# angeladai/sgnn

Hardware: AMD Instinct MI355X
Metric: TSDF blocks/sec fwd+bwd (64^3@5% occ, bs32) (higher is better)
Workload: dtype f32

## Files before the change

include/sgnn_hip.h:

```cpp
#ifndef SGNN_HIP_H
#define SGNN_HIP_H

#include <stdint.h>

#ifdef __cplusplus
extern "C" {
#endif

#define SGNN_OK 0
#define SGNN_EINVAL (-1)
#define SGNN_EHIP (-2)
#define SGNN_EOVERFLOW (-3)
#define SGNN_ENOWS (-4)

#define SGNN_STATUS_COORD_RANGE 1
#define SGNN_STATUS_DUPLICATE 2
#define SGNN_STATUS_OVERFLOW 4

typedef void *sgnn_stream_t;

const char *sgnn_last_error(void);
int sgnn_version(void);
const char *sgnn_arch(void);


int64_t sgnn_hash_capacity(int64_t n);

int sgnn_coords_from_i64(const int64_t *locs, int64_t n, int32_t *coords, int32_t *status,
                         const int64_t *n_dev, sgnn_stream_t stream);
int sgnn_coords_to_i64(const int32_t *coords, int64_t n, int64_t *locs, const int64_t *n_dev,
                       sgnn_stream_t stream);

int sgnn_hash_build(const int32_t *coords, int64_t n, uint64_t *keys, int32_t *vals, int64_t cap,
                    int32_t *status, const int64_t *n_dev, sgnn_stream_t stream);

int sgnn_hash_lookup(const uint64_t *keys, const int32_t *vals, int64_t cap, const int32_t *query,
                     int64_t m, int32_t *rows, const int64_t *m_dev, sgnn_stream_t stream);

#define SGNN_TUNE_UNKNOWN INT64_MIN
typedef struct sgnn_tune {
  int64_t conv_small;
  int64_t conv_small_rows;
  int64_t conv_unrolled;
  int64_t conv_one_round;
  int64_t conv_wide_epi;
  int64_t conv_dw_blocks;
  int64_t conv_dw_c1;
  int64_t rulebook_multi;
  int64_t scan_inline;
  int64_t chain_merged;
  int64_t prog_fusion;
  int64_t prog_lin_bn;
  int64_t prog_lin_add;
  int64_t bn_fuse;
} sgnn_tune;
int64_t sgnn_tune_set(const char *name, int64_t value);
int64_t sgnn_tune_get(const char *name);
const char *sgnn_tune_names(void);
const sgnn_tune *sgnn_tune_current(void);


int sgnn_rulebook_subm3(const uint64_t *keys, const int32_t *vals, int64_t cap,
                        const int32_t *coords, int64_t n, int32_t *nbr, int64_t ld,
                        const int64_t *n_dev, sgnn_stream_t stream);

#define SGNN_RULEBOOK_MULTI_MAX 4
int sgnn_rulebook_subm3_multi(int count, const uint64_t *const *keys, const int32_t *const *vals, const int64_t *caps,
                              const int32_t *const *coords, const int64_t *ns, int32_t *const *nbrs, const int64_t *lds,
                              const int64_t *const *n_devs, sgnn_stream_t stream);

int sgnn_rulebook_subm3_dense(const uint64_t *keys, const int32_t *vals, int64_t cap, const int32_t *coords, int64_t n,
                              int dim_z, int dim_y, int dim_x, int32_t *volume, int64_t volume_entries, int32_t *nbr,
                              int64_t ld, const int64_t *n_dev, sgnn_stream_t stream);
int sgnn_rulebook_subm3_volume(const int32_t *coords, int64_t n, int dim_z, int dim_y, int dim_x, int32_t *volume,
                               int64_t volume_entries, int32_t *nbr, int64_t ld, const int64_t *n_dev, int32_t *status,
                               sgnn_stream_t stream);

int64_t sgnn_down2_ws_bytes(int64_t nf);
int sgnn_rulebook_down2(const int32_t *fine_coords, int64_t nf, uint64_t *ckeys, int32_t *cvals,
                        int64_t ccap, int32_t *parent, int32_t *coarse_coords, int64_t *n_coarse,
                        void *ws, int64_t ws_bytes, sgnn_stream_t stream);
int sgnn_down2_tables(const int32_t *fine_coords, const int32_t *parent, int64_t nf,
                      int32_t *children, int64_t ldc, int64_t nc, int32_t *ptable, int64_t ldf,
                      const int64_t *nf_dev, const int64_t *nc_dev, sgnn_stream_t stream);

int64_t sgnn_down2_chain_ws_bytes(int64_t cap);
int sgnn_down2_chain(const int32_t *fine_coords, int64_t n0, const int64_t *n0_dev, int64_t cap, int depth,
                     void *const *ckeys, void *const *cvals, int64_t ccap, void *const *parent,
                     void *const *coarse_coords, int64_t *counts_dev, const int64_t *level_caps, int32_t *status,
                     void *ws, int64_t ws_bytes, sgnn_stream_t stream);

int64_t sgnn_down2_chain_tables_ws_bytes(int64_t cap, int depth);
int sgnn_down2_chain_tables(const int32_t *fine_coords, const int64_t *n0_dev, int64_t cap, int depth,
                            void *const *ckeys, void *const *cvals, int64_t ccap, void *const *parent,
                            void *const *coarse_coords, int64_t *counts_dev, const int64_t *level_caps,
                            void *const *children, void *const *ptable, int32_t *status, void *ws, int64_t ws_bytes,
                            sgnn_stream_t stream);

#define SGNN_CONV_TRANSPOSE_W 1
#define SGNN_CONV_FLIP_K 2
int sgnn_conv_fwd(const float *x, int64_t n_in, int cin, const float *w, int K, const int32_t *table,
                  int64_t ld, int64_t n_out, int cout, float *y, int flags, int in_shift,
                  sgnn_stream_t stream);

int sgnn_conv_fwd_ex(const float *x, int64_t n_in, int cin, const float *w, int K, const int32_t *table,
                     int64_t ld, int64_t n_out, int cout, float *y, int flags, int in_shift,
                     const int32_t *kmap, const int32_t *kadd, int in_mul, int groups, int table_rows,
                     sgnn_stream_t stream);
int sgnn_conv_bwd_weight_ex(const float *x, int64_t n_in, int cin, const float *dy, int cout,
                            const int32_t *table, int64_t ld, int K, int64_t n_out, float *dw, int in_shift,
                            const int32_t *kmap, const int32_t *kadd, int in_mul, int groups, int table_rows,
                            void *ws, int64_t ws_bytes, sgnn_stream_t stream);

int64_t sgnn_conv_stats_blocks(int64_t n_out);
int sgnn_conv_fwd_epi(const float *x, int64_t n_in, int cin, int64_t ldx, const float *w, int K,
                      const int32_t *table, int64_t ld, int64_t n_out, int cout, float *y, int64_t ldy, int flags,
                      const float *addend, int64_t ld_add, int stats, double *partial, const float *bn_x,
                      int64_t ld_bnx, const float *mean, const float *invstd, const float *gamma, const float *beta,
                      float leak, sgnn_stream_t stream);

int64_t sgnn_conv_bwd_weight_ws_bytes(int64_t n_out, int K, int cin, int cout);
int sgnn_conv_bwd_weight(const float *x, int64_t n_in, int cin, const float *dy, int cout,
                         const int32_t *table, int64_t ld, int K, int64_t n_out, float *dw, int in_shift, void *ws,
                         int64_t ws_bytes, sgnn_stream_t stream);

int sgnn_expand_weights(const float *w, int cin, int cout, float *wc, sgnn_stream_t stream);
int sgnn_expand_weights_bwd(const float *dwc, int cin, int cout, float *dw, sgnn_stream_t stream);

int64_t sgnn_bn_ws_bytes(int64_t n, int c);
int sgnn_bn_fwd(const float *x, int64_t n, int c, const float *gamma, const float *beta,
                float *running_mean, float *running_var, float eps, float momentum, int training,
                float leak, float *save_mean, float *save_invstd, float *y, void *ws,
                int64_t ws_bytes, sgnn_stream_t stream);
int sgnn_bn_bwd(const float *x, const float *dy, int64_t n, int c, const float *gamma,
                const float *beta, const float *save_mean, const float *save_invstd, int training,
                float leak, float *dx, float *dgamma, float *dbeta, void *ws, int64_t ws_bytes,
                sgnn_stream_t stream);
int sgnn_bn_bwd_add(const float *x, const float *dy, int64_t n, int c, const float *gamma, const float *beta,
                    const float *save_mean, const float *save_invstd, int training, float leak,
                    const float *addend, float *dx, float *dgamma, float *dbeta, void *ws, int64_t ws_bytes,
                    sgnn_stream_t stream);

int sgnn_bn_fwd_ex(const float *x, int64_t ldx, int64_t n, int c, const float *gamma, const float *beta,
                   float *running_mean, float *running_var, float eps, float momentum, int training, float leak,
                   float *save_mean, float *save_invstd, float *y, int64_t ldy, const double *pre_partial,
                   int64_t pre_nblk, void *ws, int64_t ws_bytes, sgnn_stream_t stream);
int sgnn_bn_bwd_ex(const float *x, int64_t ldx, const float *dy, int64_t ld_dy, int64_t n, int c, const float *gamma,
                   const float *beta, const float *save_mean, const float *save_invstd, int training, float leak,
                   const float *addend, int64_t ld_add, float *dx, int64_t ld_dx, float *dgamma, float *dbeta,
                   const double *pre_partial, int64_t pre_nblk, void *ws, int64_t ws_bytes, sgnn_stream_t stream);

int sgnn_copy_multi(void *const *dst, const void *const *src, const int64_t *bytes, int nregions, sgnn_stream_t stream);

int sgnn_gather_rows(const float *src, int c, const int32_t *idx, int64_t m, float *dst,
                     sgnn_stream_t stream);
int sgnn_gather_rows_dn(const float *src, int c, const int32_t *idx, const int64_t *m_dev, int64_t m_cap,
                        float *dst, sgnn_stream_t stream);
int sgnn_concat3_rows(const float *a, int ca, const int32_t *ia, const float *b, int cb, const int32_t *ib,
                      const float *c, int cc, const int32_t *ic, int64_t m, float *dst, sgnn_stream_t stream);
int sgnn_concat3_rows_bwd(const float *ddst, int ca, const int32_t *ia, int cb, const int32_t *ib, int cc,
                          const int32_t *ic, int64_t m, float *da, int64_t na, float *db, int64_t nb, float *dc,
                          int64_t nc, sgnn_stream_t stream);
int sgnn_scatter_rows(const float *src, int c, const int32_t *idx, int64_t m, float *dst,
                      int64_t n_dst, const int64_t *m_dev, sgnn_stream_t stream);
int sgnn_gather_sum(const float *src, int c, const int32_t *table, int64_t ld, int K,
                    int64_t n_out, float *dst, sgnn_stream_t stream);
int sgnn_repeat_rows(const float *src, int c, int64_t n, int rep, float *dst, sgnn_stream_t stream);
int sgnn_sum_groups(const float *src, int c, int64_t n, int rep, float *dst, sgnn_stream_t stream);
int sgnn_concat_rows(const float *a, int ca, const int32_t *ia, const float *b, int cb,
                     const int32_t *ib, int64_t m, float *dst, sgnn_stream_t stream);
int sgnn_concat_rows_bwd(const float *ddst, int ca, const int32_t *ia, int cb, const int32_t *ib,
                         int64_t m, float *da, int64_t na, float *db, int64_t nb,
                         sgnn_stream_t stream);
int sgnn_add(const float *a, const float *b, int64_t count, float *y, sgnn_stream_t stream);

int sgnn_expand8_coords(const int32_t *coords, int64_t n, int32_t *out, const int64_t *n_dev, sgnn_stream_t stream);
int sgnn_expand8_coords_i64(const int32_t *coords, int64_t n, int32_t *out, int64_t *locs, const int64_t *n_dev,
                            sgnn_stream_t stream);
int sgnn_dense_coords(int batch, int d0, int d1, int d2, int32_t *out, sgnn_stream_t stream);
int64_t sgnn_compact_ws_bytes(int64_t n);
int sgnn_compact_sigmoid(const float *logits, int64_t stride, int64_t n, int32_t *sel,
                         int64_t *count, void *ws, int64_t ws_bytes, sgnn_stream_t stream);
int sgnn_compact_dense(const int32_t *coords, int64_t n, const float *vol, int batch, int d0, int d1, int d2,
                       int32_t *sel, int64_t *count, void *ws, int64_t ws_bytes, sgnn_stream_t stream);
int sgnn_compact_mask(const uint8_t *mask, int64_t n, int32_t *sel, int64_t *count, void *ws,
                      int64_t ws_bytes, sgnn_stream_t stream);
int sgnn_compact_sigmoid_cap(const float *logits, int64_t stride, int64_t n, const int64_t *n_dev, int32_t *sel,
                             int64_t *count2, int64_t keep_cap, int32_t *status, void *ws, int64_t ws_bytes,
                             sgnn_stream_t stream);
int sgnn_compact_dense_cap(const int32_t *coords, int64_t n, const int64_t *n_dev, const float *vol, int batch, int d0,
                           int d1, int d2, int32_t *sel, int64_t *count2, int64_t keep_cap, int32_t *status, void *ws,
                           int64_t ws_bytes, sgnn_stream_t stream);
int sgnn_compact_sigmoid_cap_locs(const float *logits, int64_t stride, int64_t n, const int64_t *n_dev,
                                  const int32_t *coords, int32_t *sel, int32_t *locs, int64_t *count2, int64_t keep_cap,
                                  int32_t *status, void *ws, int64_t ws_bytes, sgnn_stream_t stream);
int sgnn_compact_dense_cap_locs(const int32_t *coords, int64_t n, const int64_t *n_dev, const float *vol, int batch, int d0,
                                int d1, int d2, int32_t *sel, int32_t *locs, int64_t *count2, int64_t keep_cap,
                                int32_t *status, void *ws, int64_t ws_bytes, sgnn_stream_t stream);

int sgnn_sparse_to_dense(const float *feats, const int32_t *coords, int64_t n, int c, float *dense,
                         int batch, int d0, int d1, int d2, sgnn_stream_t stream);
int sgnn_dense_to_sparse(const float *dense, const int32_t *coords, int64_t n, int c, float *feats,
                         int batch, int d0, int d1, int d2, sgnn_stream_t stream);

int64_t sgnn_linear_ws_bytes(int64_t n, int cin, int cout);
int sgnn_linear_fwd(const float *x, int64_t n, int cin, const float *w, const float *bias, int cout,
                    float *y, sgnn_stream_t stream);
// ... 366 lines not shown
```

sgnn_amd/csrc/bn.hip:

```cpp
#include "common.h"

#define BN_MAX_BLOCKS 2048
#define BN_FLUSH 2
#ifndef BN_U
#define BN_U 2
#endif
#define BN_FUSE_BLOCKS 4096
#define BN_FUSE_MAXC 64

struct BnGeom {
  int vec;
  int cq;
  int rpb;
};

static BnGeom bn_geom(int c) {
  BnGeom g;
  g.vec = (c % 4 == 0) ? 4 : 1;
  g.cq = c / g.vec;
  g.rpb = 256 / g.cq;
  if (g.rpb < 1) g.rpb = 1;
  return g;
}

static BnGeom bn_geom_scalar(int c) {
  BnGeom g;
  g.vec = 1;
  g.cq = c;
  g.rpb = 256 / c;
  if (g.rpb < 1) g.rpb = 1;
  return g;
}

static int bn_blocks(int64_t n, const BnGeom &g) {
  int64_t b = (n + (int64_t)g.rpb * BN_FLUSH - 1) / ((int64_t)g.rpb * BN_FLUSH);
  if (b < 1) b = 1;
  if (b > BN_MAX_BLOCKS) b = BN_MAX_BLOCKS;
  return (int)b;
}

SGNN_EXPORT int64_t sgnn_bn_ws_bytes(int64_t n, int c) {
  (void)n;
  return (int64_t)BN_MAX_BLOCKS * 2 * c * (int64_t)sizeof(double) + 4 * (int64_t)c * sizeof(float) + 256;
}

template <int VEC>
__device__ __forceinline__ void load_vec(const float *p, float (&v)[VEC]) {
  if constexpr (VEC == 4) {
    const float4 t = *reinterpret_cast<const float4 *>(p);
    v[0] = t.x; v[1] = t.y; v[2] = t.z; v[3] = t.w;
  } else {
    v[0] = *p;
  }
}
template <int VEC>
__device__ __forceinline__ void store_vec(float *p, const float (&v)[VEC]) {
  if constexpr (VEC == 4) {
    *reinterpret_cast<float4 *>(p) = make_float4(v[0], v[1], v[2], v[3]);
  } else {
    *p = v[0];
  }
}

template <int VEC, int MODE, bool LIN = false>
__global__ __launch_bounds__(256) void k_bn_partial(const float *__restrict__ x, int64_t ldx,
                                                   const float *__restrict__ dy, int64_t ld_dy, int64_t n, int c,
                                                   int cq, int rpb, const float *__restrict__ mean,
                                                   const float *__restrict__ invstd,
                                                   const float *__restrict__ gamma,
                                                   const float *__restrict__ beta, float leak,
                                                   double *__restrict__ partial, const int64_t *n_dev, BnLin lin) {
  extern __shared__ double sh[];
  const int tid = threadIdx.x;
  unsigned nblk = gridDim.x;
  if (n_dev) {
    n = sgnn_dyn_n(n, n_dev);
    int64_t b = (n + (int64_t)rpb * BN_FLUSH - 1) / ((int64_t)rpb * BN_FLUSH);
    if (b < 1) b = 1;
    if (b > BN_MAX_BLOCKS) b = BN_MAX_BLOCKS;
    if (b < (int64_t)nblk) nblk = (unsigned)b;
    if (blockIdx.x >= nblk) {
      for (int o = tid; o < 2 * c; o += 256) partial[(size_t)blockIdx.x * 2 * c + o] = 0.0;
      return;
    }
  }
  const int col = tid % cq, rloc = tid / cq;
  const bool active = rloc < rpb;
  double sa[VEC], sb[VEC];
#pragma unroll
  for (int v = 0; v < VEC; ++v) sa[v] = sb[v] = 0.0;
  float m_[VEC], is_[VEC], g_[VEC], b_[VEC];
  float lw[2][VEC];
  if constexpr (LIN) {
#pragma unroll
    for (int o = 0; o < 2; ++o)
#pragma unroll
      for (int v = 0; v < VEC; ++v) lw[o][v] = (active && o < lin.nout) ? lin.w[o][col * VEC + v] : 0.f;
  }
  if (MODE == 1 && active) {
#pragma unroll
    for (int v = 0; v < VEC; ++v) {
      m_[v] = mean[col * VEC + v];
      is_[v] = invstd[col * VEC + v];
      g_[v] = gamma ? gamma[col * VEC + v] : 1.f;
      b_[v] = beta ? beta[col * VEC + v] : 0.f;
    }
  }
  if (active) {
    const int64_t step = (int64_t)nblk * rpb;
    int64_t row = (int64_t)blockIdx.x * rpb + rloc;
    while (row < n) {
      float fa[VEC], fb[VEC];
#pragma unroll
      for (int v = 0; v < VEC; ++v) fa[v] = fb[v] = 0.f;
      float xv[BN_FLUSH][VEC], dv[BN_FLUSH][VEC];
      bool keep[BN_FLUSH];
#pragma unroll
      for (int it = 0; it < BN_FLUSH; ++it) {
        const int64_t rr = row + it * step;
        keep[it] = rr < n;
        const int64_t rc = rr < n ? rr : row;
        load_vec<VEC>(x + rc * ldx + col * VEC, xv[it]);
        if constexpr (LIN) {
#pragma unroll
          for (int v = 0; v < VEC; ++v) dv[it][v] = 0.f;
#pragma unroll
          for (int o = 0; o < 2; ++o)
            if (o < lin.nout) {
              const float gv = lin.g[rc * lin.ldg + o];
#pragma unroll
              for (int v = 0; v < VEC; ++v) dv[it][v] = fmaf(gv, lw[o][v], dv[it][v]);
            }
        } else if (MODE == 1) {
          load_vec<VEC>(dy + rc * ld_dy + col * VEC, dv[it]);
        }
      }
#pragma unroll
      for (int it = 0; it < BN_FLUSH; ++it) {
        if (MODE == 0) {
#pragma unroll
          for (int v = 0; v < VEC; ++v) {
            const float xm = keep[it] ? xv[it][v] : 0.f;
            fa[v] += xm;
            fb[v] = fmaf(xm, xm, fb[v]);
          }
        } else {
#pragma unroll
          for (int v = 0; v < VEC; ++v) {
            const float xh = (xv[it][v] - m_[v]) * is_[v];
            const float yv = fmaf(xh, g_[v], b_[v]);
            const float dz = keep[it] ? (yv > 0.f ? dv[it][v] : dv[it][v] * leak) : 0.f;
            fa[v] += dz;
            fb[v] = fmaf(dz, xh, fb[v]);
          }
        }
      }
      row += (int64_t)BN_FLUSH * step;
#pragma unroll
      for (int v = 0; v < VEC; ++v) {
        sa[v] += (double)fa[v];
        sb[v] += (double)fb[v];
      }
    }
  }
  double *mine = sh + ((size_t)rloc * cq + col) * 2 * VEC;
  if (active) {
#pragma unroll
    for (int v = 0; v < VEC; ++v) {
      mine[v] = sa[v];
      mine[VEC + v] = sb[v];
    }
  }
  __syncthreads();
  const int outs = cq * VEC * 2;
  for (int o = tid; o < outs; o += 256) {
    const int which = o / (cq * VEC);
    const int ch = o % (cq * VEC);
    const int cg = ch / VEC, v = ch % VEC;
    double s = 0.0;
    for (int rr = 0; rr < rpb; ++rr) s += sh[((size_t)rr * cq + cg) * 2 * VEC + which * VEC + v];
    partial[((size_t)blockIdx.x * 2 + which) * c + ch] = s;
  }
}

__device__ __forceinline__ void bn_reduce_channel(const double *__restrict__ partial, int nblk, int c, int ch,
                                                  double *sh, double &s, double &s2) {
  double a = 0.0, b = 0.0;
  for (int blk = threadIdx.x; blk < nblk; blk += 8 * 256) {
    double va[8], vb[8];
#pragma unroll
    for (int u = 0; u < 8; ++u) {
      const int bi = blk + u * 256;
      const bool ok = bi < nblk;
      va[u] = ok ? partial[((size_t)bi * 2 + 0) * c + ch] : 0.0;
      vb[u] = ok ? partial[((size_t)bi * 2 + 1) * c + ch] : 0.0;
    }
#pragma unroll
    for (int u = 0; u < 8; ++u) {
      a += va[u];
      b += vb[u];
    }
  }
  sh[threadIdx.x] = a;
  sh[256 + threadIdx.x] = b;
  __syncthreads();
  for (int d = 128; d > 0; d >>= 1) {
    if (threadIdx.x < d) {
      sh[threadIdx.x] += sh[threadIdx.x + d];
      sh[256 + threadIdx.x] += sh[256 + threadIdx.x + d];
    }
    __syncthreads();
  }
  s = sh[0];
  s2 = sh[256];
}

__global__ __launch_bounds__(256) void k_bn_finalize_fwd(const double *__restrict__ partial, int nblk,
                                                        int64_t n, int c, float eps, float momentum,
                                                        float *__restrict__ running_mean,
                                                        float *__restrict__ running_var,
                                                        float *__restrict__ save_mean,
                                                        float *__restrict__ save_invstd, const int64_t *n_dev) {
  __shared__ double sh[512];
  n = sgnn_dyn_n(n, n_dev);
  const int ch = blockIdx.x;
  double s, s2;
  bn_reduce_channel(partial, nblk, c, ch, sh, s, s2);
  if (threadIdx.x == 0) {
    if (n <= 0) {
      save_mean[ch] = 0.f;
      save_invstd[ch] = 0.f;
      return;
    }
    const double mean = s / (double)n;
    double var = s2 / (double)n - mean * mean;
    if (var < 0.0) var = 0.0;
    save_mean[ch] = (float)mean;
    save_invstd[ch] = (float)(1.0 / sqrt(var + (double)eps));
    if (running_mean) running_mean[ch] = momentum * running_mean[ch] + (1.f - momentum) * (float)mean;
    if (running_var) {
      const double unb = var * ((double)n / (double)(n > 1 ? n - 1 : 1));
      running_var[ch] = momentum * running_var[ch] + (1.f - momentum) * (float)unb;
    }
  }
}

__global__ __launch_bounds__(256) void k_bn_eval_stats(const float *__restrict__ running_mean,
                                                      const float *__restrict__ running_var, int c, float eps,
                                                      float *__restrict__ save_mean,
                                                      float *__restrict__ save_invstd) {
  for (int ch = threadIdx.x; ch < c; ch += 256) {
    save_mean[ch] = running_mean[ch];
    save_invstd[ch] = 1.0f / sqrtf(running_var[ch] + eps);
  }
}


struct BnFuse {
  const double *partial;
  int nblk;
  float eps, momentum;
  float *running_mean, *running_var, *save_mean, *save_invstd;
  float *dgamma, *dbeta;
};

#ifndef BN_TOTALS_WIDE
#define BN_TOTALS_WIDE 1
#endif
typedef double f64x2 __attribute__((ext_vector_type(2)));
__device__ __forceinline__ void bn_fuse_totals(const BnFuse &f, int c, double *scratch, double *tot) {
  const int tid = threadIdx.x;
  const int tpc = 256 / c;
  if (BN_TOTALS_WIDE && (c & 1) == 0 && (((uintptr_t)f.partial) & 15) == 0) {
    const int hp = c >> 1;
    const int p2 = tid % hp, which = (tid / hp) & 1, part = tid / c;
    f64x2 acc = {0.0, 0.0};
    if (part < tpc) {
      constexpr int U = 32;
      for (int blk = part; blk < f.nblk; blk += U * tpc) {
        f64x2 v[U];
#pragma unroll
        for (int u = 0; u < U; ++u) {
          const int bi = blk + u * tpc;
          v[u] = bi < f.nblk ? *reinterpret_cast<const f64x2 *>(f.partial + ((size_t)bi * 2 + which) * c + 2 * p2) : f64x2{0.0, 0.0};
        }
#pragma unroll
        for (int u = 0; u < U; ++u) acc += v[u];
      }
      scratch[which * 256 + part * c + 2 * p2] = acc[0];
      scratch[which * 256 + part * c + 2 * p2 + 1] = acc[1];
    }
  } else {
    const int ch = tid % c, part = tid / c;
    double a = 0.0, b = 0.0;
    if (part < tpc) {
      for (int blk = part; blk < f.nblk; blk += 8 * tpc) {
        double va[8], vb[8];
#pragma unroll
        for (int u = 0; u < 8; ++u) {
          const int bi = blk + u * tpc;
          const bool ok = bi < f.nblk;
          va[u] = ok ? f.partial[((size_t)bi * 2 + 0) * c + ch] : 0.0;
          vb[u] = ok ? f.partial[((size_t)bi * 2 + 1) * c + ch] : 0.0;
        }
#pragma unroll
        for (int u = 0; u < 8; ++u) {
          a += va[u];
          b += vb[u];
        }
      }
      scratch[part * c + ch] = a;
      scratch[256 + part * c + ch] = b;
    }
  }
  __syncthreads();
  if (tid < c) {
    double s1 = 0.0, s2 = 0.0;
    for (int p = 0; p < tpc; ++p) {
      s1 += scratch[p * c + tid];
      s2 += scratch[256 + p * c + tid];
    }
    tot[tid] = s1;
    tot[c + tid] = s2;
  }
  __syncthreads();
}

template <int VEC, bool FUSE>
__global__ __launch_bounds__(256) void k_bn_apply(const float *__restrict__ x, int64_t ldx, int64_t n, int c, int cq,
                                                 int rpb, const float *__restrict__ mean,
                                                 const float *__restrict__ invstd,
                                                 const float *__restrict__ gamma,
                                                 const float *__restrict__ beta, float leak,
                                                 float *__restrict__ y, int64_t ldy, BnFuse fuse,
                                                 const int64_t *n_dev) {
  __shared__ float s_mean[BN_FUSE_MAXC], s_inv[BN_FUSE_MAXC];
  __shared__ double s_scratch[512], s_tot[2 * BN_FUSE_MAXC];
  n = sgnn_dyn_n(n, n_dev);
  if (n <= 0) return;
  if constexpr (FUSE) {
    bn_fuse_totals(fuse, c, s_scratch, s_tot);
    for (int ch = threadIdx.x; ch < c; ch += 256) {
      const double s1 = s_tot[ch], s2 = s_tot[c + ch];
      const double mu = s1 / (double)n;
      double var = s2 / (double)n - mu * mu;
      if (var < 0.0) var = 0.0;
      const float fm = (float)mu, fi = (float)(1.0 / sqrt(var + (double)fuse.eps));
      s_mean[ch] = fm;
      s_inv[ch] = fi;
      if (blockIdx.x == 0) {
        fuse.save_mean[ch] = fm;
        fuse.save_invstd[ch] = fi;
        if (fuse.running_mean) fuse.running_mean[ch] = fuse.momentum * fuse.running_mean[ch] + (1.f - fuse.momentum) * fm;
        if (fuse.running_var) {
          const double unb = var * ((double)n / (double)(n > 1 ? n - 1 : 1));
          fuse.running_var[ch] = fuse.momentum * fuse.running_var[ch] + (1.f - fuse.momentum) * (float)unb;
        }
      }
    }
    __syncthreads();
    mean = s_mean;
    invstd = s_inv;
  }
  const int tid = threadIdx.x;
  const int col = tid % cq, rloc = tid / cq;
  if (rloc >= rpb) return;
  float km[VEC], ki[VEC], kg[VEC], kb[VEC];
#pragma unroll
  for (int v = 0; v < VEC; ++v) {
    const int ch = col * VEC + v;
    km[v] = mean[ch];
    ki[v] = invstd[ch];
    kg[v] = gamma ? gamma[ch] : 1.f;
    kb[v] = beta ? beta[ch] : 0.f;
  }
  const int64_t step = (int64_t)gridDim.x * rpb;
  for (int64_t r0 = (int64_t)blockIdx.x * rpb + rloc; r0 < n; r0 += step * BN_U) {
    float xv[BN_U][VEC];
#pragma unroll
    for (int u = 0; u < BN_U; ++u) {
      const int64_t r = r0 + u * step;
      load_vec<VEC>(x + (r < n ? r : r0) * ldx + col * VEC, xv[u]);
    }
#pragma unroll
    for (int u = 0; u < BN_U; ++u) {
      const int64_t r = r0 + u * step;
      if (r >= n) break;
      float yv[VEC];
#pragma unroll
      for (int v = 0; v < VEC; ++v) yv[v] = sgnn_bn_act(xv[u][v], km[v], ki[v], kg[v], kb[v], leak);
      store_vec<VEC>(y + r * ldy + col * VEC, yv);
    }
  }
}

__global__ __launch_bounds__(256) void k_bn_finalize_bwd(const double *__restrict__ partial, int nblk,
                                                        int64_t n, int c, float *__restrict__ dgamma,
                                                        float *__restrict__ dbeta, float *__restrict__ coef,
                                                        const int64_t *n_dev) {
  __shared__ double sh[512];
  n = sgnn_dyn_n(n, n_dev);
  const int ch = blockIdx.x;
  double s, s2;
  bn_reduce_channel(partial, nblk, c, ch, sh, s, s2);
  if (threadIdx.x == 0) {
    if (dbeta) dbeta[ch] = (float)s;
    if (dgamma) dgamma[ch] = (float)s2;
    coef[ch] = n > 0 ? (float)(s / (double)n) : 0.f;
    coef[c + ch] = n > 0 ? (float)(s2 / (double)n) : 0.f;
  }
}

template <int VEC, bool LIN, bool FUSE>
__global__ __launch_bounds__(256) void k_bn_bwd_apply(const float *__restrict__ x, int64_t ldx,
                                                     const float *__restrict__ dy, int64_t ld_dy, int64_t n, int c,
                                                     int cq, int rpb, const float *__restrict__ mean,
                                                     const float *__restrict__ invstd,
                                                     const float *__restrict__ gamma,
                                                     const float *__restrict__ beta, float leak, int training,
                                                     const float *__restrict__ coef, float *dx, int64_t ld_dx,
                                                     BnFuse fuse, const float *addend, int64_t ld_add,
                                                     const int64_t *n_dev, BnLin lin) {
  __shared__ float s_coef[2 * BN_FUSE_MAXC];
  __shared__ double s_scratch[512], s_tot[2 * BN_FUSE_MAXC];
  n = sgnn_dyn_n(n, n_dev);
  if constexpr (FUSE) {
    bn_fuse_totals(fuse, c, s_scratch, s_tot);
    for (int ch = threadIdx.x; ch < c; ch += 256) {
      const double s1 = s_tot[ch], s2 = s_tot[c + ch];
      s_coef[ch] = n > 0 ? (float)(s1 / (double)n) : 0.f;
      s_coef[c + ch] = n > 0 ? (float)(s2 / (double)n) : 0.f;
      if (blockIdx.x == 0) {
        if (fuse.dbeta) fuse.dbeta[ch] = (float)s1;
        if (fuse.dgamma) fuse.dgamma[ch] = (float)s2;
      }
    }
    __syncthreads();
    coef = s_coef;
  }
  const int tid = threadIdx.x;
  const int col = tid % cq, rloc = tid / cq;
  if (rloc >= rpb) return;
  float km[VEC], ki[VEC], kg[VEC], kb[VEC], k4[VEC], k5[VEC];
#pragma unroll
  for (int v = 0; v < VEC; ++v) {
    const int ch = col * VEC + v;
    km[v] = mean[ch];
    ki[v] = invstd[ch];
    kg[v] = gamma ? gamma[ch] : 1.f;
    kb[v] = beta ? beta[ch] : 0.f;
    k4[v] = training ? coef[ch] : 0.f;
    k5[v] = training ? coef[c + ch] : 0.f;
  }
  float lw[2][VEC];
  if constexpr (LIN) {
#pragma unroll
    for (int o = 0; o < 2; ++o)
#pragma unroll
      for (int v = 0; v < VEC; ++v) lw[o][v] = o < lin.nout ? lin.w[o][col * VEC + v] : 0.f;
  }
  const int64_t step = (int64_t)gridDim.x * rpb;
  for (int64_t r0 = (int64_t)blockIdx.x * rpb + rloc; r0 < n; r0 += step * BN_U) {
    float xv[BN_U][VEC], dv[BN_U][VEC], av[BN_U][VEC];
#pragma unroll
    for (int u = 0; u < BN_U; ++u) {
      const int64_t r = r0 + u * step, rc = (r < n ? r : r0);
      load_vec<VEC>(x + rc * ldx + col * VEC, xv[u]);
      if constexpr (LIN) {
#pragma unroll
        for (int v = 0; v < VEC; ++v) dv[u][v] = 0.f;
#pragma unroll
        for (int o = 0; o < 2; ++o)
          if (o < lin.nout) {
            const float gv = lin.g[rc * lin.ldg + o];
#pragma unroll
            for (int v = 0; v < VEC; ++v) dv[u][v] = fmaf(gv, lw[o][v], dv[u][v]);
          }
      } else {
        load_vec<VEC>(dy + rc * ld_dy + col * VEC, dv[u]);
      }
      if (addend) load_vec<VEC>(addend + rc * ld_add + col * VEC, av[u]);
    }
#pragma unroll
    for (int u = 0; u < BN_U; ++u) {
      const int64_t r = r0 + u * step;
      if (r >= n) break;
      float ov[VEC];
#pragma unroll
      for (int v = 0; v < VEC; ++v) {
        const float xh = (xv[u][v] - km[v]) * ki[v];
        const float t = fmaf(xh, kg[v], kb[v]);
        const float dz = t > 0.f ? dv[u][v] : dv[u][v] * leak;
        float d = dz;
        if (training) d = dz - k4[v] - xh * k5[v];
        ov[v] = d * kg[v] * ki[v];
        if (addend) ov[v] += av[u][v];
      }
      store_vec<VEC>(dx + r * ld_dx + col * VEC, ov);
    }
  }
}

static bool bn_fuse_ok(int64_t nblk, int c, int apply_grid) {
  return c <= BN_FUSE_MAXC && nblk <= BN_FUSE_BLOCKS && nblk * (int64_t)apply_grid * 2 * c * (int64_t)sizeof(double) <= (48ll << 20);
}

static int bn_apply_grid(int64_t n, const BnGeom &g) {
  int64_t b = (n + (int64_t)g.rpb * BN_U - 1) / ((int64_t)g.rpb * BN_U);
  if (b < 1) b = 1;
  if (b > 4096) b = 4096;
  return (int)b;
}

int sgnn_bn_fwd_impl(const float *x, int64_t ldx, int64_t n, int c, const float *gamma, const float *beta,
                     float *running_mean, float *running_var, float eps, float momentum, int training, float leak,
                     float *save_mean, float *save_invstd, float *y, int64_t ldy, const double *pre_partial,
                     int64_t pre_nblk, void *ws, int64_t ws_bytes, sgnn_stream_t stream, const int64_t *n_dev) {
  hipStream_t s = (hipStream_t)stream;
  SGNN_CHECK_ARG(n >= 0 && c >= 1 && (c % 4 == 0 ? c <= 1024 : c <= 256) && save_mean && save_invstd);
  SGNN_CHECK_ARG(training || (running_mean && running_var));
  if (ldx <= 0) ldx = c;
  if (ldy <= 0) ldy = c;
  SGNN_CHECK_ARG(ldx >= c && ldy >= c);
  BnGeom g = bn_geom(c);
  if (g.vec == 4 && (ldx % 4 || ldy % 4 || ((uintptr_t)x & 15) || ((uintptr_t)y & 15))) g = bn_geom_scalar(c);
  if (g.cq > 256) {
    sgnn_set_error("sgnn_bn_fwd: %d channels need 16-byte aligned rows (row strides multiples of 4 floats)", c);
    return SGNN_EINVAL;
  }
  BnFuse fuse{nullptr, 0, 0.f, 0.f, nullptr, nullptr, nullptr, nullptr, nullptr, nullptr};
  if (training && n > 0) {
    SGNN_CHECK_ARG(x);
    const double *partial = pre_partial;
    int64_t nblk = pre_nblk;
    if (!partial) {
      if (!ws || ws_bytes < sgnn_bn_ws_bytes(n, c)) {
        sgnn_set_error("sgnn_bn_fwd: workspace too small");
        return SGNN_ENOWS;
      }
      nblk = bn_blocks(n, g);
      const size_t shbytes = (size_t)g.rpb * g.cq * 2 * g.vec * sizeof(double);
      if (g.vec == 4)
        SGNN_LAUNCH((k_bn_partial<4, 0>), dim3((unsigned)nblk), dim3(256), shbytes, s, x, ldx, nullptr, 0, n, c,
                           g.cq, g.rpb, nullptr, nullptr, nullptr, nullptr, 0.f, (double *)ws, n_dev, BnLin{});
      else
        SGNN_LAUNCH((k_bn_partial<1, 0>), dim3((unsigned)nblk), dim3(256), shbytes, s, x, ldx, nullptr, 0, n, c,
                           g.cq, g.rpb, nullptr, nullptr, nullptr, nullptr, 0.f, (double *)ws, n_dev, BnLin{});
      partial = (const double *)ws;
    }
    if (g_tune.bn_fuse && bn_fuse_ok(nblk, c, bn_apply_grid(n, g)))
      fuse = BnFuse{partial, (int)nblk, eps, momentum, running_mean, running_var, save_mean, save_invstd, nullptr, nullptr};
    else
      SGNN_LAUNCH(k_bn_finalize_fwd, dim3(c), dim3(256), 0, s, partial, (int)nblk, n, c, eps, momentum,
                         running_mean, running_var, save_mean, save_invstd, n_dev);
  } else if (training) {
    SGNN_HIP_TRY(hipMemsetAsync(save_mean, 0, c * sizeof(float), s));
    SGNN_HIP_TRY(hipMemsetAsync(save_invstd, 0, c * sizeof(float), s));
  } else {
    SGNN_LAUNCH(k_bn_eval_stats, dim3(1), dim3(256), 0, s, (const float *)running_mean,
                       (const float *)running_var, c, eps, save_mean, save_invstd);
  }
  if (n > 0) {
    SGNN_CHECK_ARG(x && y);
    const int grid = bn_apply_grid(n, g);
#define BN_APPLY(VECV, FUSEV)                                                                                 \
  SGNN_LAUNCH((k_bn_apply<VECV, FUSEV>), dim3(grid), dim3(256), 0, s, x, ldx, n, c, g.cq, g.rpb,              \
              (const float *)save_mean, (const float *)save_invstd, gamma, beta, leak, y, ldy, fuse, n_dev)
    if (g.vec == 4 && fuse.partial) BN_APPLY(4, true);
    else if (g.vec == 4) BN_APPLY(4, false);
    else if (fuse.partial) BN_APPLY(1, true);
    else BN_APPLY(1, false);
#undef BN_APPLY
  }
  SGNN_CHECK_LAUNCH();
  return SGNN_OK;
}

SGNN_EXPORT int sgnn_bn_fwd(const float *x, int64_t n, int c, const float *gamma, const float *beta,
                            float *running_mean, float *running_var, float eps, float momentum, int training,
                            float leak, float *save_mean, float *save_invstd, float *y, void *ws,
                            int64_t ws_bytes, sgnn_stream_t stream) {
  return sgnn_bn_fwd_impl(x, c, n, c, gamma, beta, running_mean, running_var, eps, momentum, training, leak, save_mean,
                          save_invstd, y, c, nullptr, 0, ws, ws_bytes, stream);
}

SGNN_EXPORT int sgnn_bn_fwd_ex(const float *x, int64_t ldx, int64_t n, int c, const float *gamma, const float *beta,
                               float *running_mean, float *running_var, float eps, float momentum, int training,
                               float leak, float *save_mean, float *save_invstd, float *y, int64_t ldy,
                               const double *pre_partial, int64_t pre_nblk, void *ws, int64_t ws_bytes,
                               sgnn_stream_t stream) {
  return sgnn_bn_fwd_impl(x, ldx, n, c, gamma, beta, running_mean, running_var, eps, momentum, training, leak,
                          save_mean, save_invstd, y, ldy, pre_partial, pre_nblk, ws, ws_bytes, stream);
}

SGNN_EXPORT int sgnn_bn_bwd(const float *x, const float *dy, int64_t n, int c, const float *gamma,
                            const float *beta, const float *save_mean, const float *save_invstd, int training,
                            float leak, float *dx, float *dgamma, float *dbeta, void *ws, int64_t ws_bytes,
                            sgnn_stream_t stream) {
  return sgnn_bn_bwd_impl(x, c, dy, c, n, c, gamma, beta, save_mean, save_invstd, training, leak, nullptr, c, dx, c,
                          dgamma, dbeta, nullptr, 0, ws, ws_bytes, stream);
}

SGNN_EXPORT int sgnn_bn_bwd_add(const float *x, const float *dy, int64_t n, int c, const float *gamma,
                                const float *beta, const float *save_mean, const float *save_invstd, int training,
                                float leak, const float *addend, float *dx, float *dgamma, float *dbeta, void *ws,
                                int64_t ws_bytes, sgnn_stream_t stream) {
  return sgnn_bn_bwd_impl(x, c, dy, c, n, c, gamma, beta, save_mean, save_invstd, training, leak, addend, c, dx, c,
                          dgamma, dbeta, nullptr, 0, ws, ws_bytes, stream);
}

SGNN_EXPORT int sgnn_bn_bwd_ex(const float *x, int64_t ldx, const float *dy, int64_t ld_dy, int64_t n, int c,
                               const float *gamma, const float *beta, const float *save_mean,
                               const float *save_invstd, int training, float leak, const float *addend,
                               int64_t ld_add, float *dx, int64_t ld_dx, float *dgamma, float *dbeta,
                               const double *pre_partial, int64_t pre_nblk, void *ws, int64_t ws_bytes,
                               sgnn_stream_t stream) {
  return sgnn_bn_bwd_impl(x, ldx, dy, ld_dy, n, c, gamma, beta, save_mean, save_invstd, training, leak, addend, ld_add,
                          dx, ld_dx, dgamma, dbeta, pre_partial, pre_nblk, ws, ws_bytes, stream);
}

int sgnn_bn_bwd_impl(const float *x, int64_t ldx, const float *dy, int64_t ld_dy, int64_t n, int c, const float *gamma,
                     const float *beta, const float *save_mean, const float *save_invstd, int training, float leak,
                     const float *addend, int64_t ld_add, float *dx, int64_t ld_dx, float *dgamma, float *dbeta,
                     const double *pre_partial, int64_t pre_nblk, void *ws, int64_t ws_bytes, sgnn_stream_t stream,
                     const int64_t *n_dev, const BnLin *lin) {
  hipStream_t s = (hipStream_t)stream;
  SGNN_CHECK_ARG(n >= 0 && c >= 1 && (c % 4 == 0 ? c <= 1024 : c <= 256) && save_mean && save_invstd);
  SGNN_CHECK_ARG(!lin || (lin->g && lin->nout >= 1 && lin->nout <= 2 && lin->w[0] && (lin->nout < 2 || lin->w[1]) && !pre_partial));
  if (n == 0) {
    if (dgamma) SGNN_HIP_TRY(hipMemsetAsync(dgamma, 0, c * sizeof(float), s));
    if (dbeta) SGNN_HIP_TRY(hipMemsetAsync(dbeta, 0, c * sizeof(float), s));
    return SGNN_OK;
  }
  SGNN_CHECK_ARG(x && (dy || lin) && dx);
  if (ldx <= 0) ldx = c;
  if (ld_dy <= 0) ld_dy = c;
  if (ld_dx <= 0) ld_dx = c;
  if (ld_add <= 0) ld_add = c;
  SGNN_CHECK_ARG(ldx >= c && ld_dy >= c && ld_dx >= c && ld_add >= c);
  if (!ws || ws_bytes < sgnn_bn_ws_bytes(n, c)) {
    sgnn_set_error("sgnn_bn_bwd: workspace too small");
    return SGNN_ENOWS;
  }
  BnGeom g = bn_geom(c);
  if (g.vec == 4 && (ldx % 4 || ld_dy % 4 || ld_dx % 4 || ld_add % 4 || ((uintptr_t)x & 15) || ((uintptr_t)dy & 15) ||
                     ((uintptr_t)dx & 15) || ((uintptr_t)addend & 15)))
    g = bn_geom_scalar(c);
  if (g.cq > 256) {
    sgnn_set_error("sgnn_bn_bwd: %d channels need 16-byte aligned rows (row strides multiples of 4 floats)", c);
    return SGNN_EINVAL;
  }
  const double *partial = pre_partial;
  int64_t nblk = pre_nblk;
  float *coef = (float *)((char *)ws + (size_t)BN_MAX_BLOCKS * 2 * c * sizeof(double));
  if (!partial) {
    nblk = bn_blocks(n, g);
    const size_t shbytes = (size_t)g.rpb * g.cq * 2 * g.vec * sizeof(double);
    if (lin && g.vec == 4)
      SGNN_LAUNCH((k_bn_partial<4, 1, true>), dim3((unsigned)nblk), dim3(256), shbytes, s, x, ldx, dy, ld_dy, n, c, g.cq,
// ... 32 lines not shown
```

sgnn_amd/csrc/common.h:

```cpp
#pragma once
#include <hip/hip_runtime.h>
#include <stdint.h>
#include <stdio.h>
#include "../../include/sgnn_hip.h"

#define SGNN_EXPORT extern "C" __attribute__((visibility("default")))

extern "C" int sgnn_stamp(const char *label, sgnn_stream_t stream);
extern sgnn_tune g_tune;

void sgnn_set_error(const char *fmt, ...);
int sgnn_prof_begin_launch(int kind, int64_t n_out, int cin, int cout, int K, int flags, hipStream_t s);
void sgnn_prof_end_launch(int slot, hipStream_t s);

__device__ __forceinline__ float sgnn_bn_act(float x, float mean, float invstd, float gamma, float beta, float leak) {
  const float xh = (x - mean) * invstd;
  const float t = fmaf(xh, gamma, beta);
  return t > 0.f ? t : t * leak;
}

struct ConvEpi {
  int64_t ldx, ldy, ld_add;
  const float *addend;
  int stats;
  double *partial;
  const float *bn_x;
  int64_t ld_bnx;
  const float *mean, *invstd, *gamma, *beta;
  float leak;
  const int64_t *n_dev;
};

int sgnn_conv_fwd_impl(const float *x, int64_t n_in, int cin, const float *w, int K, const int32_t *table, int64_t ld,
                       int64_t n_out, int cout, float *y, int flags, int in_shift, const int32_t *kmap,
                       const int32_t *kadd, int in_mul, int groups, int table_rows, const ConvEpi *epi,
                       sgnn_stream_t stream);
int64_t sgnn_conv_grid_blocks(int64_t n_out, int cin, int cout, int K);
struct BnLin {
  const float *g;
  int64_t ldg;
  const float *w[2];
  int nout;
};
int sgnn_bn_fwd_impl(const float *x, int64_t ldx, int64_t n, int c, const float *gamma, const float *beta,
                     float *running_mean, float *running_var, float eps, float momentum, int training, float leak,
                     float *save_mean, float *save_invstd, float *y, int64_t ldy, const double *pre_partial,
                     int64_t pre_nblk, void *ws, int64_t ws_bytes, sgnn_stream_t stream, const int64_t *n_dev = nullptr);
int sgnn_bn_bwd_impl(const float *x, int64_t ldx, const float *dy, int64_t ld_dy, int64_t n, int c, const float *gamma,
                     const float *beta, const float *save_mean, const float *save_invstd, int training, float leak,
                     const float *addend, int64_t ld_add, float *dx, int64_t ld_dx, float *dgamma, float *dbeta,
                     const double *pre_partial, int64_t pre_nblk, void *ws, int64_t ws_bytes, sgnn_stream_t stream,
                     const int64_t *n_dev = nullptr, const struct BnLin *lin = nullptr);
bool sgnn_conv_epi_supported(int cin, int cout);
bool dw_shape_ok(int cin, int cout);
#define DW_BATCH_MAX 28
struct DwDesc {
  const float *partial;
  float *dw;
  int64_t nblk, elems;
  int blk0;
};
struct DwBatch {
  DwDesc d[DW_BATCH_MAX];
  int n;
};
extern DwBatch *sgnn_dw_batch;
int sgnn_dw_batch_flush(DwBatch *b, hipStream_t s);
int sgnn_gather_rows_ld(const float *src, int64_t ld_src, int c, const int32_t *idx, int64_t m, float *dst,
                        int64_t ld_dst, sgnn_stream_t stream, const int64_t *n_dev = nullptr);
int sgnn_gather_sum_ld(const float *src, int64_t ld_src, int c, const int32_t *table, int64_t ld, int K, int64_t n_out,
                       float *dst, int64_t ld_dst, sgnn_stream_t stream, const int64_t *n_dev = nullptr);
int sgnn_add_ld(const float *a, int64_t lda, const float *b, int64_t ldb, int64_t n, int c, float *y, int64_t ldy,
                sgnn_stream_t stream, const int64_t *n_dev = nullptr);
int sgnn_fill32(void *p, uint32_t pattern, int64_t words, hipStream_t s);
int sgnn_fill32_multi(void *const *p, const int64_t *words, int nregions, uint32_t pattern, hipStream_t s);
int sgnn_copy_words(void *dst, const void *src, int64_t words, hipStream_t s);
int sgnn_sum_groups_dn(const float *src, int c, int64_t n, int rep, float *dst, sgnn_stream_t stream, const int64_t *n_dev);
int sgnn_concat_rows_dn(const float *a, int ca, const int32_t *ia, const float *b, int cb, const int32_t *ib, int64_t m,
                        float *dst, sgnn_stream_t stream, const int64_t *n_dev);
int sgnn_concat_rows_bwd_dn(const float *ddst, int ca, const int32_t *ia, int cb, const int32_t *ib, int64_t m, float *da,
                            int64_t na, float *db, int64_t nb, sgnn_stream_t stream, const int64_t *n_dev);
int sgnn_concat3_rows_dn(const float *a, int ca, const int32_t *ia, const float *b, int cb, const int32_t *ib,
                         const float *c, int cc, const int32_t *ic, int64_t m, float *dst, sgnn_stream_t stream,
                         const int64_t *n_dev);
int sgnn_concat3_rows_bwd_dn(const float *ddst, int ca, const int32_t *ia, int cb, const int32_t *ib, int cc,
                             const int32_t *ic, int64_t m, float *da, int64_t na, float *db, int64_t nb, float *dc,
                             int64_t nc, sgnn_stream_t stream, const int64_t *n_dev);
int sgnn_conv_bwd_weight_impl(const float *x, int64_t n_in, int cin, int64_t ldx, const float *dy, int cout, int64_t ld_dy,
                              const int32_t *table, int64_t ld, int K, int64_t n_out, float *dw, int in_shift,
                              const int32_t *kmap, const int32_t *kadd, int in_mul, int groups, int table_rows, void *ws,
                              int64_t ws_bytes, sgnn_stream_t stream, const int64_t *n_dev = nullptr);
int sgnn_expand_maps(const int32_t **S, const int32_t **ST, const int32_t **PAR);
int sgnn_linear_fwd_rows(const float *x, int64_t n, int cin, const float *const *w, const float *const *b, int cout,
                         float *y, sgnn_stream_t stream, const int64_t *n_dev = nullptr);
int sgnn_linear_bwd_rows(const float *x, const float *dy, int64_t n, int cin, const float *const *w, int cout,
                         float *dx, float *const *dw, float *const *db, void *ws, int64_t ws_bytes,
                         sgnn_stream_t stream, const int64_t *n_dev = nullptr, const float *addend = nullptr,
                         int64_t ld_add = 0);

extern long long sgnn_launch_counter;
#define SGNN_LAUNCH(...)           \
  do {                             \
    ++sgnn_launch_counter;         \
    hipLaunchKernelGGL(__VA_ARGS__); \
  } while (0)

#define SGNN_CHECK_ARG(cond)                                                    \
  do {                                                                          \
    if (!(cond)) {                                                              \
      sgnn_set_error("%s: invalid argument: %s", __func__, #cond);              \
      return SGNN_EINVAL;                                                       \
    }                                                                           \
  } while (0)

#define SGNN_CHECK_LAUNCH()                                                     \
  do {                                                                          \
    hipError_t e_ = hipGetLastError();                                          \
    if (e_ != hipSuccess) {                                                     \
      sgnn_set_error("%s: HIP error: %s", __func__, hipGetErrorString(e_));     \
      return SGNN_EHIP;                                                         \
    }                                                                           \
  } while (0)

#define SGNN_HIP_TRY(expr)                                                      \
  do {                                                                          \
    hipError_t e_ = (expr);                                                     \
    if (e_ != hipSuccess) {                                                     \
      sgnn_set_error("%s: %s failed: %s", __func__, #expr, hipGetErrorString(e_)); \
      return SGNN_EHIP;                                                         \
    }                                                                           \
  } while (0)

__device__ __forceinline__ int64_t sgnn_dyn_n(int64_t n_host, const int64_t *n_dev) {
  if (!n_dev) return n_host;
  const int64_t v = *n_dev;
  return v < n_host ? (v < 0 ? 0 : v) : n_host;
}

static inline int sgnn_grid_for(int64_t work, int block, int cap = 1 << 20) {
  int64_t g = (work + block - 1) / block;
  if (g < 1) g = 1;
  if (g > cap) g = cap;
  return (int)g;
}

__device__ __forceinline__ unsigned sgnn_xcd_tile(unsigned b, unsigned nwg) {
  const unsigned q = nwg >> 3, r = nwg & 7u, xcd = b & 7u, i = b >> 3;
  return (xcd < r ? xcd * (q + 1) : r * (q + 1) + (xcd - r) * q) + i;
}

#define SGNN_EMPTY_KEY 0xFFFFFFFFFFFFFFFFull

__device__ __forceinline__ uint64_t sgnn_pack_key(int z, int y, int x, int b) {
  return ((uint64_t)(uint32_t)b << 48) | ((uint64_t)(uint32_t)z << 32) | ((uint64_t)(uint32_t)y << 16) |
         (uint64_t)(uint32_t)x;
}

__device__ __forceinline__ uint64_t sgnn_hash64(uint64_t k) {
  k ^= k >> 33;
  k *= 0xff51afd7ed558ccdull;
  k ^= k >> 33;
  k *= 0xc4ceb9fe1a85ec53ull;
  k ^= k >> 33;
  return k;
}

__device__ __forceinline__ int32_t sgnn_hash_find(const uint64_t *__restrict__ keys,
                                                  const int32_t *__restrict__ vals, uint64_t mask,
                                                  uint64_t key) {
  uint64_t slot = sgnn_hash64(key) & mask;
  while (true) {
    uint64_t k = keys[slot];
    if (k == key) return vals[slot];
    if (k == SGNN_EMPTY_KEY) return -1;
    slot = (slot + 1) & mask;
  }
}

__device__ __forceinline__ uint8_t sgnn_known_code(float s, float vs) {
  if (s < -vs) {
    const float q = __fdiv_rn(-s, vs);
    return !(q < 2147483648.0f) ? 2 : (uint8_t)max(2, min(255, (int)q + 1));
  }
  return s <= vs ? 1 : 0;
}

__device__ __forceinline__ int sgnn_block_rank256(bool flag, int *lds4, int &total) {
  const int lane = threadIdx.x & 63, wave = threadIdx.x >> 6;
  unsigned long long bal = __ballot(flag);
  int prefix = __popcll(bal & ((1ull << lane) - 1ull));
  if (lane == 0) lds4[wave] = __popcll(bal);
  __syncthreads();
  int w0 = lds4[0], w1 = lds4[1], w2 = lds4[2], w3 = lds4[3];
  __syncthreads();
  int base = (wave > 0 ? w0 : 0) + (wave > 1 ? w1 : 0) + (wave > 2 ? w2 : 0);
  total = w0 + w1 + w2 + w3;
  return base + prefix;
}

template <typename T, int NC>
__device__ __forceinline__ void sgnn_block_sum256(T (&sh)[NC][256], const T (&v)[NC]) {
  for (int c = 0; c < NC; ++c) sh[c][threadIdx.x] = v[c];
  __syncthreads();
  for (int d = 128; d > 0; d >>= 1) {
    if (threadIdx.x < d)
      for (int c = 0; c < NC; ++c) sh[c][threadIdx.x] += sh[c][threadIdx.x + d];
    __syncthreads();
  }
}
```

sgnn_amd/csrc/conv.hip:

```cpp
#include <stdlib.h>
#include "common.h"

#include "conv_common.h"

#define CONV_SMALL_GRID ((int64_t)((g_tune.conv_small_rows + CONV_ROWS_PER_BLOCK - 1) / CONV_ROWS_PER_BLOCK))

template <int CIN, int COUT, int M, bool EX, bool WEPI>
__device__ __forceinline__ void conv_fwd_body(const float *__restrict__ x, int64_t n_in,
                                              const float *__restrict__ w, const int32_t *__restrict__ table,
                                              int64_t ld, int K, int64_t n_out, float *y, int flags,
                                              int in_shift, const ConvEx &ex, const ConvEpi &epi, int wg_cap) {
  using C = ConvCfg<CIN, COUT>;
  constexpr int V = C::V, CINP = C::CINP, NT = C::NT, KC = C::KC;
  constexpr int RPW = 16 * M;
  __shared__ __attribute__((aligned(16))) float wl[KC * C::PER_K];
  __shared__ double sred[4 * 2 * NT * 16];
  static_assert(!WEPI || (NT == 1 && M == 4 && !EX && COUT % 4 == 0), "wide epilogue: one column tile of whole 16-byte chunks");
  __shared__ float ecst[WEPI ? 64 : 1];

  const int tid = threadIdx.x, lane = tid & 63, wave = tid >> 6;
  const int r = lane & 15, q = lane >> 4;
  const unsigned groups = EX ? (unsigned)ex.groups : 1u;
  unsigned nwg = gridDim.x;
  if (epi.n_dev) n_out = sgnn_dyn_n(n_out, epi.n_dev);
  int J = 1;
  if constexpr (!EX) {
    if (wg_cap > 0) {
      const int64_t w1 = (n_out + 4 * RPW - 1) / (4 * RPW);
      J = (int)((w1 + wg_cap - 1) / wg_cap);
      if (J < 1) J = 1;
    }
  }
  if (epi.n_dev || J > 1) {
    const int64_t rows_wg = (int64_t)4 * RPW * J;
    nwg = (unsigned)((n_out + rows_wg - 1) / rows_wg) * groups;
    if (blockIdx.x >= nwg) {
      if (!EX && epi.stats)
        for (int o = tid; o < 2 * COUT; o += 256) epi.partial[(size_t)blockIdx.x * 2 * COUT + o] = 0.0;
      return;
    }
  }
  const unsigned lin = sgnn_xcd_tile(blockIdx.x, nwg);
  const unsigned tile = lin / groups, grp = lin % groups;
  int64_t row0 = ((int64_t)tile * J * 4 + wave) * RPW;
  const int32_t *kmap = nullptr, *kadd_g = nullptr;
  if constexpr (EX) {
    w += (int64_t)grp * K * CIN * COUT;
    kmap = ex.kmap ? ex.kmap + grp * K : nullptr;
    kadd_g = ex.kadd ? ex.kadd + grp * K : nullptr;
  }
  const int table_rows = EX ? ex.table_rows : K;
  const bool transpose = flags & SGNN_CONV_TRANSPOSE_W, flip = flags & SGNN_CONV_FLIP_K;

  const uint32_t ldx4 = (uint32_t)epi.ldx * 4u;
  const __amdgpu_buffer_rsrc_t rs_x = make_rsrc(x, (uint32_t)(((n_in - 1) * epi.ldx + CIN) * 4));
  const __amdgpu_buffer_rsrc_t rs_t = make_rsrc(table, (uint32_t)((int64_t)table_rows * ld * 4));
  uint32_t lane_off = (uint32_t)(row0 + (lane & (RPW - 1))) * 4u;
  const uint32_t ld4 = (uint32_t)ld * 4u;
  int perm[M];
#pragma unroll
  for (int m = 0; m < M; ++m) perm[m] = (m * 16 + r) * 4;

  f32x4 acc[M][NT];
  double s1[NT], s2[NT];
#pragma unroll
  for (int nt = 0; nt < NT; ++nt) s1[nt] = s2[nt] = 0.0;
  if constexpr (WEPI) conv_epi_wide_constants<COUT>(ecst, epi, epi.stats);

  auto load_idx = [&](int k) -> int32_t {
    if constexpr (EX) {
      const int trow = kmap ? kmap[k] : k;
      int32_t id = (int32_t)__builtin_amdgcn_raw_buffer_load_b32(rs_t, lane_off, trow * ld4, 0);
      return (id >> in_shift) * ex.in_mul + ((kadd_g && id >= 0) ? kadd_g[k] : 0);
    } else {
      return (int32_t)__builtin_amdgcn_raw_buffer_load_b32(rs_t, lane_off, k * ld4, 0) >> in_shift;
    }
  };
  auto gather = [&](int32_t iv, float(&a)[M][V]) {
#pragma unroll
    for (int m = 0; m < M; ++m) {
      const int32_t id = __builtin_amdgcn_ds_bpermute(perm[m], iv);
      buf_load_floats<V>(rs_x, (uint32_t)id * ldx4 + (uint32_t)(q * V * 4), a[m]);
    }
  };
  auto stage = [&](int k) {
    conv_stage_weights<CIN, COUT>(wl, w, K, k, (K - k) < KC ? (K - k) : KC, transpose, flip);
  };
  auto load_b = [&](int kk, float(&b)[NT][V]) {
#pragma unroll
    for (int nt = 0; nt < NT; ++nt) {
      const float *bp = wl + (kk * NT * 16 + nt * 16 + r) * CINP + q * V;
#pragma unroll
      for (int s = 0; s < V; ++s) b[nt][s] = bp[s];
    }
  };
  auto mma_b = [&](float(&a)[M][V], const float(&b)[NT][V]) {
    if constexpr (CINP != CIN) {
#pragma unroll
      for (int m = 0; m < M; ++m)
#pragma unroll
        for (int s = 0; s < V; ++s)
          if (3 * V + s >= CIN) a[m][s] = (q >= conv_first_pad_quarter<CIN, V>(s)) ? 0.f : a[m][s];
    }
#pragma unroll
    for (int s = 0; s < V; ++s)
#pragma unroll
      for (int m = 0; m < M; ++m)
#pragma unroll
        for (int nt = 0; nt < NT; ++nt)
          acc[m][nt] = __builtin_amdgcn_mfma_f32_16x16x4f32(a[m][s], b[nt][s], acc[m][nt], 0, 0, 0);
  };
  auto mma = [&](int kk, float(&a)[M][V]) {
    float b[NT][V];
    load_b(kk, b);
    mma_b(a, b);
  };

  const int klast = K - 1;
  auto idx_at = [&](int k) { return load_idx(k < klast ? k : klast); };
  for (int j = 0; j < J; ++j) {
  if (j > 0) {
    const int64_t wg_row0 = ((int64_t)tile * J + j) * 4 * RPW;
    if (wg_row0 >= n_out) break;
    row0 = wg_row0 + wave * RPW;
    lane_off = (uint32_t)(row0 + (lane & (RPW - 1))) * 4u;
  }
  const bool restage = j == 0 || K > KC;
  EpiRows<WEPI ? M : 1> erows;
#pragma unroll
  for (int m = 0; m < M; ++m)
#pragma unroll
    for (int nt = 0; nt < NT; ++nt) acc[m][nt] = f32x4{0.f, 0.f, 0.f, 0.f};
  if constexpr (V <= 4 && (NT >= 2 || M == 1)) {
    float a0[M][V], a1[M][V], a2[M][V];
    for (int k0 = 0; k0 < K; k0 += KC) {
      const int kc = (K - k0) < KC ? (K - k0) : KC;
      if (restage) stage(k0);
      gather(idx_at(k0), a0);
      gather(idx_at(k0 + 1), a1);
      int32_t iv2 = idx_at(k0 + 2), iv3 = idx_at(k0 + 3), iv4 = idx_at(k0 + 4);
      int kk = 0;
      for (; kk + 2 < kc; kk += 3) {
        gather(iv2, a2);
        iv2 = idx_at(k0 + kk + 5);
        __builtin_amdgcn_sched_barrier(0);
        mma(kk, a0);
        __builtin_amdgcn_sched_barrier(0);
        gather(iv3, a0);
        iv3 = idx_at(k0 + kk + 6);
        __builtin_amdgcn_sched_barrier(0);
        mma(kk + 1, a1);
        __builtin_amdgcn_sched_barrier(0);
        gather(iv4, a1);
        iv4 = idx_at(k0 + kk + 7);
        __builtin_amdgcn_sched_barrier(0);
        mma(kk + 2, a2);
        __builtin_amdgcn_sched_barrier(0);
      }
      if (kk < kc) mma(kk, a0);
      if (kk + 1 < kc) mma(kk + 1, a1);
    }
  } else {
    float a0[M][V], a1[M][V], b0[NT][V], b1[NT][V];
    for (int k0 = 0; k0 < (WEPI ? 1 : K); k0 += KC) {
      const int kc = (K - k0) < KC ? (K - k0) : KC;
      if (restage) stage(k0);
      int32_t iv1 = idx_at(k0 + 1), iv2 = idx_at(k0 + 2);
      gather(idx_at(k0), a0);
      load_b(0, b0);
      int kk = 0;
      for (; kk + 1 < kc; kk += 2) {
        gather(iv1, a1);
        const int32_t iv3 = idx_at(k0 + kk + 3);
        load_b(kk + 1, b1);
        __builtin_amdgcn_sched_barrier(0);
        mma_b(a0, b0);
        __builtin_amdgcn_sched_barrier(0);
        gather(iv2, a0);
        iv1 = iv3;
        iv2 = idx_at(k0 + kk + 4);
        load_b(kk + 2 < kc ? kk + 2 : kc - 1, b0);
        __builtin_amdgcn_sched_barrier(0);
        mma_b(a1, b1);
        __builtin_amdgcn_sched_barrier(0);
      }
      if constexpr (WEPI) {
        __builtin_amdgcn_sched_barrier(0);
        if constexpr (SGNN_WEPI_EARLY != 0) conv_epi_wide_prefetch<COUT, M>(erows, row0, n_out, epi, epi.stats, x, SGNN_WEPI_EARLY);
        __builtin_amdgcn_sched_barrier(0);
      }
      if (kk < kc) mma_b(a0, b0);
    }
  }

  if constexpr (WEPI)
    conv_epi_wide_finish<COUT, M>(acc, erows, row0, n_out, y, epi, epi.stats, ecst, s1, s2, x);
  else
    conv_epilogue_rows<COUT, M, NT>(acc, row0, n_out, groups, grp, y, epi, EX ? 0 : epi.stats, x, s1, s2);
  }
  conv_epilogue_stats<COUT, NT>(s1, s2, epi, EX ? 0 : epi.stats, sred, blockIdx.x);
}

template <int CIN, int COUT, int M, bool EX>
__global__ __launch_bounds__(256) void k_conv_fwd(const float *__restrict__ x, int64_t n_in,
                                                 const float *__restrict__ w, const int32_t *__restrict__ table,
                                                 int64_t ld, int K, int64_t n_out, float *y, int flags,
                                                 int in_shift, ConvEx ex, ConvEpi epi, int wg_cap) {
  conv_fwd_body<CIN, COUT, M, EX, false>(x, n_in, w, table, ld, K, n_out, y, flags, in_shift, ex, epi, wg_cap);
}

template <int CIN, int COUT>
__global__ __launch_bounds__(256) __attribute__((amdgpu_waves_per_eu(4, 8))) void k_conv_fwd_w(
    const float *__restrict__ x, int64_t n_in, const float *__restrict__ w, const int32_t *__restrict__ table, int64_t ld,
    int K, int64_t n_out, float *y, int flags, int in_shift, ConvEx ex, ConvEpi epi, int wg_cap) {
  conv_fwd_body<CIN, COUT, CONV_MREP, false, true>(x, n_in, w, table, ld, K, n_out, y, flags, in_shift, ex, epi, wg_cap);
}

template <int CIN, int COUT>
__global__ __launch_bounds__(256) void k_conv_small(const float *__restrict__ x, int64_t n_in,
                                                   const float *__restrict__ w, const int32_t *__restrict__ table,
                                                   int64_t ld, int K, int64_t n_out, float *y, int flags, int in_shift,
                                                   ConvEpi epi) {
  using C = ConvCfg<CIN, COUT>;
  constexpr int V = C::V, CINP = C::CINP, NT = C::NT;
  constexpr int KW = 7;
  __shared__ float red[4][NT * 256];
  __shared__ double sred[4][2][NT * 16];
  const int tid = threadIdx.x, lane = tid & 63, wave = tid >> 6;
  const int r = lane & 15, q = lane >> 4;
  const int64_t row0 = (int64_t)blockIdx.x * 16;
  if (epi.n_dev) {
    n_out = sgnn_dyn_n(n_out, epi.n_dev);
    if (row0 >= n_out) {
      if (epi.stats)
        for (int o = tid; o < 2 * COUT; o += 256) epi.partial[(size_t)blockIdx.x * 2 * COUT + o] = 0.0;
      return;
    }
  }
  const bool transpose = flags & SGNN_CONV_TRANSPOSE_W, flip = flags & SGNN_CONV_FLIP_K;
  const int per = (K + 3) >> 2;
  const int k0 = wave * per;
  const int nk = (K - k0) < per ? ((K - k0) > 0 ? (K - k0) : 0) : per;

  const uint32_t ldx4 = (uint32_t)epi.ldx * 4u, ldy4 = (uint32_t)epi.ldy * 4u;
  const __amdgpu_buffer_rsrc_t rs_x = make_rsrc(x, (uint32_t)(((n_in - 1) * epi.ldx + CIN) * 4));
  const __amdgpu_buffer_rsrc_t rs_t = make_rsrc(table, (uint32_t)((int64_t)K * ld * 4));
  const __amdgpu_buffer_rsrc_t rs_y = make_rsrc(y, (uint32_t)(((n_out - 1) * epi.ldy + COUT) * 4));
  const uint32_t lane_off = (uint32_t)(row0 + r) * 4u;
  const uint32_t ld4 = (uint32_t)ld * 4u;

  int32_t id[KW];
#pragma unroll
  for (int kk = 0; kk < KW; ++kk) {
    const int k = k0 + (kk < nk ? kk : (nk > 0 ? nk - 1 : 0));
    id[kk] = (int32_t)__builtin_amdgcn_raw_buffer_load_b32(rs_t, lane_off, (k < K ? k : K - 1) * ld4, 0) >> in_shift;
  }
  float a[KW][V];
#pragma unroll
  for (int kk = 0; kk < KW; ++kk) buf_load_floats<V>(rs_x, (uint32_t)id[kk] * ldx4 + (uint32_t)(q * V * 4), a[kk]);
  float b[KW][NT][V];
  if (transpose) {
    const __amdgpu_buffer_rsrc_t rs_w = make_rsrc(w, (uint32_t)((int64_t)K * CIN * COUT * 4));
#pragma unroll
    for (int kk = 0; kk < KW; ++kk) {
      const int k = k0 + kk;
      const int ks = flip ? (K - 1 - k) : k;
#pragma unroll
      for (int nt = 0; nt < NT; ++nt) {
        const int n = nt * 16 + r;
        const bool okw = kk < nk && n < COUT;
        buf_load_floats<V>(rs_w, okw ? (uint32_t)((ks * COUT + n) * CIN + q * V) * 4u : 0xFFFFF800u, b[kk][nt]);
        if constexpr (CINP != CIN) {
#pragma unroll
          for (int s = 0; s < V; ++s)
            if (3 * V + s >= CIN) b[kk][nt][s] = (q >= conv_first_pad_quarter<CIN, V>(s)) ? 0.f : b[kk][nt][s];
        }
      }
    }
  } else if constexpr (V == 4 && CIN <= 16 && (CIN * COUT) % 4 == 0) {
    constexpr int SL = CIN * COUT, G4 = SL / 4, NL = (G4 + 63) / 64;
    static_assert(SL <= NT * 256, "the weight slice must fit the wave's partial-tile buffer");
    float *ws = red[wave];
    const __amdgpu_buffer_rsrc_t rs_w = make_rsrc(w, (uint32_t)((int64_t)K * SL * 4));
    float g[KW][NL][4];
#pragma unroll
    for (int kk = 0; kk < KW; ++kk) {
      const int k = k0 + kk;
      const int ks = flip ? (K - 1 - k) : k;
#pragma unroll
      for (int l = 0; l < NL; ++l) {
        const int e4 = l * 64 + lane;
        buf_load_floats<4>(rs_w, (kk < nk && e4 < G4) ? (uint32_t)(ks * SL + e4 * 4) * 4u : 0xFFFFF800u, g[kk][l]);
      }
    }
    auto wave_sync = [] {
      __builtin_amdgcn_fence(__ATOMIC_RELEASE, "wavefront");
      __builtin_amdgcn_wave_barrier();
      __builtin_amdgcn_fence(__ATOMIC_ACQUIRE, "wavefront");
    };
#pragma unroll
    for (int kk = 0; kk < KW; ++kk) {
      wave_sync();
#pragma unroll
      for (int l = 0; l < NL; ++l) {
        const int e4 = l * 64 + lane;
        if (e4 < G4) {
#pragma unroll
          for (int j = 0; j < 4; ++j) ws[e4 * 4 + j] = g[kk][l][j];
        }
      }
      wave_sync();
#pragma unroll
      for (int nt = 0; nt < NT; ++nt) {
        const int n = nt * 16 + r;
#pragma unroll
        for (int s = 0; s < V; ++s) {
          const int c = q * V + s;
          b[kk][nt][s] = (c < CIN && n < COUT) ? ws[c * COUT + n] : 0.f;
        }
      }
    }
  } else {
#pragma unroll
    for (int kk = 0; kk < KW; ++kk) {
      const int k = k0 + kk;
      const int ks = flip ? (K - 1 - k) : k;
#pragma unroll
      for (int nt = 0; nt < NT; ++nt) {
        const int n = nt * 16 + r;
#pragma unroll
        for (int s = 0; s < V; ++s) {
          const int c = q * V + s;
          float v = 0.f;
          if (kk < nk && c < CIN && n < COUT) v = w[((int64_t)ks * CIN + c) * COUT + n];
          b[kk][nt][s] = v;
        }
      }
    }
  }
  if constexpr (CINP != CIN) {
#pragma unroll
    for (int kk = 0; kk < KW; ++kk)
#pragma unroll
      for (int s = 0; s < V; ++s)
        if (3 * V + s >= CIN) a[kk][s] = (q >= conv_first_pad_quarter<CIN, V>(s)) ? 0.f : a[kk][s];
  }
  f32x4 acc[2][NT];
#pragma unroll
  for (int h = 0; h < 2; ++h)
#pragma unroll
    for (int nt = 0; nt < NT; ++nt) acc[h][nt] = f32x4{0.f, 0.f, 0.f, 0.f};
#pragma unroll
  for (int kk = 0; kk < KW; ++kk) {
    if (kk < nk) {
#pragma unroll
      for (int s = 0; s < V; ++s)
#pragma unroll
        for (int nt = 0; nt < NT; ++nt)
          acc[kk & 1][nt] = __builtin_amdgcn_mfma_f32_16x16x4f32(a[kk][s], b[kk][nt][s], acc[kk & 1][nt], 0, 0, 0);
    }
  }
#pragma unroll
  for (int nt = 0; nt < NT; ++nt)
#pragma unroll
    for (int i = 0; i < 4; ++i) red[wave][nt * 256 + (q * 4 + i) * 16 + r] = acc[0][nt][i] + acc[1][nt][i];
  __syncthreads();

  const bool has_add = epi.addend != nullptr;
  const __amdgpu_buffer_rsrc_t rs_a =
      make_rsrc(has_add ? epi.addend : x, has_add ? (uint32_t)(((n_out - 1) * epi.ld_add + COUT) * 4) : 0u);
  const uint32_t lda4 = (uint32_t)epi.ld_add * 4u;
  const int stats = epi.stats;
  const __amdgpu_buffer_rsrc_t rs_b =
      make_rsrc(stats == 2 ? epi.bn_x : x, stats == 2 ? (uint32_t)(((n_out - 1) * epi.ld_bnx + COUT) * 4) : 0u);
  const uint32_t ldb4 = (uint32_t)epi.ld_bnx * 4u;
  const int orow_l = tid >> 4, ocol_l = tid & 15;
  const int64_t row = row0 + orow_l;
#pragma unroll
  for (int nt = 0; nt < NT; ++nt) {
    const int col = nt * 16 + ocol_l;
    const bool ok = col < COUT && row < n_out;
    const int e = nt * 256 + orow_l * 16 + ocol_l;
    float v = (red[0][e] + red[1][e]) + (red[2][e] + red[3][e]);
    const uint32_t orow = (uint32_t)row;
    if (has_add) v += __uint_as_float(__builtin_amdgcn_raw_buffer_load_b32(rs_a, ok ? orow * lda4 + col * 4u : 0xFFFFFFFFu, 0, 0));
    __builtin_amdgcn_raw_buffer_store_b32(__float_as_uint(v), rs_y, ok ? orow * ldy4 + col * 4u : 0xFFFFFFFFu, 0, 0);
    if (stats) {
      double f1 = 0.0, f2 = 0.0;
      if (stats == 1) {
        f1 = ok ? (double)v : 0.0;
        f2 = f1 * f1;
      } else {
        float cm = 0.f, ci = 0.f, cg = 1.f, cb = 0.f;
        if (col < COUT) {
          cm = epi.mean[col];
          ci = epi.invstd[col];
          cg = epi.gamma ? epi.gamma[col] : 1.f;
          cb = epi.beta ? epi.beta[col] : 0.f;
        }
        const float xb = __uint_as_float(__builtin_amdgcn_raw_buffer_load_b32(rs_b, ok ? orow * ldb4 + col * 4u : 0xFFFFFFFFu, 0, 0));
        const float xh = (xb - cm) * ci;
        const float t = fmaf(xh, cg, cb);
        const float dz = ok ? (t > 0.f ? v : v * epi.leak) : 0.f;
        f1 = (double)dz;
        f2 = (double)dz * (double)xh;
      }
      f1 += __shfl_xor(f1, 16); f2 += __shfl_xor(f2, 16);
      f1 += __shfl_xor(f1, 32); f2 += __shfl_xor(f2, 32);
      if (lane < 16) {
        sred[wave][0][nt * 16 + lane] = f1;
        sred[wave][1][nt * 16 + lane] = f2;
      }
    }
  }
  if (stats) {
    __syncthreads();
    for (int o = tid; o < 2 * NT * 16; o += 256) {
      const int which = o / (NT * 16), col = o % (NT * 16);
      if (col < COUT)
        epi.partial[((size_t)blockIdx.x * 2 + which) * COUT + col] =
            (sred[0][which][col] + sred[1][which][col]) + (sred[2][which][col] + sred[3][which][col]);
    }
  }
}

__global__ __launch_bounds__(256) void k_conv_fwd_generic(const float *__restrict__ x, int cin,
                                                         const float *__restrict__ w, int K,
                                                         const int32_t *__restrict__ table, int64_t ld,
                                                         int64_t n_out, int cout, float *__restrict__ y,
                                                         int flags, int in_shift, ConvEx ex, const int64_t *n_dev) {
  n_out = sgnn_dyn_n(n_out, n_dev);
  const int64_t t = (int64_t)blockIdx.x * 256 + threadIdx.x;
  if (t >= n_out * ex.groups * cout) return;
  const int64_t orow = t / cout;
  const int n = (int)(t - orow * cout);
  const int64_t row = orow / ex.groups;
  const int grp = (int)(orow - row * ex.groups);
  w += (int64_t)grp * K * cin * cout;
  const bool transpose = flags & SGNN_CONV_TRANSPOSE_W, flip = flags & SGNN_CONV_FLIP_K;
  float acc = 0.f;
  for (int k = 0; k < K; ++k) {
    const int32_t idx = table[(int64_t)(ex.kmap ? ex.kmap[grp * K + k] : k) * ld + row];
    if (idx < 0) continue;
    const float *xr = x + ((int64_t)(idx >> in_shift) * ex.in_mul + (ex.kadd ? ex.kadd[grp * K + k] : 0)) * cin;
    const int ks = flip ? (K - 1 - k) : k;
    for (int c = 0; c < cin; ++c) {
      const float wv = transpose ? w[((int64_t)ks * cout + n) * cin + c] : w[((int64_t)ks * cin + c) * cout + n];
      acc = fmaf(xr[c], wv, acc);
    }
  }
  y[t] = acc;
}

#define CONV_EX_CASES(X) \
  X(48, 16) X(16, 48) X(24, 8) X(8, 24) X(16, 24) X(24, 16) X(24, 32) X(32, 24) X(64, 32) X(32, 64) X(56, 28) X(28, 56)

#define CONV_FWD_CASES(X) \
  X(1, 8) X(8, 8) X(8, 12) X(12, 12) X(12, 16) X(16, 16) X(34, 16) X(30, 16) X(26, 16) X(48, 16) \
  X(8, 1) X(12, 8) X(16, 12) X(16, 34) X(16, 30) X(16, 26) X(16, 48) X(32, 16) X(16, 32) X(4, 16) X(16, 4) \
  X(16, 24) X(24, 16) X(24, 32) X(32, 24) X(64, 32) X(32, 64) X(56, 28) X(28, 56) X(32, 32) X(28, 16) X(16, 28)

int64_t sgnn_conv_grid_blocks(int64_t n_out, int cin, int cout, int K) {
  const int64_t grid4 = (n_out + CONV_ROWS_PER_BLOCK - 1) / CONV_ROWS_PER_BLOCK;
  if (grid4 < CONV_SMALL_GRID) return (n_out + 15) / 16;
  return grid4;
}


bool sgnn_conv_u_supported(int cin, int cout, int K);
bool sgnn_conv_u_launch(const float *x, int64_t n_in, int cin, const float *w, int K, const int32_t *table, int64_t ld,
                        int64_t n_out, int cout, float *y, int flags, int in_shift, const ConvEpi &epi, hipStream_t s);

bool conv_wide_epi_ok(const ConvEpi &epi, const float *y, int K) {
  if (!g_tune.conv_wide_epi || K > 27 || (epi.ldy & 3) || ((uintptr_t)y & 15)) return false;
  if (epi.addend && ((epi.ld_add & 3) || ((uintptr_t)epi.addend & 15))) return false;
  if (epi.stats == 2 && ((epi.ld_bnx & 3) || ((uintptr_t)epi.bn_x & 15))) return false;
  return true;
}
template <int CI, int CO, bool EXV>
static void conv_launch_big(unsigned grid4, hipStream_t s, const float *x, int64_t n_in, const float *w, const int32_t *table,
                            int64_t ld, int K, int64_t n_out, float *y, int flags, int in_shift, const ConvEx &ex,
                            const ConvEpi &epi) {
  if constexpr (!EXV && CO % 4 == 0 && CO <= 16 && CI <= 16) {
    static_assert(ConvCfg<CI, CO>::KC >= 27, "one weight chunk holds a 3x3x3 filter");
    if (conv_wide_epi_ok(epi, y, K)) {
      SGNN_LAUNCH((k_conv_fwd_w<CI, CO>), dim3(grid4), dim3(256), 0, s, x, n_in, w, table, ld, K, n_out, y, flags, in_shift,
                  ex, epi, !g_tune.conv_one_round ? 0 : conv_wg_capacity<k_conv_fwd_w<CI, CO>>());
      return;
    }
  }
  SGNN_LAUNCH((k_conv_fwd<CI, CO, CONV_MREP, EXV>), dim3(grid4), dim3(256), 0, s, x, n_in, w, table, ld, K, n_out, y,
              flags, in_shift, ex, epi,
              (EXV || !g_tune.conv_one_round) ? 0 : conv_wg_capacity<k_conv_fwd<CI, CO, CONV_MREP, EXV>>());
}

bool sgnn_conv_epi_supported(int cin, int cout) {
#define X(CI, CO) \
  if (cin == CI && cout == CO) return true;
  CONV_FWD_CASES(X)
#undef X
  return false;
}

int sgnn_conv_fwd_impl(const float *x, int64_t n_in, int cin, const float *w, int K, const int32_t *table, int64_t ld,
                       int64_t n_out, int cout, float *y, int flags, int in_shift, const int32_t *kmap,
                       const int32_t *kadd, int in_mul, int groups, int table_rows, const ConvEpi *epi_in,
                       sgnn_stream_t stream) {
  SGNN_CHECK_ARG(cin >= 1 && cout >= 1 && K >= 1 && K <= 64 && n_out >= 0 && ld >= n_out && in_shift >= 0 &&
                 in_shift < 31 && in_mul >= 1 && groups >= 1 && groups <= 64 && table_rows >= 1 &&
                 table_rows <= 64 && (kmap || table_rows >= K));
  if (n_out == 0) return SGNN_OK;
  SGNN_CHECK_ARG(x && w && table && y && n_in >= 1);
  SGNN_CHECK_ARG(ld % CONV_ROWS_PER_BLOCK == 0);
  ConvEpi epi{};
  if (epi_in) epi = *epi_in;
  if (epi.ldx <= 0) epi.ldx = cin;
  if (epi.ldy <= 0) epi.ldy = cout;
  if (epi.ld_add <= 0) epi.ld_add = cout;
  if (epi.ld_bnx <= 0) epi.ld_bnx = cout;
  const bool plain = !kmap && !kadd && in_mul == 1 && groups == 1 && table_rows == K;
  const bool has_epi = epi.ldx != cin || epi.ldy != cout || epi.addend || epi.stats;
  SGNN_CHECK_ARG(epi.ldx >= cin && epi.ldx <= 1024 && epi.ldy >= cout && epi.ldy <= 1024 && epi.ld_add >= cout &&
                 epi.ld_add <= 1024 && epi.ld_bnx >= cout && epi.ld_bnx <= 1024);
  SGNN_CHECK_ARG(epi.stats >= 0 && epi.stats <= 2 && (!epi.stats || (plain && epi.partial)));
  SGNN_CHECK_ARG(epi.stats != 2 || (epi.bn_x && epi.mean && epi.invstd));
  SGNN_CHECK_ARG(!epi.stats || K <= 28);
  const int64_t lmax = epi.ldy > epi.ld_add ? (epi.ldy > epi.ld_bnx ? epi.ldy : epi.ld_bnx)
                                            : (epi.ld_add > epi.ld_bnx ? epi.ld_add : epi.ld_bnx);
  if (n_in * epi.ldx * 4 > 0xFFFFF000ll || n_out * groups * lmax * 4 > 0xFFFFF000ll ||
      (int64_t)table_rows * ld * 4 > 0xFFFFF000ll) {
    sgnn_set_error("sgnn_conv_fwd: a slab exceeds the 4 GiB raw-buffer window (n_in=%lld cin=%d n_out=%lld cout=%d)",
                   (long long)n_in, cin, (long long)n_out, cout);
    return SGNN_EOVERFLOW;
  }
  hipStream_t s = (hipStream_t)stream;
  const ConvEx ex{kmap, kadd, in_mul, groups, table_rows};
  const unsigned grid4 = (unsigned)((n_out + CONV_ROWS_PER_BLOCK - 1) / CONV_ROWS_PER_BLOCK) * (unsigned)groups;
  const unsigned grid1 = (unsigned)((n_out + 63) / 64) * (unsigned)groups;
  const bool small = grid4 < CONV_SMALL_GRID;
  bool done = false;
  const int prof = sgnn_prof_begin_launch(0, n_out * groups, cin, cout, K, flags, s);
#define LAUNCH_FWD(CI, CO, EXV)                                                                         \
  do {                                                                                                  \
    if (small && !EXV && K <= 28 && (g_tune.conv_small || epi.stats))                                      \
      SGNN_LAUNCH((k_conv_small<CI, CO>), dim3((unsigned)((n_out + 15) / 16)), dim3(256), 0, s,         \
                         x, n_in, w, table, ld, K, n_out, y, flags, in_shift, epi);                     \
    else if (small)                                                                                     \
      SGNN_LAUNCH((k_conv_fwd<CI, CO, 1, EXV>), dim3(grid1), dim3(256), 0, s, x, n_in, w, table,        \
                         ld, K, n_out, y, flags, in_shift, ex, epi, 0);                                 \
    else                                                                                                \
      conv_launch_big<CI, CO, EXV>(grid4, s, x, n_in, w, table, ld, K, n_out, y, flags, in_shift, ex, epi); \
    done = true;                                                                                        \
  } while (0)
  if (plain && !small && g_tune.conv_unrolled && sgnn_conv_u_supported(cin, cout, K))
    done = sgnn_conv_u_launch(x, n_in, cin, w, K, table, ld, n_out, cout, y, flags, in_shift, epi, s);
#define X(CI, CO) \
  if (!done && plain && cin == CI && cout == CO) LAUNCH_FWD(CI, CO, false);
  CONV_FWD_CASES(X)
#undef X
#define X(CI, CO) \
  if (!done && !plain && cin == CI && cout == CO) LAUNCH_FWD(CI, CO, true);
  CONV_EX_CASES(X)
#undef X
  if (!done) {
    if (has_epi) {
      sgnn_set_error("sgnn_conv_fwd_epi: strided / fused epilogues need one of the compiled (cin, cout) shapes, got (%d, %d)", cin, cout);
      return SGNN_EINVAL;
    }
    const int64_t total = n_out * groups * cout;
    SGNN_LAUNCH(k_conv_fwd_generic, dim3((unsigned)((total + 255) / 256)), dim3(256), 0, s, x, cin, w, K,
                       table, ld, n_out, cout, y, flags, in_shift, ex, epi.n_dev);
  }
  sgnn_prof_end_launch(prof, s);
  SGNN_CHECK_LAUNCH();
  return SGNN_OK;
}

SGNN_EXPORT int sgnn_conv_fwd_ex(const float *x, int64_t n_in, int cin, const float *w, int K, const int32_t *table,
                                 int64_t ld, int64_t n_out, int cout, float *y, int flags, int in_shift,
                                 const int32_t *kmap, const int32_t *kadd, int in_mul, int groups,
                                 int table_rows, sgnn_stream_t stream) {
  return sgnn_conv_fwd_impl(x, n_in, cin, w, K, table, ld, n_out, cout, y, flags, in_shift, kmap, kadd, in_mul,
                            groups, table_rows, nullptr, stream);
}

SGNN_EXPORT int sgnn_conv_fwd(const float *x, int64_t n_in, int cin, const float *w, int K, const int32_t *table,
                              int64_t ld, int64_t n_out, int cout, float *y, int flags, int in_shift,
                              sgnn_stream_t stream) {
  return sgnn_conv_fwd_impl(x, n_in, cin, w, K, table, ld, n_out, cout, y, flags, in_shift, nullptr, nullptr, 1, 1,
                            K, nullptr, stream);
}

SGNN_EXPORT int64_t sgnn_conv_stats_blocks(int64_t n_out) { return n_out > 0 ? sgnn_conv_grid_blocks(n_out, 0, 0, 0) : 0; }

SGNN_EXPORT int sgnn_conv_fwd_epi(const float *x, int64_t n_in, int cin, int64_t ldx, const float *w, int K,
                                  const int32_t *table, int64_t ld, int64_t n_out, int cout, float *y, int64_t ldy,
                                  int flags, const float *addend, int64_t ld_add, int stats, double *partial,
                                  const float *bn_x, int64_t ld_bnx, const float *mean, const float *invstd,
                                  const float *gamma, const float *beta, float leak, sgnn_stream_t stream) {
  ConvEpi epi{ldx, ldy, ld_add, addend, stats, partial, bn_x, ld_bnx, mean, invstd, gamma, beta, leak, nullptr};
  return sgnn_conv_fwd_impl(x, n_in, cin, w, K, table, ld, n_out, cout, y, flags, 0, nullptr, nullptr, 1, 1, K, &epi,
                            stream);
}

__device__ int32_t g_expand_maps[192];

int sgnn_expand_maps(const int32_t **S, const int32_t **ST, const int32_t **PAR) {
  static const int32_t *base = nullptr;
  if (!base) {
    int32_t host[192];
    for (int g = 0; g < 8; ++g)
      for (int i = 0; i < 8; ++i) {
        const int o0 = ((i >> 2) & 1) - 1 + ((g >> 2) & 1), o1 = ((i >> 1) & 1) - 1 + ((g >> 1) & 1),
                  o2 = (i & 1) - 1 + (g & 1);
        const int srow = (o0 + 1) * 9 + (o1 + 1) * 3 + (o2 + 1);
        host[g * 8 + i] = srow;
        host[64 + g * 8 + i] = 26 - srow;
        host[128 + g * 8 + i] = g;
      }
    SGNN_HIP_TRY(hipMemcpyToSymbol(HIP_SYMBOL(g_expand_maps), host, sizeof(host)));
    void *p = nullptr;
    SGNN_HIP_TRY(hipGetSymbolAddress(&p, HIP_SYMBOL(g_expand_maps)));
    base = (const int32_t *)p;
  }
  *S = base;
  *ST = base + 64;
  *PAR = base + 128;
  return SGNN_OK;
}

__device__ __forceinline__ void axis_taps(int j, int i, int &lo, int &hi) {
  if (j == 0) { lo = i ? 0 : -1; hi = i ? 1 : -1; }
  else        { lo = i ? 1 : -1; hi = i ? 1 : 0; }
}

__global__ __launch_bounds__(256) void k_expand_weights(const float *__restrict__ w, int cc, float *__restrict__ wc) {
  const int t = blockIdx.x * 256 + threadIdx.x;
  if (t >= 64 * cc) return;
  const int gi = t / cc, e = t - gi * cc, g = gi >> 3, i = gi & 7;
  int l0, h0, l1, h1, l2, h2;
  axis_taps((g >> 2) & 1, (i >> 2) & 1, l0, h0);
  axis_taps((g >> 1) & 1, (i >> 1) & 1, l1, h1);
  axis_taps(g & 1, i & 1, l2, h2);
  float acc = 0.f;
  for (int dz = l0; dz <= h0; ++dz)
    for (int dy = l1; dy <= h1; ++dy)
      for (int dx = l2; dx <= h2; ++dx) acc += w[(size_t)((dz + 1) * 9 + (dy + 1) * 3 + (dx + 1)) * cc + e];
  wc[t] = acc;
}

__global__ __launch_bounds__(256) void k_expand_weights_bwd(const float *__restrict__ dwc, int cc,
                                                           float *__restrict__ dw) {
  const int t = blockIdx.x * 256 + threadIdx.x;
  if (t >= 27 * cc) return;
  const int tap = t / cc, e = t - tap * cc;
  const int d0 = tap / 9 - 1, d1 = (tap / 3) % 3 - 1, d2 = tap % 3 - 1;
  float acc = 0.f;
  for (int g = 0; g < 8; ++g) {
    const int j0 = (g >> 2) & 1, j1 = (g >> 1) & 1, j2 = g & 1;
    const int i0 = j0 ? (d0 > 0) : (d0 >= 0), i1 = j1 ? (d1 > 0) : (d1 >= 0), i2 = j2 ? (d2 > 0) : (d2 >= 0);
    acc += dwc[(size_t)(g * 8 + i0 * 4 + i1 * 2 + i2) * cc + e];
  }
  dw[t] = acc;
}

SGNN_EXPORT int sgnn_expand_weights(const float *w, int cin, int cout, float *wc, sgnn_stream_t stream) {
  SGNN_CHECK_ARG(w && wc && cin >= 1 && cout >= 1);
  const int cc = cin * cout;
  SGNN_LAUNCH(k_expand_weights, dim3((64 * cc + 255) / 256), dim3(256), 0, (hipStream_t)stream, w, cc, wc);
  SGNN_CHECK_LAUNCH();
  return SGNN_OK;
}

SGNN_EXPORT int sgnn_expand_weights_bwd(const float *dwc, int cin, int cout, float *dw, sgnn_stream_t stream) {
  SGNN_CHECK_ARG(dwc && dw && cin >= 1 && cout >= 1);
  const int cc = cin * cout;
  SGNN_LAUNCH(k_expand_weights_bwd, dim3((27 * cc + 255) / 256), dim3(256), 0, (hipStream_t)stream, dwc, cc, dw);
  SGNN_CHECK_LAUNCH();
  return SGNN_OK;
}

template <int CIN, int COUT>
struct DwCfg {
  static constexpr int MT = (CIN + 15) / 16, NT = (COUT + 15) / 16;
  static constexpr int KPB = (MT * NT == 1) ? 9 : ((MT * NT <= 3) ? 5 : 3);
};

#ifndef DW_PAIR
#define DW_PAIR 1
#endif
template <int CIN, int COUT, bool EX, int KPBT = 0>
__global__ __launch_bounds__(256) void k_conv_dw(const float *__restrict__ x, int64_t n_in,
                                                const float *__restrict__ dy, const int32_t *__restrict__ table,
                                                int64_t ld, int K, int64_t n_out, float *__restrict__ partial,
                                                int64_t rows_per_block, int in_shift, ConvEx ex, int64_t ldx,
                                                int64_t ld_dy, const int64_t *n_dev) {
  if (n_dev) {
    n_out = sgnn_dyn_n(n_out, n_dev);
    const int64_t per = (n_out + gridDim.x - 1) / gridDim.x;
    rows_per_block = ((per + 255) / 256) * 256;
    if (rows_per_block < 256) rows_per_block = 256;
  }
  constexpr int MT = (CIN + 15) / 16, NT = (COUT + 15) / 16;
  constexpr int DW_KPB = KPBT > 0 ? KPBT : DwCfg<CIN, COUT>::KPB;
  constexpr int V = (CIN + 3) / 4, CINP = 4 * V;
  constexpr int W = (COUT + 3) / 4, COUTP = 4 * W;
  constexpr int XS = 64 * CINP, YS = 64 * COUTP;
  constexpr bool PAIR = DW_PAIR && MT * NT == 1 && CIN == 8 && KPBT == 0 && !EX;
  constexpr int XT = PAIR ? 2 : 1;
  constexpr int RED = DW_KPB * MT * 16 * NT * 16;
  constexpr int LDS_FLOATS = (4 * (XT * XS + YS) > RED) ? 4 * (XT * XS + YS) : RED;
  __shared__ __attribute__((aligned(16))) float lds[LDS_FLOATS];

  const int tid = threadIdx.x, lane = tid & 63, wave = tid >> 6;
  const int i16 = lane & 15, q = lane >> 4;
  const unsigned lin = sgnn_xcd_tile(blockIdx.y * gridDim.x + blockIdx.x, gridDim.x * gridDim.y);
  const unsigned bx = lin / gridDim.y, by = lin % gridDim.y;
  const unsigned groups = EX ? (unsigned)ex.groups : 1u;
  const unsigned kgroups = gridDim.y / groups;
  const unsigned grp = by / kgroups;
  const int k0 = (by % kgroups) * DW_KPB;
  const int32_t *kmap = (EX && ex.kmap) ? ex.kmap + grp * K : nullptr;
  const int table_rows = EX ? ex.table_rows : K;
  const int kc = (K - k0) < DW_KPB ? (K - k0) : DW_KPB;
  const int64_t blk_row0 = (int64_t)bx * rows_per_block;
  int64_t blk_row1 = blk_row0 + rows_per_block;
  if (blk_row1 > n_out) blk_row1 = n_out;

  const uint32_t ldx4 = (uint32_t)ldx * 4u;
  const __amdgpu_buffer_rsrc_t rs_x = make_rsrc(x, (uint32_t)(((n_in - 1) * ldx + CIN) * 4));
  const __amdgpu_buffer_rsrc_t rs_t = make_rsrc(table, (uint32_t)((int64_t)table_rows * ld * 4));
  const __amdgpu_buffer_rsrc_t rs_dy = make_rsrc(dy, (uint32_t)(((n_out * groups - 1) * ld_dy + COUT) * 4));
  const uint32_t ld4 = (uint32_t)ld * 4u;
  float *xs = lds + wave * (XT * XS + YS);
  float *ys = xs + XT * XS;

  constexpr int NP = (DW_KPB + 1) / 2;
  f32x4 accp[PAIR ? NP : 1];
#pragma unroll
  for (int p = 0; p < (PAIR ? NP : 1); ++p) accp[p] = f32x4{0.f, 0.f, 0.f, 0.f};
  f32x4 acc[DW_KPB][MT][NT];
#pragma unroll
  for (int kk = 0; kk < DW_KPB; ++kk)
#pragma unroll
    for (int mt = 0; mt < MT; ++mt)
#pragma unroll
      for (int nt = 0; nt < NT; ++nt) acc[kk][mt][nt] = f32x4{0.f, 0.f, 0.f, 0.f};

  constexpr bool RCX = (CIN == 16 || CIN == 8);
  constexpr int LPR = RCX ? CIN / 4 : 1, RPI = 64 / LPR, NI = RCX ? LPR : 4, GW = RCX ? 4 : V;
  const int rc_row = lane / LPR, rc_chunk = lane % LPR;
  auto gather = [&](int32_t iv, float(&g)[NI][GW]) {
#pragma unroll
    for (int m = 0; m < NI; ++m) {
      const int32_t id = __builtin_amdgcn_ds_bpermute((RCX ? m * RPI + rc_row : m * 16 + i16) * 4, iv);
      buf_load_floats<GW>(rs_x, (uint32_t)id * ldx4 + (uint32_t)(RCX ? rc_chunk * 16 : q * V * 4), g[m]);
    }
  };
  auto norm_rows = [&](float(&g)[NI][GW]) {
    if constexpr (CINP != CIN) {
#pragma unroll
      for (int m = 0; m < NI; ++m)
#pragma unroll
        for (int s = 0; s < GW; ++s)
          if (3 * V + s >= CIN) g[m][s] = (q == 3) ? 0.f : g[m][s];
    }
  };
  auto store_rows = [&](const float(&g)[NI][GW]) {
#pragma unroll
    for (int m = 0; m < NI; ++m) {
      float *p = RCX ? xs + (m * RPI + rc_row) * CINP + rc_chunk * 4 : xs + (m * 16 + i16) * CINP + q * V;
#pragma unroll
      for (int s = 0; s < GW; ++s) p[s] = g[m][s];
    }
  };
  auto store_rows_to = [&](const float(&g)[NI][GW], float *tile) {
#pragma unroll
    for (int m = 0; m < NI; ++m) {
      float *p = tile + (m * RPI + rc_row) * CINP + rc_chunk * 4;
#pragma unroll
      for (int s = 0; s < GW; ++s) p[s] = g[m][s];
    }
  };
  auto mma_pair = [&](int p, const float(&b)[16][NT]) {
    const float *src = xs + (i16 >> 3) * XS + (i16 & 7);
#pragma unroll
    for (int t = 0; t < 16; ++t) {
      const float a = ((i16 & 7) < CINP) ? src[(4 * t + q) * CINP] : 0.f;
      accp[p] = __builtin_amdgcn_mfma_f32_16x16x4f32(a, b[t][0], accp[p], 0, 0, 0);
    }
  };
  auto mma_chunk = [&](int kk, const float(&b)[16][NT]) {
#pragma unroll
    for (int t = 0; t < 16; ++t) {
      float a[MT];
#pragma unroll
      for (int mt = 0; mt < MT; ++mt) {
        const int ch = mt * 16 + i16;
        a[mt] = (ch < CINP) ? xs[(4 * t + q) * CINP + ch] : 0.f;
      }
#pragma unroll
      for (int mt = 0; mt < MT; ++mt)
#pragma unroll
        for (int nt = 0; nt < NT; ++nt)
          acc[kk][mt][nt] = __builtin_amdgcn_mfma_f32_16x16x4f32(a[mt], b[t][nt], acc[kk][mt][nt], 0, 0, 0);
    }
  };

  for (int64_t base = blk_row0 + wave * 64; base < blk_row1; base += 256) {
    int32_t idxv[DW_KPB];
#pragma unroll
    for (int kk = 0; kk < DW_KPB; ++kk) {
      const int ko = k0 + (kk < kc ? kk : kc - 1);
      int32_t id;
      if constexpr (EX) {
        const int trow = kmap ? kmap[ko] : ko;
        id = (int32_t)__builtin_amdgcn_raw_buffer_load_b32(rs_t, (uint32_t)(base + lane) * 4u, trow * ld4, 0);
        id = (id >> in_shift) * ex.in_mul + ((ex.kadd && id >= 0) ? ex.kadd[grp * K + ko] : 0);
      } else {
        id = (int32_t)__builtin_amdgcn_raw_buffer_load_b32(rs_t, (uint32_t)(base + lane) * 4u, ko * ld4, 0) >> in_shift;
      }
      idxv[kk] = (kk < kc) ? id : -1;
    }
    if constexpr (COUT == 16 || COUT == 8) {
      constexpr int LY = COUT / 4, RY = 64 / LY;
      const int yr = lane / LY, yc = lane % LY;
      float g[LY][4];
#pragma unroll
      for (int m = 0; m < LY; ++m) {
        const int64_t row = base + m * RY + yr;
        const uint32_t off = (row < blk_row1) ? (uint32_t)((row * groups + grp) * ld_dy + yc * 4) * 4u : 0xFFFFF800u;
        buf_load_floats<4>(rs_dy, off, g[m]);
      }
#pragma unroll
      for (int m = 0; m < LY; ++m) {
        float *p = ys + (m * RY + yr) * COUTP + yc * 4;
#pragma unroll
        for (int s = 0; s < 4; ++s) p[s] = g[m][s];
      }
    } else {
      float g[4][W];
#pragma unroll
      for (int m = 0; m < 4; ++m) {
        const int64_t row = base + m * 16 + i16;
        const uint32_t off =
            (row < blk_row1) ? (uint32_t)((row * groups + grp) * ld_dy + q * W) * 4u : 0xFFFFF800u;
        buf_load_floats<W>(rs_dy, off, g[m]);
        if constexpr (COUTP != COUT) {
#pragma unroll
          for (int s = 0; s < W; ++s)
            if (3 * W + s >= COUT) g[m][s] = (q == 3) ? 0.f : g[m][s];
        }
      }
#pragma unroll
      for (int m = 0; m < 4; ++m) {
        float *p = ys + (m * 16 + i16) * COUTP + q * W;
#pragma unroll
        for (int s = 0; s < W; ++s) p[s] = g[m][s];
      }
    }
    float b[16][NT];
#pragma unroll
    for (int t = 0; t < 16; ++t)
#pragma unroll
      for (int nt = 0; nt < NT; ++nt) {
        const int co = nt * 16 + i16;
        b[t][nt] = (co < COUTP) ? ys[(4 * t + q) * COUTP + co] : 0.f;
      }

    if constexpr (PAIR) {
      static_assert(RCX, "the paired path stores row-contiguous gathers");
      float ga[2][NI][GW], gb[2][NI][GW];
      auto idx_of = [&](int kk) { return kk < DW_KPB ? idxv[kk < DW_KPB ? kk : 0] : -1; };
      gather(idx_of(0), ga[0]);
      gather(idx_of(1), gb[0]);
#pragma unroll
      for (int p = 0; p < NP; ++p) {
        if (p + 1 < NP) {
          gather(idx_of(2 * p + 2), ga[(p + 1) & 1]);
          gather(idx_of(2 * p + 3), gb[(p + 1) & 1]);
        }
        __builtin_amdgcn_sched_barrier(0);
        store_rows_to(ga[p & 1], xs);
        store_rows_to(gb[p & 1], xs + XS);
        mma_pair(p, b);
        __builtin_amdgcn_sched_barrier(0);
      }
    } else if constexpr (MT * NT == 1) {
      float g0[NI][GW], g1[NI][GW];
      gather(idxv[0], g0);
#pragma unroll
      for (int kk = 0; kk < DW_KPB; kk += 2) {
        if (kk + 1 < DW_KPB) gather(idxv[kk + 1], g1);
        __builtin_amdgcn_sched_barrier(0);
        norm_rows(g0);
        store_rows(g0);
        mma_chunk(kk, b);
        __builtin_amdgcn_sched_barrier(0);
        if (kk + 1 < DW_KPB) {
          if (kk + 2 < DW_KPB) gather(idxv[kk + 2], g0);
          __builtin_amdgcn_sched_barrier(0);
          norm_rows(g1);
          store_rows(g1);
          mma_chunk(kk + 1, b);
          __builtin_amdgcn_sched_barrier(0);
        }
      }
    } else {
      float g0[NI][GW];
#pragma unroll
      for (int kk = 0; kk < DW_KPB; ++kk) {
        gather(idxv[kk], g0);
        norm_rows(g0);
        store_rows(g0);
        mma_chunk(kk, b);
      }
    }
  }

  __syncthreads();
  float *red = lds;
  for (int wv = 0; wv < 4; ++wv) {
    if constexpr (PAIR) {
      if (wave == wv) {
#pragma unroll
        for (int p = 0; p < NP; ++p)
#pragma unroll
          for (int i = 0; i < 4; ++i) {
            const int row = q * 4 + i, kk = 2 * p + (row >> 3), ci = row & 7, co = i16;
            if (kk < DW_KPB) {
              float *pr = &red[(kk * MT * 16 + ci) * NT * 16 + co];
              if (wv == 0)
                *pr = accp[p][i];
              else
                *pr += accp[p][i];
            }
          }
      }
    } else if (wave == wv) {
#pragma unroll
      for (int kk = 0; kk < DW_KPB; ++kk)
#pragma unroll
        for (int mt = 0; mt < MT; ++mt)
#pragma unroll
          for (int nt = 0; nt < NT; ++nt)
#pragma unroll
            for (int i = 0; i < 4; ++i) {
              const int ci = mt * 16 + q * 4 + i, co = nt * 16 + i16;
              float *p = &red[(kk * MT * 16 + ci) * NT * 16 + co];
              if (wv == 0)
                *p = acc[kk][mt][nt][i];
              else
                *p += acc[kk][mt][nt][i];
            }
    }
    __syncthreads();
  }
  float *out = partial + (((int64_t)bx * groups + grp) * K + k0) * CIN * COUT;
  for (int e = tid; e < kc * CIN * COUT; e += 256) {
    const int co = e % COUT, ci = (e / COUT) % CIN, kk = e / (CIN * COUT);
    out[e] = red[(kk * MT * 16 + ci) * NT * 16 + co];
  }
}

template <int COUT, int KP>
__global__ __launch_bounds__(256) void k_conv_dw_c1(const float *__restrict__ x, int64_t n_in, const float *__restrict__ dy,
                                                   const int32_t *__restrict__ table, int64_t ld, int K, int64_t n_out,
                                                   float *__restrict__ partial, int64_t rows_per_block, int in_shift,
                                                   int64_t ldx, int64_t ld_dy, const int64_t *n_dev) {
  static_assert(COUT % 4 == 0, "dy rows are loaded 16 bytes at a time");
  if (n_dev) {
    n_out = sgnn_dyn_n(n_out, n_dev);
    const int64_t per = (n_out + gridDim.x - 1) / gridDim.x;
    rows_per_block = ((per + 255) / 256) * 256;
    if (rows_per_block < 256) rows_per_block = 256;
  }
  constexpr int NV = KP * COUT;
  __shared__ float red[NV][65];
  const int tid = threadIdx.x, lane = tid & 63, wave = tid >> 6;
  const unsigned lin = sgnn_xcd_tile(blockIdx.y * gridDim.x + blockIdx.x, gridDim.x * gridDim.y);
  const unsigned bx = lin / gridDim.y, by = lin % gridDim.y;
  const int k0 = by * KP;
  const int kc = (K - k0) < KP ? (K - k0) : KP;
  const int64_t blk_row0 = (int64_t)bx * rows_per_block;
  int64_t blk_row1 = blk_row0 + rows_per_block;
  if (blk_row1 > n_out) blk_row1 = n_out;
  const __amdgpu_buffer_rsrc_t rs_x = make_rsrc(x, (uint32_t)(((n_in - 1) * ldx + 1) * 4));
  const __amdgpu_buffer_rsrc_t rs_t = make_rsrc(table, (uint32_t)((int64_t)K * ld * 4));
  const __amdgpu_buffer_rsrc_t rs_dy = make_rsrc(dy, (uint32_t)(((n_out - 1) * ld_dy + COUT) * 4));
  const uint32_t ld4 = (uint32_t)ld * 4u, ldx4 = (uint32_t)ldx * 4u;
  float acc[KP][COUT];
#pragma unroll
  for (int kk = 0; kk < KP; ++kk)
#pragma unroll
    for (int c = 0; c < COUT; ++c) acc[kk][c] = 0.f;
  for (int64_t row = blk_row0 + tid; row < blk_row1; row += 256) {
    int32_t id[KP];
#pragma unroll
    for (int kk = 0; kk < KP; ++kk) {
      const int ko = k0 + (kk < kc ? kk : kc - 1);
      id[kk] = (int32_t)__builtin_amdgcn_raw_buffer_load_b32(rs_t, (uint32_t)row * 4u, ko * ld4, 0) >> in_shift;
    }
    float g[COUT];
    buf_load_floats<COUT>(rs_dy, (uint32_t)(row * ld_dy) * 4u, g);
    float xv[KP];
#pragma unroll
    for (int kk = 0; kk < KP; ++kk)
      xv[kk] = __uint_as_float(__builtin_amdgcn_raw_buffer_load_b32(rs_x, (uint32_t)id[kk] * ldx4, 0, 0));
#pragma unroll
    for (int kk = 0; kk < KP; ++kk) {
      const float v = (kk < kc) ? xv[kk] : 0.f;
#pragma unroll
      for (int c = 0; c < COUT; ++c) acc[kk][c] = fmaf(v, g[c], acc[kk][c]);
    }
  }
  for (int wv = 0; wv < 4; ++wv) {
    if (wave == wv) {
#pragma unroll
      for (int kk = 0; kk < KP; ++kk)
#pragma unroll
        for (int c = 0; c < COUT; ++c) {
          float *p = &red[kk * COUT + c][lane];
          if (wv == 0)
            *p = acc[kk][c];
          else
            *p += acc[kk][c];
        }
    }
    __syncthreads();
  }
  float *out = partial + ((int64_t)bx * K + k0) * COUT;
  if (tid < kc * COUT) {
    float t = 0.f;
    for (int l = 0; l < 64; ++l) t += red[tid][l];
    out[tid] = t;
  }
}

__global__ __launch_bounds__(256) void k_dw_reduce(const float *__restrict__ partial, int64_t nblk,
                                                  int64_t elems, float *__restrict__ dw) {
  __shared__ float red[8][32];
  const int part = threadIdx.x >> 5, le = threadIdx.x & 31;
  const int64_t e = (int64_t)blockIdx.x * 32 + le;
  float s = 0.f;
  if (e < elems)
    for (int64_t b = part; b < nblk; b += 8) s += partial[b * elems + e];
  red[part][le] = s;
  __syncthreads();
  if (part == 0 && e < elems) {
    float t = 0.f;
#pragma unroll
    for (int p = 0; p < 8; ++p) t += red[p][le];
    dw[e] = t;
  }
}

__global__ __launch_bounds__(256) void k_dw_reduce_batch(DwBatch b) {
  __shared__ float red[8][32];
  int i = 0;
  while (i + 1 < b.n && (int)blockIdx.x >= b.d[i + 1].blk0) ++i;
  const DwDesc d = b.d[i];
  const int part = threadIdx.x >> 5, le = threadIdx.x & 31;
  const int64_t e = (int64_t)((int)blockIdx.x - d.blk0) * 32 + le;
  float s = 0.f;
  if (e < d.elems)
    for (int64_t k = part; k < d.nblk; k += 8) s += d.partial[k * d.elems + e];
  red[part][le] = s;
  __syncthreads();
  if (part == 0 && e < d.elems) {
    float t = 0.f;
#pragma unroll
    for (int p = 0; p < 8; ++p) t += red[p][le];
    d.dw[e] = t;
  }
}

DwBatch *sgnn_dw_batch = nullptr;

int sgnn_dw_batch_flush(DwBatch *b, hipStream_t s) {
  if (!b || b->n == 0) return SGNN_OK;
  int blocks = 0;
  for (int i = 0; i < b->n; ++i) {
    b->d[i].blk0 = blocks;
    blocks += (int)((b->d[i].elems + 31) / 32);
  }
  SGNN_LAUNCH(k_dw_reduce_batch, dim3((unsigned)blocks), dim3(256), 0, s, *b);
  b->n = 0;
  SGNN_CHECK_LAUNCH();
  return SGNN_OK;
}

__global__ __launch_bounds__(256) void k_conv_dw_generic(const float *__restrict__ x, int cin,
                                                        const float *__restrict__ dy, int cout,
                                                        const int32_t *__restrict__ table, int64_t ld, int K,
                                                        int64_t n_out, float *__restrict__ dw, int in_shift,
                                                        ConvEx ex, const int64_t *n_dev) {
  n_out = sgnn_dyn_n(n_out, n_dev);
  const int64_t e = (int64_t)blockIdx.x * 256 + threadIdx.x;
  if (e >= (int64_t)ex.groups * K * cin * cout) return;
  const int co = (int)(e % cout), ci = (int)((e / cout) % cin), k = (int)((e / ((int64_t)cin * cout)) % K);
  const int grp = (int)(e / ((int64_t)K * cin * cout));
  float s = 0.f;
  for (int64_t j = 0; j < n_out; ++j) {
    const int32_t id = table[(int64_t)(ex.kmap ? ex.kmap[grp * K + k] : k) * ld + j];
    if (id >= 0) {
      const float xv = x[((int64_t)(id >> in_shift) * ex.in_mul + (ex.kadd ? ex.kadd[grp * K + k] : 0)) * cin + ci];
      s = fmaf(xv, dy[(j * ex.groups + grp) * cout + co], s);
    }
  }
  dw[e] = s;
}

#define DW_FINE_ROWS 16384
static int64_t dw_rows_per_block(int64_t n_out) {
  int64_t rpb = (n_out + g_tune.conv_dw_blocks - 1) / g_tune.conv_dw_blocks;
  rpb = ((rpb + 255) / 256) * 256;
  if (rpb < 256) rpb = 256;
  return rpb;
}

bool dw_shape_ok(int cin, int cout) {
  static const int shapes[][2] = {{1, 8}, {8, 8}, {8, 12}, {12, 12}, {12, 16}, {16, 16}, {34, 16}, {30, 16}, {26, 16}, {48, 16},
                                  {32, 16}, {4, 16}, {16, 24}, {24, 32}, {64, 32}, {56, 28}, {32, 32}, {28, 16}};
  for (const auto &sh : shapes)
    if (sh[0] == cin && sh[1] == cout) return true;
  return false;
}

SGNN_EXPORT int64_t sgnn_conv_bwd_weight_ws_bytes(int64_t n_out, int K, int cin, int cout) {
  if (n_out <= 0) return 0;
  const int64_t rpb = dw_rows_per_block(n_out);
  const int64_t nblk = (n_out + rpb - 1) / rpb;
  return nblk * (int64_t)K * cin * cout * (int64_t)sizeof(float);
}

#define CONV_DW_CASES(X) \
  X(1, 8) X(8, 8) X(8, 12) X(12, 12) X(12, 16) X(16, 16) X(34, 16) X(30, 16) X(26, 16) X(48, 16) X(32, 16) X(4, 16) \
  X(16, 24) X(24, 32) X(64, 32) X(56, 28) X(32, 32) X(28, 16)

SGNN_EXPORT int sgnn_conv_bwd_weight_ex(const float *x, int64_t n_in, int cin, const float *dy, int cout,
                                        const int32_t *table, int64_t ld, int K, int64_t n_out, float *dw,
                                        int in_shift, const int32_t *kmap, const int32_t *kadd, int in_mul,
                                        int groups, int table_rows, void *ws, int64_t ws_bytes,
                                        sgnn_stream_t stream) {
  return sgnn_conv_bwd_weight_impl(x, n_in, cin, cin, dy, cout, cout, table, ld, K, n_out, dw, in_shift, kmap, kadd,
                                   in_mul, groups, table_rows, ws, ws_bytes, stream);
}

int sgnn_conv_bwd_weight_impl(const float *x, int64_t n_in, int cin, int64_t ldx, const float *dy, int cout, int64_t ld_dy,
                              const int32_t *table, int64_t ld, int K, int64_t n_out, float *dw, int in_shift,
                              const int32_t *kmap, const int32_t *kadd, int in_mul, int groups, int table_rows, void *ws,
                              int64_t ws_bytes, sgnn_stream_t stream, const int64_t *n_dev) {
  SGNN_CHECK_ARG(ldx >= cin && ldx <= 1024 && ld_dy >= cout && ld_dy <= 1024);
  SGNN_CHECK_ARG(cin >= 1 && cout >= 1 && K >= 1 && K <= 64 && n_out >= 0 && ld >= n_out && dw &&
                 in_shift >= 0 && in_shift < 31 && in_mul >= 1 && groups >= 1 && groups <= 64 && table_rows >= 1 &&
                 table_rows <= 64 && (kmap || table_rows >= K));
  hipStream_t s = (hipStream_t)stream;
  const int64_t elems = (int64_t)groups * K * cin * cout;
  if (n_out == 0) {
    if (sgnn_fill32(dw, 0u, elems, s) != SGNN_OK) return SGNN_EHIP;
    return SGNN_OK;
  }
  SGNN_CHECK_ARG(x && dy && table && n_in >= 1);
  SGNN_CHECK_ARG(ld % CONV_ROWS_PER_BLOCK == 0);
  if (n_in * ldx * 4 > 0xFFFFF000ll || n_out * groups * ld_dy * 4 > 0xFFFFF000ll ||
      (int64_t)table_rows * ld * 4 > 0xFFFFF000ll) {
    sgnn_set_error("sgnn_conv_bwd_weight: a slab exceeds the 4 GiB raw-buffer window");
    return SGNN_EOVERFLOW;
  }
  const ConvEx ex{kmap, kadd, in_mul, groups, table_rows};
  bool done = false;
  const int64_t rpb = dw_rows_per_block(n_out);
  const int64_t nblk = (n_out + rpb - 1) / rpb;
  const bool plain = !kmap && !kadd && in_mul == 1 && groups == 1 && table_rows == K;
#define LAUNCH_DW(CI, CO, EXV)                                                                             \
  do {                                                                                                     \
    if (!ws || ws_bytes < sgnn_conv_bwd_weight_ws_bytes(n_out, groups * K, cin, cout)) {                   \
      sgnn_set_error("sgnn_conv_bwd_weight: workspace too small");                                         \
      return SGNN_ENOWS;                                                                                   \
    }                                                                                                      \
    constexpr int kpb_ = DwCfg<CI, CO>::KPB;                                                               \
    const int prof = sgnn_prof_begin_launch(1, n_out * groups, cin, cout, K, 0, s);                        \
    if constexpr (!EXV && kpb_ == 9) {                                                                     \
       \
       \
      if (n_out < DW_FINE_ROWS && g_tune.conv_small)                                                          \
        SGNN_LAUNCH((k_conv_dw<CI, CO, false, 1>), dim3((unsigned)nblk, (unsigned)K), dim3(256), 0, s, \
                           x, n_in, dy, table, ld, K, n_out, (float *)ws, rpb, in_shift, ex, ldx, ld_dy, n_dev); \
      else                                                                                                 \
        SGNN_LAUNCH((k_conv_dw<CI, CO, false, 0>), dim3((unsigned)nblk, (unsigned)((K + kpb_ - 1) / kpb_)), \
                           dim3(256), 0, s, x, n_in, dy, table, ld, K, n_out, (float *)ws, rpb, in_shift,  \
                           ex, ldx, ld_dy, n_dev);                                                         \
    } else {                                                                                               \
      SGNN_LAUNCH((k_conv_dw<CI, CO, EXV, 0>),                                                \
                         dim3((unsigned)nblk, (unsigned)(groups * ((K + kpb_ - 1) / kpb_))), dim3(256), 0, \
                         s, x, n_in, dy, table, ld, K, n_out, (float *)ws, rpb, in_shift, ex, ldx, ld_dy, n_dev); \
    }                                                                                                      \
    sgnn_prof_end_launch(prof, s);                                                                         \
    if (sgnn_dw_batch && sgnn_dw_batch->n < DW_BATCH_MAX) {                                                \
      sgnn_dw_batch->d[sgnn_dw_batch->n++] = DwDesc{(const float *)ws, dw, nblk, elems, 0};                \
    } else {                                                                                               \
      SGNN_LAUNCH(k_dw_reduce, dim3((unsigned)((elems + 31) / 32)), dim3(256), 0, s,                \
                         (const float *)ws, nblk, elems, dw);                                              \
    }                                                                                                      \
    done = true;                                                                                           \
  } while (0)
  if (plain && cin == 1 && cout == 8 && g_tune.conv_dw_c1) {
    if (!ws || ws_bytes < sgnn_conv_bwd_weight_ws_bytes(n_out, K, cin, cout)) {
      sgnn_set_error("sgnn_conv_bwd_weight: workspace too small");
      return SGNN_ENOWS;
    }
    const int prof = sgnn_prof_begin_launch(1, n_out, cin, cout, K, 0, s);
    SGNN_LAUNCH((k_conv_dw_c1<8, 9>), dim3((unsigned)nblk, (unsigned)((K + 8) / 9)), dim3(256), 0, s, x, n_in, dy, table, ld,
                K, n_out, (float *)ws, rpb, in_shift, ldx, ld_dy, n_dev);
    sgnn_prof_end_launch(prof, s);
    if (sgnn_dw_batch && sgnn_dw_batch->n < DW_BATCH_MAX)
      sgnn_dw_batch->d[sgnn_dw_batch->n++] = DwDesc{(const float *)ws, dw, nblk, elems, 0};
    else
      SGNN_LAUNCH(k_dw_reduce, dim3((unsigned)((elems + 31) / 32)), dim3(256), 0, s, (const float *)ws, nblk, elems, dw);
    done = true;
  }
#define X(CI, CO) \
  if (!done && plain && cin == CI && cout == CO) LAUNCH_DW(CI, CO, false);
  CONV_DW_CASES(X)
#undef X
#define X(CI, CO) \
  if (!done && !plain && cin == CI && cout == CO) LAUNCH_DW(CI, CO, true);
  X(48, 16) X(24, 8) X(64, 32) X(56, 28)
#undef X
  if (!done) {
    if (ldx != cin || ld_dy != cout) {
      sgnn_set_error("sgnn_conv_bwd_weight: strided rows need one of the compiled (cin, cout) shapes, got (%d, %d)", cin, cout);
      return SGNN_EINVAL;
    }
    SGNN_LAUNCH(k_conv_dw_generic, dim3((unsigned)((elems + 255) / 256)), dim3(256), 0, s, x, cin, dy,
                       cout, table, ld, K, n_out, dw, in_shift, ex, n_dev);
  }
  SGNN_CHECK_LAUNCH();
  return SGNN_OK;
}

SGNN_EXPORT int sgnn_conv_bwd_weight(const float *x, int64_t n_in, int cin, const float *dy, int cout,
                                     const int32_t *table, int64_t ld, int K, int64_t n_out, float *dw,
                                     int in_shift, void *ws, int64_t ws_bytes, sgnn_stream_t stream) {
  return sgnn_conv_bwd_weight_ex(x, n_in, cin, dy, cout, table, ld, K, n_out, dw, in_shift, nullptr, nullptr, 1, 1,
                                 K, ws, ws_bytes, stream);
}
```

sgnn_amd/csrc/prog.hip:

```cpp
#include <mutex>
#include <vector>
#include "common.h"

enum {
  OP_CONV_SUBM = 0, OP_CONV_DOWN = 1, OP_UNPOOL = 2, OP_BN = 3, OP_ADD = 4, OP_JOIN = 5,
  OP_CONCAT_IN = 6,
  OP_EXPAND = 7,
  OP_LINEAR = 8
};
#define OPW 12
#define EXPAND_DX_SPLIT 4

extern "C" int sgnn_expand_weights(const float *w, int cin, int cout, float *wc, sgnn_stream_t stream);
extern "C" int sgnn_expand_weights_bwd(const float *dwc, int cin, int cout, float *dw, sgnn_stream_t stream);
int64_t sgnn_bf16_wfrag_bytes(int cin, int cout, int K, int groups);
int sgnn_bf16_conv_prepare(const float *w, int cin, int cout, int K, int groups, void *wf, sgnn_stream_t stream);
int sgnn_bf16_conv_run(const void *x, int64_t n_in, int cin, int64_t ldx, const float *w, const void *wf, int K,
                       const int32_t *table, int64_t ld, int64_t n_out, int cout, void *y, int64_t ldy,
                       const void *addend, int64_t ld_add, const int32_t *kmap, int groups, int table_rows,
                       const int64_t *n_dev, sgnn_stream_t stream);
int sgnn_bf16_conv_expand_impl(const void *x, int64_t n, int cin, int64_t ldx, const float *w, const int32_t *nbr,
                               int64_t ld, int cout, void *y, int64_t ldy, const int64_t *n_dev, void *ws,
                               sgnn_stream_t stream);
int sgnn_bf16_linear_rows(const void *x, int64_t ldx, int64_t n, int cin, const float *const *w, const float *const *b,
                          int cout, float *y, const int64_t *n_dev, sgnn_stream_t stream);

namespace {

struct Op {
  int32_t type, in0, in1, out, par, lev, cin, cout, in2, ia, ib, ic;
  bool is_conv() const { return type == OP_CONV_SUBM || type == OP_CONV_DOWN; }
  int K() const { return type == OP_CONV_DOWN ? 8 : 27; }
  int out_class() const { return type == OP_CONV_DOWN ? lev + 1 : lev; }
  template <class F>
  void for_inputs(F f) const {
    f(in0);
    if (type == OP_ADD || type == OP_JOIN || type == OP_CONCAT_IN) f(in1);
    if (type == OP_CONCAT_IN) f(in2);
  }
};
static_assert(sizeof(Op) == sizeof(int32_t[OPW]), "Op mirrors one record of the caller's int32 array");

struct View {
  const int32_t *ops;
  const float *opf;
  int nops;
  const int32_t *bufs;
  int nbuf, n_ext;
  const int64_t *lev_n, *lev_ld;
  void *const *lev_nbr, *const *lev_children, *const *lev_ptable, *const *lev_parent;
  int nlev;
  const Op &op(int i) const { return reinterpret_cast<const Op *>(ops)[i]; }
};

enum Kind { TRAINING, INFERENCE, INFERENCE_BF16 };

Kind kind_of_mode(int mode) { return mode == 3 ? INFERENCE_BF16 : mode == 2 ? INFERENCE : TRAINING; }

inline int64_t round64(int64_t v) { return (v + 63) & ~int64_t(63); }

struct ConvSetup {
  bool ok = false;
  int K = 0, cnt_class = 0;
  int64_t n = 0, n_out = 0;
  const int32_t *tab_f = nullptr, *tab_b = nullptr;
  int64_t ld_f = 0, ld_b = 0;
  int flags_b = 0;
  ConvSetup(const View &v, const Op &o) {
    const bool down = o.type == OP_CONV_DOWN;
    K = o.K();
    cnt_class = o.out_class();
    ok = o.lev >= 0 && cnt_class < v.nlev;
    if (!ok) return;
    n = v.lev_n[o.lev];
    n_out = v.lev_n[cnt_class];
    if (!v.lev_ld) return;
    tab_f = (const int32_t *)(down ? v.lev_children[o.lev] : v.lev_nbr[o.lev]);
    ld_f = v.lev_ld[cnt_class];
    tab_b = (const int32_t *)(down ? v.lev_ptable[o.lev] : v.lev_nbr[o.lev]);
    ld_b = v.lev_ld[o.lev];
    flags_b = down ? SGNN_CONV_TRANSPOSE_W : (SGNN_CONV_TRANSPOSE_W | SGNN_CONV_FLIP_K);
  }
};

std::vector<int> count_readers(const View &v) {
  std::vector<int> r(v.nbuf, 0);
  for (int i = 0; i < v.nops; ++i)
    v.op(i).for_inputs([&](int b) {
      if (b >= 0 && b < v.nbuf) ++r[b];
    });
  return r;
}

#define g_fuse (g_tune.prog_fusion != 0)
#define g_lin_add (g_tune.prog_lin_add != 0)
#define g_lin_bn (g_tune.prog_lin_bn != 0)
struct Plan {
  std::vector<int> add_dst;
  std::vector<int> add_src;
  std::vector<char> skip;
  std::vector<int> root, col;
  std::vector<int64_t> ld;
  std::vector<char> join_view;
  std::vector<int> lin_bn;
  Kind kind = TRAINING;
  std::vector<char> f32;
  bool bf16() const { return kind == INFERENCE_BF16; }
};

inline int64_t round8(int64_t v) { return (v + 7) & ~int64_t(7); }

bool strided_conv_ok(const Op &o) {
  return sgnn_conv_epi_supported(o.cin, o.cout) && sgnn_conv_epi_supported(o.cout, o.cin) && dw_shape_ok(o.cin, o.cout);
}

void make_plan(const View &v, const int32_t *keep, Plan &P, Kind kind) {
  P.kind = kind;
  P.f32.assign(v.nbuf, P.bf16() ? 0 : 1);
  if (P.bf16())
    for (int i = 0; i < v.nops; ++i)
      if (v.op(i).type == OP_LINEAR && v.op(i).out >= 0 && v.op(i).out < v.nbuf) P.f32[v.op(i).out] = 1;
  auto row_ld = [&](int r) -> int64_t { return P.f32[r] ? v.bufs[2 * r + 1] : round8(v.bufs[2 * r + 1]); };
  P.add_dst.assign(v.nops, -1);
  P.add_src.assign(v.nops, -1);
  P.skip.assign(v.nops, 0);
  P.join_view.assign(v.nops, 0);
  P.lin_bn.assign(v.nops, -1);
  P.root.resize(v.nbuf);
  P.col.assign(v.nbuf, 0);
  P.ld.resize(v.nbuf);
  for (int b = 0; b < v.nbuf; ++b) {
    P.root[b] = b;
    P.ld[b] = row_ld(b);
  }
  if (!g_fuse) return;
  std::vector<int> readers = count_readers(v);
  if (keep)
    for (int b = 0; b < v.nbuf; ++b)
      if (keep[b]) ++readers[b];
  if (g_lin_bn)
    for (int i = 0; i < v.nops; ++i) {
      const Op &o = v.op(i);
      if (o.type != OP_LINEAR || o.cout > 2 || readers[o.in0] != 1) continue;
      for (int j = 0; j < i; ++j) {
        const Op &b = v.op(j);
        if (b.type == OP_BN && b.out == o.in0 && b.lev == o.lev) P.lin_bn[i] = j;
      }
    }
  for (int i = 0; i + 1 < v.nops; ++i) {
    const Op &o = v.op(i), &a = v.op(i + 1);
    if (!o.is_conv() || a.type != OP_ADD) continue;
    if (!sgnn_conv_epi_supported(o.cin, o.cout) || ConvSetup(v, o).n_out <= 0 || readers[o.out] != 1) continue;
    if ((a.in0 != o.out && a.in1 != o.out) || a.in0 == a.in1) continue;
    P.add_dst[i] = a.out;
    P.add_src[i] = a.in0 == o.out ? a.in1 : a.in0;
    P.skip[i + 1] = 1;
  }
  std::vector<int> prod(v.nbuf, -1), last_reader(v.nbuf, -1);
  std::vector<char> strided_ok(v.nbuf, 1);
  for (int i = 0; i < v.nops; ++i) {
    const Op &o = v.op(i);
    if (!P.skip[i]) prod[P.add_dst[i] >= 0 ? P.add_dst[i] : o.out] = i;
    auto reads = [&](int b, bool ok) {
      if (b < 0) return;
      last_reader[b] = i;
      if (!ok) strided_ok[b] = 0;
    };
    auto join_read = [&](int b) { return last_reader[b] >= 0 && v.op(last_reader[b]).type == OP_JOIN; };
    switch (o.type) {
      case OP_CONV_SUBM:
      case OP_CONV_DOWN: reads(o.in0, strided_conv_ok(o)); break;
      case OP_BN:
      case OP_UNPOOL: reads(o.in0, true); break;
      case OP_JOIN:
        reads(o.in0, !join_read(o.in0));
        reads(o.in1, !join_read(o.in1));
        break;
      case OP_ADD: reads(o.in0, P.skip[i] != 0); reads(o.in1, P.skip[i] != 0); break;
      default: o.for_inputs([&](int b) { reads(b, false); }); break;
    }
  }
  for (int i = 0; i < v.nops; ++i) {
    const Op &o = v.op(i);
    if (o.type != OP_JOIN || v.lev_n[o.lev] <= 0) continue;
    bool ok = true;
    for (int side = 0; side < 2 && ok; ++side) {
      const int q = side ? o.in1 : o.in0;
      ok = q >= v.n_ext && !(keep && keep[q]) && P.root[q] == q && strided_ok[q] && last_reader[q] == i && prod[q] >= 0;
      if (!ok) break;
      const Op &p = v.op(prod[q]);
      ok = (p.is_conv() && strided_conv_ok(p)) || p.type == OP_BN || p.type == OP_UNPOOL;
    }
    if (!ok || o.in0 == o.in1) continue;
    if (P.bf16() && (o.cin & 1)) continue;
    P.join_view[i] = 1;
    P.skip[i] = 1;
    P.root[o.in0] = o.out;
    P.col[o.in0] = 0;
    P.root[o.in1] = o.out;
    P.col[o.in1] = o.cin;
  }
  for (int b = 0; b < v.nbuf; ++b) {
    int r = b, c = 0;
    while (P.root[r] != r) {
      c += P.col[r];
      r = P.root[r];
    }
    P.root[b] = r;
    P.col[b] = c;
    P.ld[b] = row_ld(r);
  }
}

struct Layout {
  std::vector<int64_t> buf_off, buf_floats, aux_off;
  int64_t max_buf = 0, total = 0, fwd_total = 0, scratch0 = 0, scratch1 = 0, bextra = 0;
  std::vector<char> shadow;
  std::vector<int> first;
};

int64_t aux_floats(const Op &o, Kind kind) {
  const int64_t slices = round64(64 * (int64_t)o.cin * o.cout);
  if (kind == INFERENCE_BF16) {
    if (o.is_conv()) return round64(sgnn_bf16_wfrag_bytes(o.cin, o.cout, o.K(), 1) / 4);
    return o.type == OP_EXPAND ? slices + round64(sgnn_bf16_wfrag_bytes(o.cin, o.cout, 8, 8) / 4) : 0;
  }
  return o.type == OP_BN ? round64(2 * (int64_t)o.cin) : o.type == OP_EXPAND ? slices : 0;
}

int64_t place_aux(const View &v, Kind kind, Layout &L, int64_t off) {
  for (int i = 0; i < v.nops; ++i) {
    const int64_t a = aux_floats(v.op(i), kind);
    if (a <= 0) continue;
    L.aux_off[i] = off;
    off += a;
  }
  return off;
}

int make_layout_infer(const View &v, const Plan &P, const int32_t *keep, Layout &L) {
  const int never = v.nops + 1;
  std::vector<int> first(v.nbuf, never), last(v.nbuf, -1);
  auto in_arena = [&](int b) { return b >= v.n_ext || L.shadow[b]; };
  for (int i = 0; i < v.nops; ++i) {
    auto touch = [&](int b) {
      if (b < 0 || b >= v.nbuf || !in_arena(b)) return;
      const int r = P.root[b];
      if (i < first[r]) first[r] = i;
      if (i > last[r]) last[r] = i;
    };
    v.op(i).for_inputs(touch);
    touch(P.add_dst[i] >= 0 ? P.add_dst[i] : v.op(i).out);
  }
  for (int b = v.n_ext; b < v.nbuf; ++b)
    if (keep && keep[b]) last[P.root[b]] = never;
  std::vector<std::pair<int64_t, int64_t>> free_list;
  int64_t top = place_aux(v, P.kind, L, 0);
  auto release = [&](int64_t o, int64_t n) {
    if (n <= 0) return;
    size_t k = 0;
    while (k < free_list.size() && free_list[k].first < o) ++k;
    free_list.insert(free_list.begin() + k, std::make_pair(o, n));
    if (k + 1 < free_list.size() && free_list[k].first + free_list[k].second == free_list[k + 1].first) {
      free_list[k].second += free_list[k + 1].second;
      free_list.erase(free_list.begin() + k + 1);
    }
    if (k > 0 && free_list[k - 1].first + free_list[k - 1].second == free_list[k].first) {
      free_list[k - 1].second += free_list[k].second;
      free_list.erase(free_list.begin() + k);
    }
  };
  auto take = [&](int64_t n) -> int64_t {
    if (n <= 0) return 0;
    size_t best = free_list.size();
    for (size_t k = 0; k < free_list.size(); ++k)
      if (free_list[k].second >= n && (best == free_list.size() || free_list[k].second < free_list[best].second)) best = k;
    if (best < free_list.size()) {
      const int64_t o = free_list[best].first;
      free_list[best].first += n;
      free_list[best].second -= n;
      if (free_list[best].second == 0) free_list.erase(free_list.begin() + best);
      return o;
    }
    if (!free_list.empty() && free_list.back().first + free_list.back().second == top) {
      const int64_t o = free_list.back().first;
      free_list.pop_back();
      top = o + n;
      return o;
    }
    const int64_t o = top;
    top += n;
    return o;
  };
  for (int i = 0; i < v.nops; ++i) {
    for (int b = 0; b < v.nbuf; ++b)
      if (in_arena(b) && P.root[b] == b && L.buf_off[b] >= 0 && last[b] == i - 1) release(L.buf_off[b], round64(L.buf_floats[b]));
    for (int b = 0; b < v.nbuf; ++b)
      if (in_arena(b) && P.root[b] == b && first[b] == i) L.buf_off[b] = take(round64(L.buf_floats[b]));
  }
  for (int b = v.n_ext; b < v.nbuf; ++b) {
    if (P.root[b] == b && L.buf_off[b] < 0) L.buf_off[b] = 0;
  }
  for (int b = v.n_ext; b < v.nbuf; ++b)
    if (P.root[b] != b) L.buf_off[b] = P.bf16() ? L.buf_off[P.root[b]] : L.buf_off[P.root[b]] + P.col[b];
  L.first = first;
  L.fwd_total = L.total = top;
  L.scratch0 = L.scratch1 = L.bextra = top;
  return 0;
}

int make_layout(const View &v, const Plan &P, Layout &L, const int32_t *keep) {
  L.buf_off.assign(v.nbuf, -1);
  L.buf_floats.resize(v.nbuf);
  L.aux_off.assign(v.nops, -1);
  L.shadow.assign(v.nbuf, 0);
  for (int b = 0; b < v.nbuf; ++b) {
    const int lev = v.bufs[2 * b], ch = v.bufs[2 * b + 1];
    if (lev < 0 || lev >= v.nlev || ch < 1) return -1;
    const int64_t elems = v.lev_n[lev] * (int64_t)(P.root[b] == b ? P.ld[b] : ch);
    L.buf_floats[b] = P.f32[b] ? elems : (elems + 1) / 2;
    if (L.buf_floats[b] > L.max_buf) L.max_buf = L.buf_floats[b];
  }
  if (P.kind != TRAINING) {
    if (P.bf16())
      for (int i = 0; i < v.nops; ++i) {
        if (v.op(i).type == OP_CONCAT_IN) continue;
        v.op(i).for_inputs([&](int b) {
          if (b >= 0 && b < v.n_ext) L.shadow[b] = 1;
        });
      }
    return make_layout_infer(v, P, keep, L);
  }
  int64_t off = 0;
  for (int b = v.n_ext; b < v.nbuf; ++b) {
    if (P.root[b] != b) continue;
    L.buf_off[b] = off;
    off += round64(L.buf_floats[b]);
  }
  for (int b = v.n_ext; b < v.nbuf; ++b)
    if (P.root[b] != b) L.buf_off[b] = L.buf_off[P.root[b]] + P.col[b];
  off = place_aux(v, TRAINING, L, off);
  int64_t bextra = 0;
  for (int i = 0; i < v.nops; ++i) {
    const Op &o = v.op(i);
    if (o.type != OP_EXPAND) continue;
    const int64_t need = aux_floats(o, TRAINING) + round64(v.lev_n[o.lev] * EXPAND_DX_SPLIT * (int64_t)o.cin);
    if (need > bextra) bextra = need;
  }
  L.fwd_total = off;
  L.scratch0 = off;
  off += round64(L.max_buf);
  L.scratch1 = off;
  off += round64(L.max_buf);
  L.bextra = off;
  off += bextra;
  L.total = off;
  return 0;
}

inline int64_t expand_dwc_bytes(int cin, int cout) { return (64 * (int64_t)cin * cout * 4 + 255) & ~int64_t(255); }

int64_t dw_slice(const View &v, int i) {
  const Op &o = v.op(i);
  int64_t w = 0;
  if (o.is_conv()) w = sgnn_conv_bwd_weight_ws_bytes(ConvSetup(v, o).n_out, o.K(), o.cin, o.cout);
  if (o.type == OP_EXPAND)
    w = ((sgnn_conv_bwd_weight_ws_bytes(v.lev_n[o.lev], 64, o.cin, o.cout) + 255) & ~int64_t(255)) + expand_dwc_bytes(o.cin, o.cout);
  return (w + 255) & ~int64_t(255);
}

int64_t dw_ws_need(const View &v) {
  int64_t need = 0;
  for (int i = 0; i < v.nops; ++i) need += dw_slice(v, i);
  return need;
}

int64_t ws_main(const View &v) {
  int64_t need = 0;
  for (int i = 0; i < v.nops; ++i) {
    const Op &o = v.op(i);
    int64_t w = 0;
    if (o.type == OP_BN) w = sgnn_bn_ws_bytes(v.lev_n[o.lev], o.cin);
    if (o.type == OP_LINEAR) w = sgnn_linear_ws_bytes(v.lev_n[o.lev], o.cin, o.cout);
    if (w > need) need = w;
  }
  const int64_t dw = dw_ws_need(v);
  if (dw > need) need = dw;
  return (need + 255) & ~int64_t(255);
}

int64_t ws_stats(const View &v) {
  int64_t need = 0;
  for (int i = 0; i < v.nops; ++i) {
    const Op &o = v.op(i);
    if (!o.is_conv()) continue;
    const ConvSetup cs(v, o);
    const int64_t a = ((cs.n_out > 0 ? cs.n_out : 1) + 15) / 16 * 2 * o.cout * (int64_t)sizeof(double);
    const int64_t b = ((cs.n > 0 ? cs.n : 1) + 15) / 16 * 2 * o.cin * (int64_t)sizeof(double);
    if (a > need) need = a;
    if (b > need) need = b;
  }
  return (need + 255) & ~int64_t(255);
}

int64_t ws_need(const View &v) { return ws_main(v) + ws_stats(v); }

struct SideLane {
  hipStream_t stream = nullptr;
  void *ws = nullptr;
  int64_t ws_bytes = 0;
  hipEvent_t fork = nullptr, join = nullptr;
} g_side;
std::mutex g_side_mu;
bool g_defer_join = false;

#define PROG_TRY(call)           \
  do {                           \
    const int rc_ = (call);      \
    if (rc_ != SGNN_OK) return rc_; \
  } while (0)

struct Ctx {
  View v;
  void *const *params, *const *idx, *const *lev_cnt;
  int nparams, nidx, training;
  void *ws;
  int64_t ws_bytes;
  sgnn_stream_t stream;
  Plan P;
  Layout L;
  std::vector<const double *> pre;
  std::vector<int64_t> pre_nblk;
  double *stats_ws;

  bool prepare(Kind kind, const int32_t *keep) {
    make_plan(v, keep, P, kind);
    if (make_layout(v, P, L, keep) != 0) return false;
    pre = std::vector<const double *>(v.nops, nullptr);
    pre_nblk = std::vector<int64_t>(v.nops, 0);
    stats_ws = (double *)((char *)ws + ws_main(v));
    return true;
  }
  int ch(int b) const { return b < 0 ? 0 : v.bufs[2 * b + 1]; }
  int cls(int b) const { return v.bufs[2 * b]; }
  int64_t rows(int b) const { return v.lev_n[cls(b)]; }
  int64_t ld(int b) const { return P.ld[b]; }
  float *param(int p) const { return (p >= 0 && p < nparams) ? (float *)params[p] : nullptr; }
  const int32_t *index(int i) const { return (i >= 0 && i < nidx && idx) ? (const int32_t *)idx[i] : nullptr; }
  const int64_t *count(int c) const { return (lev_cnt && c >= 0 && c < v.nlev) ? (const int64_t *)lev_cnt[c] : nullptr; }
  int wait_once(void *&wait_event) const {
    if (!wait_event) return SGNN_OK;
    sgnn_stamp("down-wait<", stream);
    SGNN_HIP_TRY(hipStreamWaitEvent((hipStream_t)stream, (hipEvent_t)wait_event, 0));
    sgnn_stamp("down-wait>", stream);
    wait_event = nullptr;
    return SGNN_OK;
  }
};

}

SGNN_EXPORT int sgnn_prog_set_side_stream(sgnn_stream_t stream2, void *ws2, int64_t ws2_bytes) {
  std::lock_guard<std::mutex> hold(g_side_mu);
  if (stream2 && !g_side.fork) {
    SGNN_HIP_TRY(hipEventCreateWithFlags(&g_side.fork, hipEventDisableTiming));
    SGNN_HIP_TRY(hipEventCreateWithFlags(&g_side.join, hipEventDisableTiming));
  }
  g_side.stream = (hipStream_t)stream2;
  g_side.ws = stream2 ? ws2 : nullptr;
  g_side.ws_bytes = stream2 ? ws2_bytes : 0;
  return SGNN_OK;
}

SGNN_EXPORT int sgnn_prog_defer_join(int on) {
  const int prev = g_defer_join ? 1 : 0;
  g_defer_join = on != 0;
  return prev;
}

SGNN_EXPORT int64_t sgnn_prog_arena_floats(const int32_t *ops, int nops, const int32_t *bufs, int nbuf, int n_ext,
                                           const int64_t *lev_n, int nlev, const int32_t *keep, int mode) {
  View v{ops, nullptr, nops, bufs, nbuf, n_ext, lev_n, nullptr, nullptr, nullptr, nullptr, nullptr, nlev};
  if (mode < 0 || mode > 3) return -1;
  Plan P;
  make_plan(v, keep, P, kind_of_mode(mode));
  Layout L;
  if (make_layout(v, P, L, keep) != 0) return -1;
  return mode == 0 ? L.total : L.fwd_total;
}

SGNN_EXPORT int64_t sgnn_prog_ws_bytes(const int32_t *ops, int nops, const int64_t *lev_n, int nlev) {
  View v{ops, nullptr, nops, nullptr, 0, 0, lev_n, nullptr, nullptr, nullptr, nullptr, nullptr, nlev};
  return ws_need(v);
}

SGNN_EXPORT int64_t sgnn_prog_buffer_offset(const int32_t *ops, int nops, const int32_t *bufs, int nbuf, int n_ext,
                                            const int64_t *lev_n, int nlev, const int32_t *keep, int infer, int b) {
  View v{ops, nullptr, nops, bufs, nbuf, n_ext, lev_n, nullptr, nullptr, nullptr, nullptr, nullptr, nlev};
  if (infer < 0 || infer > 2) return -1;
  const Kind kind = infer == 2 ? INFERENCE_BF16 : infer == 1 ? INFERENCE : TRAINING;
  Plan P;
  make_plan(v, keep, P, kind);
  Layout L;
  if (make_layout(v, P, L, keep) != 0 || b < 0 || b >= nbuf) return -1;
  if (b < n_ext) return L.shadow[b] ? L.buf_off[b] : -1;
  return P.root[b] == b ? L.buf_off[b] : -1;
}

SGNN_EXPORT int sgnn_prog_plan(const int32_t *ops, int nops, const int32_t *bufs, int nbuf, int n_ext, const int64_t *lev_n,
                               int nlev, const int32_t *keep, int mode, int32_t *out) {
  SGNN_CHECK_ARG(ops && bufs && lev_n && out && nops >= 0 && nbuf >= 1 && nlev >= 1 && n_ext >= 0 && n_ext <= nbuf &&
                 mode >= 0 && mode <= 3);
  View v{ops, nullptr, nops, bufs, nbuf, n_ext, lev_n, nullptr, nullptr, nullptr, nullptr, nullptr, nlev};
  Plan P;
  make_plan(v, keep, P, kind_of_mode(mode));
  for (int i = 0; i < nops; ++i) {
    out[4 * i] = P.skip[i];
    out[4 * i + 1] = P.add_dst[i];
    out[4 * i + 2] = P.join_view[i];
    out[4 * i + 3] = P.lin_bn[i];
  }
  for (int b = 0; b < nbuf; ++b) {
    out[4 * nops + 3 * b] = P.root[b];
    out[4 * nops + 3 * b + 1] = P.col[b];
    out[4 * nops + 3 * b + 2] = (int32_t)P.ld[b];
  }
  return SGNN_OK;
}

static int forward_bf16(const Ctx &c, void *const *ext, float *arena, void *wait_event) {
  const View &v = c.v;
  const Plan &PL = c.P;
  const Layout &L = c.L;
  const sgnn_stream_t stream = c.stream;
  const int n_ext = v.n_ext, nbuf = v.nbuf, nlev = v.nlev;
  auto B = [&](int b) -> void * {
    if (b < 0) return nullptr;
    if (b < n_ext && !L.shadow[b]) return ext[b];
    const int r = PL.root[b];
    return (char *)arena + 4 * L.buf_off[r] + (PL.f32[r] ? 4 : 2) * (int64_t)PL.col[b];
  };
  auto EXT = [&](int b) -> const float * { return b < 0 ? nullptr : (const float *)ext[b]; };
  for (int i = 0; i < v.nops; ++i) {
    const Op &o = v.op(i);
    const int in0 = o.in0, in1 = o.in1, out = o.out, par = o.par, lev = o.lev, cin = o.cin, cout = o.cout;
    SGNN_CHECK_ARG(out >= n_ext && out < nbuf && lev >= 0 && lev < nlev && in0 < nbuf && in1 < nbuf);
    SGNN_CHECK_ARG(o.type == OP_CONCAT_IN || in0 >= 0);
    SGNN_CHECK_ARG(o.type == OP_LINEAR || !PL.f32[out]);
    const int64_t n = v.lev_n[lev];
    for (int b = 0; b < n_ext; ++b)
      if (L.shadow[b] && L.first[b] == i)
        PROG_TRY(sgnn_bf16_concat3(EXT(b), c.ch(b), nullptr, nullptr, 0, nullptr, nullptr, 0, nullptr, c.rows(b), B(b), c.ld(b),
                                   c.count(c.cls(b)), stream));
    if (PL.skip[i]) continue;
    if (o.type == OP_CONV_DOWN) PROG_TRY(c.wait_once(wait_event));
    switch (o.type) {
      case OP_CONV_SUBM:
      case OP_CONV_DOWN: {
        const ConvSetup cs(v, o);
        SGNN_CHECK_ARG(cs.ok);
        int dst = out;
        const void *addend = nullptr;
        int64_t ld_add = 0;
        if (PL.add_dst[i] >= 0) {
          addend = B(PL.add_src[i]);
          ld_add = c.ld(PL.add_src[i]);
          dst = PL.add_dst[i];
        }
        void *wf = arena + L.aux_off[i];
        PROG_TRY(sgnn_bf16_conv_prepare(c.param(par), cin, cout, cs.K, 1, wf, stream));
        PROG_TRY(sgnn_bf16_conv_run(B(in0), c.rows(in0), cin, c.ld(in0), c.param(par), wf, cs.K, cs.tab_f, cs.ld_f, cs.n_out, cout,
                                    B(dst), c.ld(dst), addend, ld_add, nullptr, 1, cs.K, c.count(cs.cnt_class), stream));
        break;
      }
      case OP_UNPOOL:
        SGNN_CHECK_ARG(lev + 1 < nlev);
        PROG_TRY(sgnn_bf16_gather_rows(B(in0), c.ld(in0), cin, (const int32_t *)v.lev_parent[lev], n, B(out), c.ld(out),
                                       c.count(lev), stream));
        break;
      case OP_BN:
        PROG_TRY(sgnn_bf16_bn_eval(B(in0), c.ld(in0), n, cin, c.param(par), c.param(par + 1), c.param(par + 2), c.param(par + 3),
                                   v.opf[4 * i], v.opf[4 * i + 2], B(out), c.ld(out), c.count(lev), stream));
        break;
      case OP_ADD:
        SGNN_CHECK_ARG(in1 >= 0);
        PROG_TRY(sgnn_bf16_add(B(in0), c.ld(in0), B(in1), c.ld(in1), n, cin, B(out), c.ld(out), c.count(lev), stream));
        break;
      case OP_JOIN:
        SGNN_CHECK_ARG(in1 >= 0);
        PROG_TRY(sgnn_bf16_join(B(in0), c.ld(in0), cin, B(in1), c.ld(in1), cout, n, B(out), c.ld(out), c.count(lev), stream));
        break;
      case OP_CONCAT_IN: {
        const int in2 = o.in2;
        SGNN_CHECK_ARG(in2 < nbuf && in0 < n_ext && in1 < n_ext && in2 < n_ext && c.ch(in0) + c.ch(in1) + c.ch(in2) == c.ch(out));
        PROG_TRY(sgnn_bf16_concat3(EXT(in0), c.ch(in0), c.index(o.ia), EXT(in1), c.ch(in1), c.index(o.ib), EXT(in2), c.ch(in2),
                                   c.index(o.ic), n, B(out), c.ld(out), c.count(lev), stream));
        break;
      }
      case OP_EXPAND:
        SGNN_CHECK_ARG(c.rows(out) == 8 * n);
        PROG_TRY(sgnn_bf16_conv_expand_impl(B(in0), n, cin, c.ld(in0), c.param(par), (const int32_t *)v.lev_nbr[lev], v.lev_ld[lev],
                                            cout, B(out), c.ld(out), c.count(lev), arena + L.aux_off[i], stream));
        break;
      case OP_LINEAR: {
        SGNN_CHECK_ARG(cout >= 1 && cout <= 4 && PL.f32[out] && c.ld(out) == cout);
        const float *w[4] = {}, *b[4] = {};
        for (int q = 0; q < cout; ++q) {
          w[q] = c.param(par + 2 * q);
          b[q] = c.param(par + 2 * q + 1);
        }
        PROG_TRY(sgnn_bf16_linear_rows(B(in0), c.ld(in0), n, cin, w, b, cout, (float *)B(out), c.count(lev), stream));
        break;
      }
      default:
        sgnn_set_error("sgnn_prog_forward: unknown op %d", o.type);
        return SGNN_EINVAL;
    }
  }
  return SGNN_OK;
}

SGNN_EXPORT int sgnn_prog_forward(const int32_t *ops, const float *opf, int nops, const int32_t *bufs, int nbuf, int n_ext,
                                  const int64_t *lev_n, const int64_t *lev_ld, void *const *lev_nbr,
                                  void *const *lev_children, void *const *lev_ptable, void *const *lev_parent,
                                  void *const *lev_cnt, int nlev, void *const *params, int nparams,
                                  void *const *ext, void *const *idx,
                                  int nidx, float *arena, int64_t arena_floats, const int32_t *keep, int training,
                                  void *wait_event, void *ws, int64_t ws_bytes, sgnn_stream_t stream) {
  SGNN_CHECK_ARG(ops && opf && bufs && lev_n && lev_ld && params && arena && nops >= 0 && nbuf >= 1 && nlev >= 1 &&
                 n_ext >= 0 && n_ext <= nbuf && (n_ext == 0 || ext));
  const Kind kind = (training & 4) ? INFERENCE_BF16 : (training & 2) ? INFERENCE : TRAINING;
  if ((training & 4) && (training & 3) != 2) {
    sgnn_set_error("sgnn_prog_forward: bf16 storage needs the inference layout in eval mode (training = 2 | 4)");
    return SGNN_EINVAL;
  }
  training &= 1;
  Ctx c{View{ops, opf, nops, bufs, nbuf, n_ext, lev_n, lev_ld, lev_nbr, lev_children, lev_ptable, lev_parent, nlev},
        params, idx, lev_cnt, nparams, nidx, training, ws, ws_bytes, stream};
  SGNN_CHECK_ARG(c.prepare(kind, keep));
  const View &v = c.v;
  const Plan &PL = c.P;
  const Layout &L = c.L;
  if (arena_floats < L.fwd_total) {
    sgnn_set_error("sgnn_prog_forward: arena too small (%lld < %lld floats)", (long long)arena_floats,
                   (long long)L.fwd_total);
    return SGNN_ENOWS;
  }
  if (ws_bytes < ws_need(v)) {
    sgnn_set_error("sgnn_prog_forward: workspace too small");
    return SGNN_ENOWS;
  }
  if (kind == INFERENCE_BF16) return forward_bf16(c, ext, arena, wait_event);
  auto B = [&](int b) -> float * { return b < 0 ? nullptr : (b < n_ext ? (float *)ext[b] : arena + L.buf_off[b]); };
  for (int i = 0; i < nops; ++i) {
    const Op &o = v.op(i);
    const int in0 = o.in0, in1 = o.in1, out = o.out, par = o.par, lev = o.lev, cin = o.cin, cout = o.cout;
    SGNN_CHECK_ARG(out >= n_ext && out < nbuf && lev >= 0 && lev < nlev && in0 < nbuf && in1 < nbuf);
    SGNN_CHECK_ARG(o.type == OP_CONCAT_IN || in0 >= 0);
    const int64_t n = lev_n[lev];
    if (PL.skip[i]) continue;
    if (o.type == OP_CONV_DOWN) PROG_TRY(c.wait_once(wait_event));
    switch (o.type) {
      case OP_CONV_SUBM:
      case OP_CONV_DOWN: {
        const ConvSetup cs(v, o);
        SGNN_CHECK_ARG(cs.ok);
        ConvEpi epi{};
        int dst_buf = out;
        if (PL.add_dst[i] >= 0) {
          epi.addend = B(PL.add_src[i]);
          epi.ld_add = c.ld(PL.add_src[i]);
          dst_buf = PL.add_dst[i];
        }
        const int j = i + 1 + (PL.add_dst[i] >= 0 ? 1 : 0);
        if (g_fuse && training && cs.n_out > 0 && j < nops && v.op(j).type == OP_BN && v.op(j).in0 == dst_buf &&
            sgnn_conv_epi_supported(cin, cout)) {
          epi.stats = 1;
          epi.partial = c.stats_ws;
          c.pre[j] = c.stats_ws;
          c.pre_nblk[j] = sgnn_conv_grid_blocks(cs.n_out, cin, cout, cs.K);
        }
        epi.ldx = c.ld(in0);
        epi.ldy = c.ld(dst_buf);
        epi.n_dev = c.count(cs.cnt_class);
        PROG_TRY(sgnn_conv_fwd_impl(B(in0), n, cin, c.param(par), cs.K, cs.tab_f, cs.ld_f, cs.n_out, cout, B(dst_buf), 0, 0,
                                    nullptr, nullptr, 1, 1, cs.K, &epi, stream));
        break;
      }
      case OP_UNPOOL:
        SGNN_CHECK_ARG(lev + 1 < nlev);
        PROG_TRY(sgnn_gather_rows_ld(B(in0), c.ld(in0), cin, (const int32_t *)lev_parent[lev], n, B(out), c.ld(out), stream,
                                     c.count(lev)));
        break;
      case OP_BN: {
        float *save = arena + L.aux_off[i];
        PROG_TRY(sgnn_bn_fwd_impl(B(in0), c.ld(in0), n, cin, c.param(par), c.param(par + 1), c.param(par + 2), c.param(par + 3),
                                  opf[4 * i], opf[4 * i + 1], training, opf[4 * i + 2], save, save + cin, B(out), c.ld(out),
                                  c.pre[i], c.pre_nblk[i], ws, ws_bytes, stream, c.count(lev)));
        break;
      }
      case OP_ADD:
        SGNN_CHECK_ARG(in1 >= 0);
        PROG_TRY(sgnn_add_ld(B(in0), c.ld(in0), B(in1), c.ld(in1), n, cin, B(out), c.ld(out), stream, c.count(lev)));
        break;
      case OP_JOIN:
        SGNN_CHECK_ARG(in1 >= 0 && c.ld(in0) == cin && c.ld(in1) == cout && c.ld(out) == cin + cout);
        PROG_TRY(sgnn_concat_rows_dn(B(in0), cin, nullptr, B(in1), cout, nullptr, n, B(out), stream, c.count(lev)));
        break;
      case OP_CONCAT_IN: {
        const int in2 = o.in2;
        SGNN_CHECK_ARG(in2 < nbuf && c.ch(in0) + c.ch(in1) + c.ch(in2) == c.ch(out) && c.ld(out) == c.ch(out));
        PROG_TRY(sgnn_concat3_rows_dn(B(in0), c.ch(in0), c.index(o.ia), B(in1), c.ch(in1), c.index(o.ib), B(in2), c.ch(in2),
                                      c.index(o.ic), n, B(out), stream, c.count(lev)));
        break;
      }
      case OP_EXPAND: {
        SGNN_CHECK_ARG(c.rows(out) == 8 * n && c.ld(in0) == cin && c.ld(out) == cout);
        const int32_t *S, *ST, *PAR;
        PROG_TRY(sgnn_expand_maps(&S, &ST, &PAR));
        float *wc = arena + L.aux_off[i];
        PROG_TRY(sgnn_expand_weights(c.param(par), cin, cout, wc, stream));
        ConvEpi xepi{};
        xepi.n_dev = c.count(lev);
        PROG_TRY(sgnn_conv_fwd_impl(B(in0), n, cin, wc, 8, (const int32_t *)lev_nbr[lev], lev_ld[lev], n, cout, B(out), 0,
                                    0, S, nullptr, 1, 8, 27, &xepi, stream));
        break;
      }
      case OP_LINEAR: {
        SGNN_CHECK_ARG(cout >= 1 && cout <= 4 && c.ld(in0) == cin);
        const float *w[4] = {}, *b[4] = {};
        for (int q = 0; q < cout; ++q) {
          w[q] = c.param(par + 2 * q);
          b[q] = c.param(par + 2 * q + 1);
        }
        PROG_TRY(sgnn_linear_fwd_rows(B(in0), n, cin, w, b, cout, B(out), stream, c.count(lev)));
        break;
      }
      default:
        sgnn_set_error("sgnn_prog_forward: unknown op %d", o.type);
        return SGNN_EINVAL;
    }
  }
  return SGNN_OK;
}

namespace {

struct Grads {
  enum State : char { NONE, HELD, ALIAS, CALLER };
  const Ctx &c;
  void *const *pgrads, *const *ext, *const *gext, *const *gout;
  const float *arena;
  float *garena;
  std::vector<State> state;
  std::vector<int> alias;
  std::vector<int> lazy_lin;
  std::vector<char> viewed;
  float *scratch[2];

  Grads(const Ctx &c_, void *const *pgrads_, void *const *ext_, void *const *gext_, void *const *gout_, const float *arena_,
        float *garena_)
      : c(c_), pgrads(pgrads_), ext(ext_), gext(gext_), gout(gout_), arena(arena_), garena(garena_),
        state(c_.v.nbuf, NONE), alias(c_.v.nbuf, -1), lazy_lin(c_.v.nbuf, -1), viewed(c_.v.nbuf, 0),
        scratch{garena_ + c_.L.scratch0, garena_ + c_.L.scratch1} {
    for (int b = 0; b < c.v.nbuf; ++b)
      if (c.P.root[b] != b) viewed[b] = viewed[c.P.root[b]] = 1;
  }
  const float *X(int b) const { return b < 0 ? nullptr : (b < c.v.n_ext ? (const float *)ext[b] : arena + c.L.buf_off[b]); }
  float *G(int b) const { return b < c.v.n_ext ? (float *)gext[b] : garena + c.L.buf_off[b]; }
  float *PG(int p) const { return (p >= 0 && p < c.nparams) ? (float *)pgrads[p] : nullptr; }
  bool wants(int b) const { return b >= c.v.n_ext || gext[b] != nullptr; }
  bool has(int b) const { return state[b] != NONE; }
  const float *held(int b) const { return state[b] == CALLER ? (const float *)gout[b] : G(b); }
  int64_t held_ld(int b) const { return state[b] == CALLER ? (int64_t)c.ch(b) : c.ld(b); }
  const float *read(int b) const { return state[b] == ALIAS ? held(alias[b]) : held(b); }
  int64_t read_ld(int b) const { return state[b] == ALIAS ? held_ld(alias[b]) : held_ld(b); }
  void written(int b) {
    state[b] = HELD;
    alias[b] = -1;
  }
  float *target(int b, int which) const { return state[b] == HELD ? scratch[which] : G(b); }
  int64_t target_ld(int b, const float *t) const { return t == G(b) ? c.ld(b) : c.ch(b); }
  int commit(int b, float *wrote) {
    const int64_t n = c.rows(b);
    const int ch = c.ch(b);
    const int64_t *cnt = c.count(c.cls(b));
    if (wrote != G(b)) return sgnn_add_ld(G(b), c.ld(b), wrote, ch, n, ch, G(b), c.ld(b), c.stream, cnt);
    if (state[b] == ALIAS || state[b] == CALLER) {
      const float *other = read(b);
      const int64_t ldo = read_ld(b);
      written(b);
      return sgnn_add_ld(G(b), c.ld(b), other, ldo, n, ch, G(b), c.ld(b), c.stream, cnt);
    }
    written(b);
    return SGNN_OK;
  }
  int adopt_outputs() {
    for (int b = c.v.n_ext; b < c.v.nbuf; ++b) {
      if (!gout[b]) continue;
      if (viewed[b] || !g_fuse) {
        if (c.L.buf_floats[b] > 0) PROG_TRY(sgnn_copy_words(G(b), gout[b], c.L.buf_floats[b], (hipStream_t)c.stream));
        state[b] = HELD;
      } else {
        state[b] = CALLER;
      }
    }
    return SGNN_OK;
  }
  int finish_externals() {
    for (int b = 0; b < c.v.n_ext; ++b) {
      if (!gext[b] || c.L.buf_floats[b] == 0) continue;
      if (state[b] == ALIAS)
        PROG_TRY(sgnn_copy_words(G(b), read(b), c.L.buf_floats[b], (hipStream_t)c.stream));
      else if (state[b] == NONE)
        PROG_TRY(sgnn_fill32(G(b), 0u, c.L.buf_floats[b], (hipStream_t)c.stream));
    }
    return SGNN_OK;
  }
};

struct Lane {
  struct PendingExpand { const float *dwc; int cin, cout; float *dw; };
  std::unique_lock<std::mutex> lock;
  hipStream_t hs;
  bool side, forked = false;
  char *ws;
  int64_t off = 0;
  DwBatch batch{};
  std::vector<PendingExpand> pending_expand;

  Lane(const Ctx &c, hipStream_t hs_) : lock(g_side_mu, std::try_to_lock), hs(hs_) {
    side = lock.owns_lock() && g_side.stream && g_side.stream != hs && g_side.ws && g_side.ws_bytes >= dw_ws_need(c.v);
    ws = (char *)(side ? g_side.ws : c.ws);
    sgnn_dw_batch = side ? &batch : nullptr;
  }
  ~Lane() { sgnn_dw_batch = nullptr; }
  hipStream_t stream() const { return side ? g_side.stream : hs; }
  hipStream_t fork() {
    if (!side) return hs;
    (void)hipEventRecord(g_side.fork, hs);
    (void)hipStreamWaitEvent(g_side.stream, g_side.fork, 0);
    forked = true;
    return g_side.stream;
  }
  int finish() {
    PROG_TRY(sgnn_dw_batch_flush(&batch, stream()));
    for (const PendingExpand &pe : pending_expand)
      PROG_TRY(sgnn_expand_weights_bwd(pe.dwc, pe.cin, pe.cout, pe.dw, (sgnn_stream_t)stream()));
    if (forked && !g_defer_join) {
      SGNN_HIP_TRY(hipEventRecord(g_side.join, g_side.stream));
      SGNN_HIP_TRY(hipStreamWaitEvent(hs, g_side.join, 0));
    }
    return SGNN_OK;
  }
};

int bwd_unreached(const Ctx &c, const Grads &g, const Op &o) {
  const hipStream_t hs = (hipStream_t)c.stream;
  if (o.is_conv() || o.type == OP_EXPAND) PROG_TRY(sgnn_fill32(g.PG(o.par), 0u, (int64_t)o.K() * o.cin * o.cout, hs));
  if (o.type == OP_BN) {
    void *zp[2] = {g.PG(o.par), g.PG(o.par + 1)};
    const int64_t zw[2] = {o.cin, o.cin};
    PROG_TRY(sgnn_fill32_multi(zp, zw, 2, 0u, hs));
  }
  if (o.type == OP_LINEAR)
    for (int q = 0; q < o.cout; ++q) {
      void *zp[2] = {g.PG(o.par + 2 * q), g.PG(o.par + 2 * q + 1)};
      const int64_t zw[2] = {o.cin, 1};
      PROG_TRY(sgnn_fill32_multi(zp, zw, 2, 0u, hs));
    }
  return SGNN_OK;
}

int bwd_conv(Ctx &c, Grads &g, Lane &lane, int i) {
  const Op &o = c.v.op(i);
  const ConvSetup cs(c.v, o);
  SGNN_CHECK_ARG(cs.ok);
  const int in0 = o.in0, cin = o.cin, cout = o.cout;
  const float *dy = g.read(o.out);
  const int64_t ld_dy = g.read_ld(o.out);
  const hipStream_t ls = lane.fork();
  if (g.wants(in0)) {
    if (g_fuse && sgnn_conv_epi_supported(cout, cin) && cs.n > 0) {
      ConvEpi epi{};
      if (g.has(in0)) {
        epi.addend = g.read(in0);
        epi.ld_add = g.read_ld(in0);
      }
      if (i > 0 && c.v.op(i - 1).type == OP_BN && c.v.op(i - 1).out == in0 && c.v.op(i - 1).cin == cin) {
        const Op &bo = c.v.op(i - 1);
        const float *save = g.arena + c.L.aux_off[i - 1];
        epi.stats = 2;
        epi.partial = c.stats_ws;
        epi.bn_x = g.X(bo.in0);
        epi.ld_bnx = c.ld(bo.in0);
        epi.mean = save;
        epi.invstd = save + cin;
        epi.gamma = c.param(bo.par);
        epi.beta = c.param(bo.par + 1);
        epi.leak = c.v.opf[4 * (i - 1) + 2];
        c.pre[i - 1] = c.stats_ws;
        c.pre_nblk[i - 1] = sgnn_conv_grid_blocks(cs.n, cout, cin, cs.K);
      }
      epi.ldx = ld_dy;
      epi.ldy = c.ld(in0);
      epi.n_dev = c.count(o.lev);
      PROG_TRY(sgnn_conv_fwd_impl(dy, cs.n_out, cout, c.param(o.par), cs.K, cs.tab_b, cs.ld_b, cs.n, cin, g.G(in0), cs.flags_b, 0,
                                  nullptr, nullptr, 1, 1, cs.K, &epi, c.stream));
      g.written(in0);
    } else {
      SGNN_CHECK_ARG(ld_dy == cout);
      float *t = g.target(in0, 0);
      ConvEpi pepi{};
      pepi.n_dev = c.count(o.lev);
      PROG_TRY(sgnn_conv_fwd_impl(dy, cs.n_out, cout, c.param(o.par), cs.K, cs.tab_b, cs.ld_b, cs.n, cin, t, cs.flags_b, 0, nullptr,
                                  nullptr, 1, 1, cs.K, &pepi, c.stream));
      PROG_TRY(g.commit(in0, t));
    }
  }
  const int64_t slice = dw_slice(c.v, i);
  PROG_TRY(sgnn_conv_bwd_weight_impl(g.X(in0), cs.n, cin, c.ld(in0), dy, cout, ld_dy, cs.tab_f, cs.ld_f, cs.K, cs.n_out,
                                     g.PG(o.par), 0, nullptr, nullptr, 1, 1, cs.K, lane.ws + lane.off, slice, (sgnn_stream_t)ls,
                                     c.count(cs.cnt_class)));
  if (ls != lane.hs) sgnn_stamp("dw>", (sgnn_stream_t)ls);
  lane.off += slice;
  return SGNN_OK;
}

int bwd_unpool(Ctx &c, Grads &g, Lane &, int i) {
  const Op &o = c.v.op(i);
  if (!g.wants(o.in0)) return SGNN_OK;
  float *t = g.target(o.in0, 0);
  PROG_TRY(sgnn_gather_sum_ld(g.read(o.out), g.read_ld(o.out), o.cin, (const int32_t *)c.v.lev_children[o.lev],
                              c.v.lev_ld[o.lev + 1], 8, c.v.lev_n[o.lev + 1], t, g.target_ld(o.in0, t), c.stream,
                              c.count(o.lev + 1)));
  return g.commit(o.in0, t);
}

int bwd_bn(Ctx &c, Grads &g, Lane &, int i) {
  const Op &o = c.v.op(i);
  const int in0 = o.in0, cin = o.cin;
  const float *save = g.arena + c.L.aux_off[i];
  const float *addend = nullptr;
  int64_t ld_add = cin;
  if (g.wants(in0) && g.has(in0)) {
    addend = g.read(in0);
    ld_add = g.read_ld(in0);
  }
  float *t = g.wants(in0) ? g.G(in0) : g.scratch[0];
  BnLin bl{};
  const bool lazy = g.lazy_lin[o.out] >= 0;
  if (lazy) {
    const Op &lo = c.v.op(g.lazy_lin[o.out]);
    bl.g = g.read(lo.out);
    bl.ldg = g.read_ld(lo.out);
    bl.nout = lo.cout;
    for (int q = 0; q < lo.cout; ++q) bl.w[q] = c.param(lo.par + 2 * q);
  }
  PROG_TRY(sgnn_bn_bwd_impl(g.X(in0), c.ld(in0), lazy ? nullptr : g.read(o.out), g.read_ld(o.out), c.v.lev_n[o.lev], cin,
                            c.param(o.par), c.param(o.par + 1), save, save + cin, c.training, c.v.opf[4 * i + 2], addend, ld_add,
                            t, g.wants(in0) ? c.ld(in0) : cin, g.PG(o.par), g.PG(o.par + 1), c.pre[i], c.pre_nblk[i], c.ws,
                            c.ws_bytes, c.stream, c.count(o.lev), lazy ? &bl : nullptr));
  if (g.wants(in0)) g.written(in0);
  return SGNN_OK;
}

int bwd_add(Ctx &c, Grads &g, Lane &, int i) {
  const Op &o = c.v.op(i);
  const int64_t n = c.v.lev_n[o.lev];
  const float *dy = g.read(o.out);
  const int64_t ld_dy = g.read_ld(o.out);
  const int src = g.state[o.out] == Grads::ALIAS ? g.alias[o.out] : o.out;
  for (int b : {o.in0, o.in1}) {
    if (!g.wants(b)) continue;
    if (g.state[b] == Grads::HELD) {
      PROG_TRY(sgnn_add_ld(g.G(b), c.ld(b), dy, ld_dy, n, o.cin, g.G(b), c.ld(b), c.stream, c.count(o.lev)));
    } else if (g.has(b)) {
      PROG_TRY(sgnn_add_ld(g.read(b), g.read_ld(b), dy, ld_dy, n, o.cin, g.G(b), c.ld(b), c.stream, c.count(o.lev)));
      g.written(b);
    } else {
      g.state[b] = Grads::ALIAS;
      g.alias[b] = src;
    }
  }
  return SGNN_OK;
}

int bwd_join(Ctx &c, Grads &g, Lane &, int i) {
  const Op &o = c.v.op(i);
  const int in0 = o.in0, in1 = o.in1;
  if (c.P.join_view[i]) {
    if (g.state[o.out] != Grads::HELD || g.has(in0) || g.has(in1)) {
      sgnn_set_error("sgnn_prog_backward: in-place JoinTable met an unexpected gradient state");
      return SGNN_EINVAL;
    }
    g.written(in0);
    g.written(in1);
    return SGNN_OK;
  }
  const int64_t n = c.v.lev_n[o.lev];
  SGNN_CHECK_ARG(g.read_ld(o.out) == o.cin + o.cout && c.ld(in0) == o.cin && c.ld(in1) == o.cout);
  float *ta = g.wants(in0) ? g.target(in0, 0) : nullptr;
  float *tb = g.wants(in1) ? g.target(in1, 1) : nullptr;
  PROG_TRY(sgnn_concat_rows_bwd_dn(g.read(o.out), o.cin, nullptr, o.cout, nullptr, n, ta, n, tb, n, c.stream, c.count(o.lev)));
  if (ta) PROG_TRY(g.commit(in0, ta));
  if (tb) PROG_TRY(g.commit(in1, tb));
  return SGNN_OK;
}

int bwd_concat_in(Ctx &c, Grads &g, Lane &, int i) {
  const Op &o = c.v.op(i);
  const int src[3] = {o.in0, o.in1, o.in2};
  float *d[3] = {nullptr, nullptr, nullptr};
  for (int q = 0; q < 3; ++q)
    if (src[q] >= 0 && g.wants(src[q])) {
      if (g.has(src[q])) {
        sgnn_set_error("sgnn_prog_backward: a CONCAT_IN source already carries a gradient (unsupported)");
        return SGNN_EINVAL;
      }
      d[q] = g.G(src[q]);
      g.written(src[q]);
    }
  SGNN_CHECK_ARG(g.read_ld(o.out) == c.ch(o.out));
  return sgnn_concat3_rows_bwd_dn(g.read(o.out), c.ch(o.in0), c.index(o.ia), c.ch(o.in1), c.index(o.ib), c.ch(o.in2),
                                  c.index(o.ic), c.v.lev_n[o.lev], d[0], o.in0 >= 0 ? c.rows(o.in0) : 0, d[1],
                                  o.in1 >= 0 ? c.rows(o.in1) : 0, d[2], o.in2 >= 0 ? c.rows(o.in2) : 0, c.stream, c.count(o.lev));
}

int bwd_expand(Ctx &c, Grads &g, Lane &lane, int i) {
  const Op &o = c.v.op(i);
  const int in0 = o.in0, cin = o.cin, cout = o.cout;
  const int64_t n = c.v.lev_n[o.lev], ld_nbr = c.v.lev_ld[o.lev], slice = dw_slice(c.v, i);
  const float *dy = g.read(o.out);
  const int32_t *S, *ST, *PAR;
  PROG_TRY(sgnn_expand_maps(&S, &ST, &PAR));
  const float *wc = g.arena + c.L.aux_off[i];
  const int32_t *nbr = (const int32_t *)c.v.lev_nbr[o.lev];
  float *dwc = lane.side ? (float *)(lane.ws + lane.off + slice - expand_dwc_bytes(cin, cout)) : g.garena + c.L.bextra;
  float *part = g.garena + c.L.bextra + round64(64 * (int64_t)cin * cout);
  const hipStream_t ls = lane.fork();
  SGNN_CHECK_ARG(g.read_ld(o.out) == cout && c.ld(in0) == cin);
  if (g.wants(in0) && n > 0) {
    const int Gs = EXPAND_DX_SPLIT;
    ConvEpi xepi{};
    xepi.n_dev = c.count(o.lev);
    PROG_TRY(sgnn_conv_fwd_impl(dy, 8 * n, cout, wc, 64 / Gs, nbr, ld_nbr, n, cin, part, SGNN_CONV_TRANSPOSE_W, 0, ST, PAR, 8,
                                Gs, 27, &xepi, c.stream));
    float *t = g.target(in0, 0);
    PROG_TRY(sgnn_sum_groups_dn(part, cin, n, Gs, t, c.stream, c.count(o.lev)));
    PROG_TRY(g.commit(in0, t));
  }
  PROG_TRY(sgnn_conv_bwd_weight_impl(g.X(in0), n, cin, cin, dy, cout, cout, nbr, ld_nbr, 8, n, dwc, 0, S, nullptr, 1, 8, 27,
                                     lane.ws + lane.off, slice, (sgnn_stream_t)ls, c.count(o.lev)));
  lane.off += slice;
  lane.pending_expand.push_back(Lane::PendingExpand{dwc, cin, cout, g.PG(o.par)});
  return SGNN_OK;
}

int bwd_linear(Ctx &c, Grads &g, Lane &, int i) {
  const Op &o = c.v.op(i);
  const int in0 = o.in0, cin = o.cin, cout = o.cout;
  const int64_t n = c.v.lev_n[o.lev];
  const float *dy = g.read(o.out);
  const float *w[4] = {};
  float *dw[4] = {}, *db[4] = {};
  for (int q = 0; q < cout; ++q) {
    w[q] = c.param(o.par + 2 * q);
    dw[q] = g.PG(o.par + 2 * q);
    db[q] = g.PG(o.par + 2 * q + 1);
  }
  SGNN_CHECK_ARG(g.read_ld(o.out) == cout && c.ld(in0) == cin);
  if (c.P.lin_bn[i] >= 0 && g.wants(in0) && !g.has(in0) && n > 0 && !c.pre[c.P.lin_bn[i]]) {
    PROG_TRY(sgnn_linear_bwd_rows(g.X(in0), dy, n, cin, w, cout, nullptr, dw, db, c.ws, c.ws_bytes, c.stream, c.count(o.lev)));
    g.lazy_lin[in0] = i;
    return SGNN_OK;
  }
// ... 61 lines not shown
```

sgnn_amd/csrc/tune.hip:

```cpp
#include <string.h>
#include "common.h"

sgnn_tune g_tune = {
     1,
     160 * 256,
     1,
     1,
     1,
     256,
     1,
     1,
     1,
     1,
     1,
     1,
     1,
     1,
};

namespace {
struct Field {
  const char *name;
  int64_t sgnn_tune::*ptr;
  int64_t lo, hi;
  bool boolean;
};
const Field kFields[] = {
    {"conv_small", &sgnn_tune::conv_small, 0, 1, true},
    {"conv_small_rows", &sgnn_tune::conv_small_rows, 0, (int64_t)1 << 36, false},
    {"conv_unrolled", &sgnn_tune::conv_unrolled, 0, 1, true},
    {"conv_one_round", &sgnn_tune::conv_one_round, 0, 1, true},
    {"conv_wide_epi", &sgnn_tune::conv_wide_epi, 0, 1, true},
    {"conv_dw_blocks", &sgnn_tune::conv_dw_blocks, 1, 4096, false},
    {"conv_dw_c1", &sgnn_tune::conv_dw_c1, 0, 1, true},
    {"rulebook_multi", &sgnn_tune::rulebook_multi, 0, 1, true},
    {"scan_inline", &sgnn_tune::scan_inline, 0, 1, true},
    {"chain_merged", &sgnn_tune::chain_merged, 0, 1, true},
    {"prog_fusion", &sgnn_tune::prog_fusion, 0, 1, true},
    {"prog_lin_bn", &sgnn_tune::prog_lin_bn, 0, 1, true},
    {"prog_lin_add", &sgnn_tune::prog_lin_add, 0, 1, true},
    {"bn_fuse", &sgnn_tune::bn_fuse, 0, 1, true},
};
const Field *find(const char *name) {
  if (!name) return nullptr;
  for (const Field &f : kFields)
    if (strcmp(f.name, name) == 0) return &f;
  return nullptr;
}
}

SGNN_EXPORT int64_t sgnn_tune_get(const char *name) {
  const Field *f = find(name);
  if (!f) {
    sgnn_set_error("sgnn_tune_get: no switch named '%s' (sgnn_tune_names lists them)", name ? name : "(null)");
    return SGNN_TUNE_UNKNOWN;
  }
  return g_tune.*(f->ptr);
}

SGNN_EXPORT int64_t sgnn_tune_set(const char *name, int64_t value) {
  const Field *f = find(name);
  if (!f) {
    sgnn_set_error("sgnn_tune_set: no switch named '%s' (sgnn_tune_names lists them)", name ? name : "(null)");
    return SGNN_TUNE_UNKNOWN;
  }
  const int64_t prev = g_tune.*(f->ptr);
  if (f->boolean) value = value != 0;
  if (value < f->lo || value > f->hi) {
    sgnn_set_error("sgnn_tune_set: %s = %lld is outside [%lld, %lld]", name, (long long)value, (long long)f->lo, (long long)f->hi);
    return SGNN_TUNE_UNKNOWN;
  }
  g_tune.*(f->ptr) = value;
  return prev;
}

SGNN_EXPORT const char *sgnn_tune_names(void) {
  static char buf[512];
  if (!buf[0]) {
    size_t n = 0;
    for (const Field &f : kFields) n += (size_t)snprintf(buf + n, sizeof(buf) - n, "%s%s", n ? "," : "", f.name);
  }
  return buf;
}

SGNN_EXPORT const sgnn_tune *sgnn_tune_current(void) { return &g_tune; }
```

Baseline: 5717.

## Fold training BatchNorm+activation into the following small sparse convolution

Adds a planner pass that finds a BatchNorm whose only reader is the next small submanifold convolution. It skips the standalone BN kernel and applies the normalisation and leaky activation on the fly in the conv's input load, forward and weight-gradient. The conv kernel reduces the producer's statistics partials itself, issuing the loads early and finishing them after the gathers, and block 0 writes the saved and running stats. This removes one kernel launch and a full write and read of the normalised activation per folded layer. In exchange every conv block repeats the stats reduction, a second stats workspace is needed, and the weight-gradient path recomputes BN on the fly.

New measurement: 5793 (median of 6 runs). 1.01x the previous value.

```diff
diff --git a/include/sgnn_hip.h b/include/sgnn_hip.h
--- a/include/sgnn_hip.h
+++ b/include/sgnn_hip.h
@@ -53,6 +53,7 @@
   int64_t prog_lin_bn;
   int64_t prog_lin_add;
   int64_t bn_fuse;
+  int64_t prog_bn_fold_small;
 } sgnn_tune;
 int64_t sgnn_tune_set(const char *name, int64_t value);
 int64_t sgnn_tune_get(const char *name);
diff --git a/sgnn_amd/csrc/bn.hip b/sgnn_amd/csrc/bn.hip
--- a/sgnn_amd/csrc/bn.hip
+++ b/sgnn_amd/csrc/bn.hip
@@ -1,12 +1,11 @@
 #include "common.h"
+#include "bn_fuse.h"
 
 #define BN_MAX_BLOCKS 2048
 #define BN_FLUSH 2
 #ifndef BN_U
 #define BN_U 2
 #endif
-#define BN_FUSE_BLOCKS 4096
-#define BN_FUSE_MAXC 64
 
 struct BnGeom {
   int vec;
@@ -255,76 +254,6 @@
   }
 }
 
-
-struct BnFuse {
-  const double *partial;
-  int nblk;
-  float eps, momentum;
-  float *running_mean, *running_var, *save_mean, *save_invstd;
-  float *dgamma, *dbeta;
-};
-
-#ifndef BN_TOTALS_WIDE
-#define BN_TOTALS_WIDE 1
-#endif
-typedef double f64x2 __attribute__((ext_vector_type(2)));
-__device__ __forceinline__ void bn_fuse_totals(const BnFuse &f, int c, double *scratch, double *tot) {
-  const int tid = threadIdx.x;
-  const int tpc = 256 / c;
-  if (BN_TOTALS_WIDE && (c & 1) == 0 && (((uintptr_t)f.partial) & 15) == 0) {
-    const int hp = c >> 1;
-    const int p2 = tid % hp, which = (tid / hp) & 1, part = tid / c;
-    f64x2 acc = {0.0, 0.0};
-    if (part < tpc) {
-      constexpr int U = 32;
-      for (int blk = part; blk < f.nblk; blk += U * tpc) {
-        f64x2 v[U];
-#pragma unroll
-        for (int u = 0; u < U; ++u) {
-          const int bi = blk + u * tpc;
-          v[u] = bi < f.nblk ? *reinterpret_cast<const f64x2 *>(f.partial + ((size_t)bi * 2 + which) * c + 2 * p2) : f64x2{0.0, 0.0};
-        }
-#pragma unroll
-        for (int u = 0; u < U; ++u) acc += v[u];
-      }
-      scratch[which * 256 + part * c + 2 * p2] = acc[0];
-      scratch[which * 256 + part * c + 2 * p2 + 1] = acc[1];
-    }
-  } else {
-    const int ch = tid % c, part = tid / c;
-    double a = 0.0, b = 0.0;
-    if (part < tpc) {
-      for (int blk = part; blk < f.nblk; blk += 8 * tpc) {
-        double va[8], vb[8];
-#pragma unroll
-        for (int u = 0; u < 8; ++u) {
-          const int bi = blk + u * tpc;
-          const bool ok = bi < f.nblk;
-          va[u] = ok ? f.partial[((size_t)bi * 2 + 0) * c + ch] : 0.0;
-          vb[u] = ok ? f.partial[((size_t)bi * 2 + 1) * c + ch] : 0.0;
-        }
-#pragma unroll
-        for (int u = 0; u < 8; ++u) {
-          a += va[u];
-          b += vb[u];
-        }
-      }
-      scratch[part * c + ch] = a;
-      scratch[256 + part * c + ch] = b;
-    }
-  }
-  __syncthreads();
-  if (tid < c) {
-    double s1 = 0.0, s2 = 0.0;
-    for (int p = 0; p < tpc; ++p) {
-      s1 += scratch[p * c + tid];
-      s2 += scratch[256 + p * c + tid];
-    }
-    tot[tid] = s1;
-    tot[c + tid] = s2;
-  }
-  __syncthreads();
-}
 
 template <int VEC, bool FUSE>
 __global__ __launch_bounds__(256) void k_bn_apply(const float *__restrict__ x, int64_t ldx, int64_t n, int c, int cq,
@@ -501,10 +430,6 @@
   }
 }
 
-static bool bn_fuse_ok(int64_t nblk, int c, int apply_grid) {
-  return c <= BN_FUSE_MAXC && nblk <= BN_FUSE_BLOCKS && nblk * (int64_t)apply_grid * 2 * c * (int64_t)sizeof(double) <= (48ll << 20);
-}
-
 static int bn_apply_grid(int64_t n, const BnGeom &g) {
   int64_t b = (n + (int64_t)g.rpb * BN_U - 1) / ((int64_t)g.rpb * BN_U);
   if (b < 1) b = 1;
diff --git a/sgnn_amd/csrc/bn_fuse.h b/sgnn_amd/csrc/bn_fuse.h
--- /dev/null
+++ b/sgnn_amd/csrc/bn_fuse.h
@@ -0,0 +1,140 @@
+#pragma once
+#include "common.h"
+
+#define BN_FUSE_BLOCKS 4096
+#define BN_FUSE_MAXC 64
+
+
+struct BnFuse {
+  const double *partial;
+  int nblk;
+  float eps, momentum;
+  float *running_mean, *running_var, *save_mean, *save_invstd;
+  float *dgamma, *dbeta;
+};
+
+#ifndef BN_TOTALS_WIDE
+#define BN_TOTALS_WIDE 1
+#endif
+typedef double f64x2 __attribute__((ext_vector_type(2)));
+__device__ __forceinline__ void bn_fuse_totals(const BnFuse &f, int c, double *scratch, double *tot) {
+  const int tid = threadIdx.x;
+  const int tpc = 256 / c;
+  if (BN_TOTALS_WIDE && (c & 1) == 0 && (((uintptr_t)f.partial) & 15) == 0) {
+    const int hp = c >> 1;
+    const int p2 = tid % hp, which = (tid / hp) & 1, part = tid / c;
+    f64x2 acc = {0.0, 0.0};
+    if (part < tpc) {
+      constexpr int U = 32;
+      for (int blk = part; blk < f.nblk; blk += U * tpc) {
+        f64x2 v[U];
+#pragma unroll
+        for (int u = 0; u < U; ++u) {
+          const int bi = blk + u * tpc;
+          v[u] = bi < f.nblk ? *reinterpret_cast<const f64x2 *>(f.partial + ((size_t)bi * 2 + which) * c + 2 * p2) : f64x2{0.0, 0.0};
+        }
+#pragma unroll
+        for (int u = 0; u < U; ++u) acc += v[u];
+      }
+      scratch[which * 256 + part * c + 2 * p2] = acc[0];
+      scratch[which * 256 + part * c + 2 * p2 + 1] = acc[1];
+    }
+  } else {
+    const int ch = tid % c, part = tid / c;
+    double a = 0.0, b = 0.0;
+    if (part < tpc) {
+      for (int blk = part; blk < f.nblk; blk += 8 * tpc) {
+        double va[8], vb[8];
+#pragma unroll
+        for (int u = 0; u < 8; ++u) {
+          const int bi = blk + u * tpc;
+          const bool ok = bi < f.nblk;
+          va[u] = ok ? f.partial[((size_t)bi * 2 + 0) * c + ch] : 0.0;
+          vb[u] = ok ? f.partial[((size_t)bi * 2 + 1) * c + ch] : 0.0;
+        }
+#pragma unroll
+        for (int u = 0; u < 8; ++u) {
+          a += va[u];
+          b += vb[u];
+        }
+      }
+      scratch[part * c + ch] = a;
+      scratch[256 + part * c + ch] = b;
+    }
+  }
+  __syncthreads();
+  if (tid < c) {
+    double s1 = 0.0, s2 = 0.0;
+    for (int p = 0; p < tpc; ++p) {
+      s1 += scratch[p * c + tid];
+      s2 += scratch[256 + p * c + tid];
+    }
+    tot[tid] = s1;
+    tot[c + tid] = s2;
+  }
+  __syncthreads();
+}
+
+#define BN_TOTALS_EARLY 16
+template <int C>
+struct BnTotalsEarly {
+  f64x2 v[BN_TOTALS_EARLY];
+};
+template <int C>
+__device__ __forceinline__ void bn_totals_issue(const BnFuse &f, BnTotalsEarly<C> &e) {
+  static_assert((C & 1) == 0 && C <= BN_FUSE_MAXC, "wide form: two channels per 16-byte load");
+  constexpr int tpc = 256 / C, hp = C / 2;
+  const int tid = threadIdx.x;
+  const int p2 = tid % hp, which = (tid / hp) & 1, part = tid / C;
+#pragma unroll
+  for (int u = 0; u < BN_TOTALS_EARLY; ++u) {
+    const int bi = part + u * tpc;
+    e.v[u] = (part < tpc && bi < f.nblk) ? *reinterpret_cast<const f64x2 *>(f.partial + ((size_t)bi * 2 + which) * C + 2 * p2)
+                                          : f64x2{0.0, 0.0};
+  }
+}
+template <int C>
+__device__ __forceinline__ void bn_totals_finish(const BnFuse &f, const BnTotalsEarly<C> &e, double *scratch, double *tot) {
+  constexpr int tpc = 256 / C, hp = C / 2, U = BN_TOTALS_EARLY;
+  const int tid = threadIdx.x;
+  const int p2 = tid % hp, which = (tid / hp) & 1, part = tid / C;
+  if (part < tpc) {
+    f64x2 acc = {0.0, 0.0};
+#pragma unroll
+    for (int u = 0; u < U; ++u) acc += e.v[u];
+    for (int blk = part + U * tpc; blk < f.nblk; blk += U * tpc) {
+      f64x2 v[U];
+#pragma unroll
+      for (int u = 0; u < U; ++u) {
+        const int bi = blk + u * tpc;
+        v[u] = bi < f.nblk ? *reinterpret_cast<const f64x2 *>(f.partial + ((size_t)bi * 2 + which) * C + 2 * p2) : f64x2{0.0, 0.0};
+      }
+#pragma unroll
+      for (int u = 0; u < U; ++u) acc += v[u];
+    }
+    scratch[which * 256 + part * C + 2 * p2] = acc[0];
+    scratch[which * 256 + part * C + 2 * p2 + 1] = acc[1];
+  }
+  __syncthreads();
+  if (tid < C) {
+    double s1 = 0.0, s2 = 0.0;
+    for (int p = 0; p < tpc; ++p) {
+      s1 += scratch[p * C + tid];
+      s2 += scratch[256 + p * C + tid];
+    }
+    tot[tid] = s1;
+    tot[C + tid] = s2;
+  }
+}
+
+static inline bool bn_fuse_ok(int64_t nblk, int c, int64_t apply_grid) {
+  return c <= BN_FUSE_MAXC && nblk <= BN_FUSE_BLOCKS && nblk * apply_grid * 2 * c * (int64_t)sizeof(double) <= (48ll << 20);
+}
+
+struct ConvPre {
+  BnFuse fuse;
+  const float *gamma, *beta;
+  float leak;
+  int64_t n_bn;
+  const int64_t *n_bn_dev;
+};
diff --git a/sgnn_amd/csrc/common.h b/sgnn_amd/csrc/common.h
--- a/sgnn_amd/csrc/common.h
+++ b/sgnn_amd/csrc/common.h
@@ -34,7 +34,8 @@
 int sgnn_conv_fwd_impl(const float *x, int64_t n_in, int cin, const float *w, int K, const int32_t *table, int64_t ld,
                        int64_t n_out, int cout, float *y, int flags, int in_shift, const int32_t *kmap,
                        const int32_t *kadd, int in_mul, int groups, int table_rows, const ConvEpi *epi,
-                       sgnn_stream_t stream);
+                       sgnn_stream_t stream, const struct ConvPre *pre = nullptr);
+bool sgnn_conv_fold_small_ok(int cin, int cout, int K, int64_t n_out);
 int64_t sgnn_conv_grid_blocks(int64_t n_out, int cin, int cout, int K);
 struct BnLin {
   const float *g;
@@ -89,7 +90,8 @@
 int sgnn_conv_bwd_weight_impl(const float *x, int64_t n_in, int cin, int64_t ldx, const float *dy, int cout, int64_t ld_dy,
                               const int32_t *table, int64_t ld, int K, int64_t n_out, float *dw, int in_shift,
                               const int32_t *kmap, const int32_t *kadd, int in_mul, int groups, int table_rows, void *ws,
-                              int64_t ws_bytes, sgnn_stream_t stream, const int64_t *n_dev = nullptr);
+                              int64_t ws_bytes, sgnn_stream_t stream, const int64_t *n_dev = nullptr,
+                              const struct ConvPre *pre = nullptr);
 int sgnn_expand_maps(const int32_t **S, const int32_t **ST, const int32_t **PAR);
 int sgnn_linear_fwd_rows(const float *x, int64_t n, int cin, const float *const *w, const float *const *b, int cout,
                          float *y, sgnn_stream_t stream, const int64_t *n_dev = nullptr);
diff --git a/sgnn_amd/csrc/conv.hip b/sgnn_amd/csrc/conv.hip
--- a/sgnn_amd/csrc/conv.hip
+++ b/sgnn_amd/csrc/conv.hip
@@ -2,6 +2,7 @@
 #include "common.h"
 
 #include "conv_common.h"
+#include "bn_fuse.h"
 
 #define CONV_SMALL_GRID ((int64_t)((g_tune.conv_small_rows + CONV_ROWS_PER_BLOCK - 1) / CONV_ROWS_PER_BLOCK))
 
@@ -216,16 +217,25 @@
   conv_fwd_body<CIN, COUT, CONV_MREP, false, true>(x, n_in, w, table, ld, K, n_out, y, flags, in_shift, ex, epi, wg_cap);
 }
 
-template <int CIN, int COUT>
+template <class T>
+__device__ __forceinline__ const T &conv_pack_first(const T &t) { return t; }
+
+template <int CIN, int COUT, class... PREARG>
 __global__ __launch_bounds__(256) void k_conv_small(const float *__restrict__ x, int64_t n_in,
                                                    const float *__restrict__ w, const int32_t *__restrict__ table,
                                                    int64_t ld, int K, int64_t n_out, float *y, int flags, int in_shift,
-                                                   ConvEpi epi) {
+                                                   ConvEpi epi, PREARG... prearg) {
+  constexpr bool PRE = sizeof...(PREARG) == 1;
+  static_assert(sizeof...(PREARG) <= 1, "at most one folded layer");
   using C = ConvCfg<CIN, COUT>;
   constexpr int V = C::V, CINP = C::CINP, NT = C::NT;
   constexpr int KW = 7;
   __shared__ float red[4][NT * 256];
   __shared__ double sred[4][2][NT * 16];
+  constexpr int PC = PRE ? CIN : 1;
+  __shared__ double pre_scratch[PRE ? 512 : 1], pre_tot[2 * PC];
+  __shared__ float pre_mean[PC], pre_inv[PC];
+  static_assert(!PRE || (CINP == CIN && (CIN & 1) == 0 && CIN <= 16), "folded BatchNorm: whole quarters, the wide table form");
   const int tid = threadIdx.x, lane = tid & 63, wave = tid >> 6;
   const int r = lane & 15, q = lane >> 4;
   const int64_t row0 = (int64_t)blockIdx.x * 16;
@@ -249,6 +259,26 @@
   const uint32_t lane_off = (uint32_t)(row0 + r) * 4u;
   const uint32_t ld4 = (uint32_t)ld * 4u;
 
+  BnTotalsEarly<PC == 1 ? 2 : PC> pre_early;
+  float km[PRE ? V : 1], ki[PRE ? V : 1], kg[PRE ? V : 1], kb[PRE ? V : 1];
+  if constexpr (PRE) {
+    const ConvPre &pre = conv_pack_first(prearg...);
+    if (pre.fuse.partial) {
+      bn_totals_issue<CIN>(pre.fuse, pre_early);
+    } else {
+#pragma unroll
+      for (int s = 0; s < V; ++s) {
+        km[s] = pre.fuse.running_mean[q * V + s];
+        ki[s] = pre.fuse.running_var[q * V + s];
+      }
+    }
+#pragma unroll
+    for (int s = 0; s < V; ++s) {
+      kg[s] = pre.gamma ? pre.gamma[q * V + s] : 1.f;
+      kb[s] = pre.beta ? pre.beta[q * V + s] : 0.f;
+    }
+  }
+
   int32_t id[KW];
 #pragma unroll
   for (int kk = 0; kk < KW; ++kk) {
@@ -344,6 +374,53 @@
 #pragma unroll
       for (int s = 0; s < V; ++s)
         if (3 * V + s >= CIN) a[kk][s] = (q >= conv_first_pad_quarter<CIN, V>(s)) ? 0.f : a[kk][s];
+  }
+  if constexpr (PRE) {
+    const ConvPre &pre = conv_pack_first(prearg...);
+    if (pre.fuse.partial) {
+      const int64_t n_bn = sgnn_dyn_n(pre.n_bn, pre.n_bn_dev);
+      bn_totals_finish<CIN>(pre.fuse, pre_early, pre_scratch, pre_tot);
+      if (tid < CIN) {
+        const BnFuse &fuse = pre.fuse;
+        const int ch = tid;
+        const double s1 = pre_tot[ch], s2 = pre_tot[CIN + ch];
+        const double mu = s1 / (double)n_bn;
+        double var = s2 / (double)n_bn - mu * mu;
+        if (var < 0.0) var = 0.0;
+        const float fm = (float)mu, fi = (float)(1.0 / sqrt(var + (double)fuse.eps));
+        pre_mean[ch] = fm;
+        pre_inv[ch] = fi;
+        if (blockIdx.x == 0) {
+          fuse.save_mean[ch] = fm;
+          fuse.save_invstd[ch] = fi;
+          if (fuse.running_mean) fuse.running_mean[ch] = fuse.momentum * fuse.running_mean[ch] + (1.f - fuse.momentum) * fm;
+          if (fuse.running_var) {
+            const double unb = var * ((double)n_bn / (double)(n_bn > 1 ? n_bn - 1 : 1));
+            fuse.running_var[ch] = fuse.momentum * fuse.running_var[ch] + (1.f - fuse.momentum) * (float)unb;
+          }
+        }
+      }
+      __syncthreads();
+#pragma unroll
+      for (int s = 0; s < V; ++s) {
+        km[s] = pre_mean[q * V + s];
+        ki[s] = pre_inv[q * V + s];
+      }
+    } else {
+#pragma unroll
+      for (int s = 0; s < V; ++s) ki[s] = 1.0f / sqrtf(ki[s] + pre.fuse.eps);
+      if (blockIdx.x == 0 && wave == 0 && r == 0) {
+#pragma unroll
+        for (int s = 0; s < V; ++s) {
+          pre.fuse.save_mean[q * V + s] = km[s];
+          pre.fuse.save_invstd[q * V + s] = ki[s];
+        }
+      }
+    }
+#pragma unroll
+    for (int kk = 0; kk < KW; ++kk)
+#pragma unroll
+      for (int s = 0; s < V; ++s) a[kk][s] = id[kk] < 0 ? 0.f : sgnn_bn_act(a[kk][s], km[s], ki[s], kg[s], kb[s], pre.leak);
   }
   f32x4 acc[2][NT];
 #pragma unroll
@@ -460,6 +537,19 @@
   X(8, 1) X(12, 8) X(16, 12) X(16, 34) X(16, 30) X(16, 26) X(16, 48) X(32, 16) X(16, 32) X(4, 16) X(16, 4) \
   X(16, 24) X(24, 16) X(24, 32) X(32, 24) X(64, 32) X(32, 64) X(56, 28) X(28, 56) X(32, 32) X(28, 16) X(16, 28)
 
+#define CONV_PRE_CASES(X) X(8, 8) X(8, 12) X(12, 12) X(12, 16) X(16, 16) X(4, 16)
+#define DW_FINE_ROWS 16384
+
+bool sgnn_conv_fold_small_ok(int cin, int cout, int K, int64_t n_out) {
+  const int64_t grid4 = (n_out + CONV_ROWS_PER_BLOCK - 1) / CONV_ROWS_PER_BLOCK;
+  if (!g_tune.conv_small || K > 28 || n_out <= 0 || grid4 >= CONV_SMALL_GRID || n_out >= DW_FINE_ROWS) return false;
+#define X(CI, CO) \
+  if (cin == CI && cout == CO) return true;
+  CONV_PRE_CASES(X)
+#undef X
+  return false;
+}
+
 int64_t sgnn_conv_grid_blocks(int64_t n_out, int cin, int cout, int K) {
   const int64_t grid4 = (n_out + CONV_ROWS_PER_BLOCK - 1) / CONV_ROWS_PER_BLOCK;
   if (grid4 < CONV_SMALL_GRID) return (n_out + 15) / 16;
@@ -505,7 +595,7 @@
 int sgnn_conv_fwd_impl(const float *x, int64_t n_in, int cin, const float *w, int K, const int32_t *table, int64_t ld,
                        int64_t n_out, int cout, float *y, int flags, int in_shift, const int32_t *kmap,
                        const int32_t *kadd, int in_mul, int groups, int table_rows, const ConvEpi *epi_in,
-                       sgnn_stream_t stream) {
+                       sgnn_stream_t stream, const ConvPre *pre) {
   SGNN_CHECK_ARG(cin >= 1 && cout >= 1 && K >= 1 && K <= 64 && n_out >= 0 && ld >= n_out && in_shift >= 0 &&
                  in_shift < 31 && in_mul >= 1 && groups >= 1 && groups <= 64 && table_rows >= 1 &&
                  table_rows <= 64 && (kmap || table_rows >= K));
@@ -552,7 +642,22 @@
       conv_launch_big<CI, CO, EXV>(grid4, s, x, n_in, w, table, ld, K, n_out, y, flags, in_shift, ex, epi); \
     done = true;                                                                                        \
   } while (0)
-  if (plain && !small && g_tune.conv_unrolled && sgnn_conv_u_supported(cin, cout, K))
+  if (pre) {
+    SGNN_CHECK_ARG(plain && flags == 0 && in_shift == 0 && sgnn_conv_fold_small_ok(cin, cout, K, n_out));
+    SGNN_CHECK_ARG(pre->fuse.save_mean && pre->fuse.save_invstd && pre->n_bn > 0);
+    SGNN_CHECK_ARG(pre->fuse.partial ? (pre->fuse.nblk >= 1 && (((uintptr_t)pre->fuse.partial) & 15) == 0)
+                                     : (pre->fuse.running_mean && pre->fuse.running_var));
+#define X(CI, CO)                                                                                              \
+  if (!done && cin == CI && cout == CO) {                                                                      \
+    SGNN_LAUNCH((k_conv_small<CI, CO, ConvPre>), dim3((unsigned)((n_out + 15) / 16)), dim3(256), 0, s, x, n_in, w, \
+                table, ld, K, n_out, y, flags, in_shift, epi, *pre);                                           \
+    done = true;                                                                                               \
+  }
+    CONV_PRE_CASES(X)
+#undef X
+    SGNN_CHECK_ARG(done);
+  }
+  if (!done && plain && !small && g_tune.conv_unrolled && sgnn_conv_u_supported(cin, cout, K))
     done = sgnn_conv_u_launch(x, n_in, cin, w, K, table, ld, n_out, cout, y, flags, in_shift, epi, s);
 #define X(CI, CO) \
   if (!done && plain && cin == CI && cout == CO) LAUNCH_FWD(CI, CO, false);
@@ -689,12 +794,18 @@
 #ifndef DW_PAIR
 #define DW_PAIR 1
 #endif
-template <int CIN, int COUT, bool EX, int KPBT = 0>
+struct DwPre {
+  const float *mean, *invstd, *gamma, *beta;
+  float leak;
+};
+template <int CIN, int COUT, bool EX, int KPBT = 0, class... PREARG>
 __global__ __launch_bounds__(256) void k_conv_dw(const float *__restrict__ x, int64_t n_in,
                                                 const float *__restrict__ dy, const int32_t *__restrict__ table,
                                                 int64_t ld, int K, int64_t n_out, float *__restrict__ partial,
                                                 int64_t rows_per_block, int in_shift, ConvEx ex, int64_t ldx,
-                                                int64_t ld_dy, const int64_t *n_dev) {
+                                                int64_t ld_dy, const int64_t *n_dev, PREARG... prearg) {
+  constexpr bool PRE = sizeof...(PREARG) == 1;
+  static_assert(sizeof...(PREARG) <= 1, "at most one folded layer");
   if (n_dev) {
     n_out = sgnn_dyn_n(n_out, n_dev);
     const int64_t per = (n_out + gridDim.x - 1) / gridDim.x;
@@ -766,6 +877,30 @@
           if (3 * V + s >= CIN) g[m][s] = (q == 3) ? 0.f : g[m][s];
     }
   };
+  static_assert(!PRE || (KPBT == 1 && !EX && CINP == CIN), "folded BatchNorm: the one-offset kernel of whole quarters");
+  float pm[PRE ? GW : 1], pi[PRE ? GW : 1], pg[PRE ? GW : 1], pb[PRE ? GW : 1];
+  if constexpr (PRE) {
+    const DwPre &pre = conv_pack_first(prearg...);
+    const int pch0 = RCX ? rc_chunk * 4 : q * V;
+#pragma unroll
+    for (int s = 0; s < GW; ++s) {
+      pm[s] = pre.mean[pch0 + s];
+      pi[s] = pre.invstd[pch0 + s];
+      pg[s] = pre.gamma ? pre.gamma[pch0 + s] : 1.f;
+      pb[s] = pre.beta ? pre.beta[pch0 + s] : 0.f;
+    }
+  }
+  auto act_rows = [&](int32_t iv, float(&g)[NI][GW]) {
+    if constexpr (PRE) {
+      const float leak = conv_pack_first(prearg...).leak;
+#pragma unroll
+      for (int m = 0; m < NI; ++m) {
+        const int32_t id = __builtin_amdgcn_ds_bpermute((RCX ? m * RPI + rc_row : m * 16 + i16) * 4, iv);
+#pragma unroll
+        for (int s = 0; s < GW; ++s) g[m][s] = id < 0 ? 0.f : sgnn_bn_act(g[m][s], pm[s], pi[s], pg[s], pb[s], leak);
+      }
+    }
+  };
   auto store_rows = [&](const float(&g)[NI][GW]) {
 #pragma unroll
     for (int m = 0; m < NI; ++m) {
@@ -894,6 +1029,7 @@
         if (kk + 1 < DW_KPB) gather(idxv[kk + 1], g1);
         __builtin_amdgcn_sched_barrier(0);
         norm_rows(g0);
+        if constexpr (PRE) act_rows(idxv[kk], g0);
         store_rows(g0);
         mma_chunk(kk, b);
         __builtin_amdgcn_sched_barrier(0);
@@ -901,6 +1037,7 @@
           if (kk + 2 < DW_KPB) gather(idxv[kk + 2], g0);
           __builtin_amdgcn_sched_barrier(0);
           norm_rows(g1);
+          if constexpr (PRE) act_rows(idxv[kk + 1], g1);
           store_rows(g1);
           mma_chunk(kk + 1, b);
           __builtin_amdgcn_sched_barrier(0);
@@ -1111,7 +1248,6 @@
   dw[e] = s;
 }
 
-#define DW_FINE_ROWS 16384
 static int64_t dw_rows_per_block(int64_t n_out) {
   int64_t rpb = (n_out + g_tune.conv_dw_blocks - 1) / g_tune.conv_dw_blocks;
   rpb = ((rpb + 255) / 256) * 256;
@@ -1150,7 +1286,7 @@
 int sgnn_conv_bwd_weight_impl(const float *x, int64_t n_in, int cin, int64_t ldx, const float *dy, int cout, int64_t ld_dy,
                               const int32_t *table, int64_t ld, int K, int64_t n_out, float *dw, int in_shift,
                               const int32_t *kmap, const int32_t *kadd, int in_mul, int groups, int table_rows, void *ws,
-                              int64_t ws_bytes, sgnn_stream_t stream, const int64_t *n_dev) {
+                              int64_t ws_bytes, sgnn_stream_t stream, const int64_t *n_dev, const ConvPre *pre) {
   SGNN_CHECK_ARG(ldx >= cin && ldx <= 1024 && ld_dy >= cout && ld_dy <= 1024);
   SGNN_CHECK_ARG(cin >= 1 && cout >= 1 && K >= 1 && K <= 64 && n_out >= 0 && ld >= n_out && dw &&
                  in_shift >= 0 && in_shift < 31 && in_mul >= 1 && groups >= 1 && groups <= 64 && table_rows >= 1 &&
@@ -1205,7 +1341,31 @@
     }                                                                                                      \
     done = true;                                                                                           \
   } while (0)
-  if (plain && cin == 1 && cout == 8 && g_tune.conv_dw_c1) {
+  if (pre) {
+    SGNN_CHECK_ARG(plain && in_shift == 0 && sgnn_conv_fold_small_ok(cin, cout, K, n_out) && pre->fuse.save_mean &&
+                   pre->fuse.save_invstd);
+    if (!ws || ws_bytes < sgnn_conv_bwd_weight_ws_bytes(n_out, K, cin, cout)) {
+      sgnn_set_error("sgnn_conv_bwd_weight: workspace too small");
+      return SGNN_ENOWS;
+    }
+    const DwPre dp{pre->fuse.save_mean, pre->fuse.save_invstd, pre->gamma, pre->beta, pre->leak};
+    const int prof = sgnn_prof_begin_launch(1, n_out, cin, cout, K, 0, s);
+#define X(CI, CO)                                                                                                    \
+  if (!done && cin == CI && cout == CO) {                                                                            \
+    SGNN_LAUNCH((k_conv_dw<CI, CO, false, 1, DwPre>), dim3((unsigned)nblk, (unsigned)K), dim3(256), 0, s, x, n_in, dy, table, ld, \
+                K, n_out, (float *)ws, rpb, in_shift, ex, ldx, ld_dy, n_dev, dp);                                    \
+    done = true;                                                                                                     \
+  }
+    CONV_PRE_CASES(X)
+#undef X
+    sgnn_prof_end_launch(prof, s);
+    SGNN_CHECK_ARG(done);
+    if (sgnn_dw_batch && sgnn_dw_batch->n < DW_BATCH_MAX)
+      sgnn_dw_batch->d[sgnn_dw_batch->n++] = DwDesc{(const float *)ws, dw, nblk, elems, 0};
+    else
+      SGNN_LAUNCH(k_dw_reduce, dim3((unsigned)((elems + 31) / 32)), dim3(256), 0, s, (const float *)ws, nblk, elems, dw);
+  }
+  if (!done && plain && cin == 1 && cout == 8 && g_tune.conv_dw_c1) {
     if (!ws || ws_bytes < sgnn_conv_bwd_weight_ws_bytes(n_out, K, cin, cout)) {
       sgnn_set_error("sgnn_conv_bwd_weight: workspace too small");
       return SGNN_ENOWS;
diff --git a/sgnn_amd/csrc/prog.hip b/sgnn_amd/csrc/prog.hip
--- a/sgnn_amd/csrc/prog.hip
+++ b/sgnn_amd/csrc/prog.hip
@@ -1,6 +1,7 @@
 #include <mutex>
 #include <vector>
 #include "common.h"
+#include "bn_fuse.h"
 
 enum {
   OP_CONV_SUBM = 0, OP_CONV_DOWN = 1, OP_UNPOOL = 2, OP_BN = 3, OP_ADD = 4, OP_JOIN = 5,
@@ -95,6 +96,7 @@
 #define g_fuse (g_tune.prog_fusion != 0)
 #define g_lin_add (g_tune.prog_lin_add != 0)
 #define g_lin_bn (g_tune.prog_lin_bn != 0)
+#define g_bn_fold (g_tune.prog_bn_fold_small != 0)
 struct Plan {
   std::vector<int> add_dst;
   std::vector<int> add_src;
@@ -102,6 +104,7 @@
   std::vector<int> root, col;
   std::vector<int64_t> ld;
   std::vector<char> join_view;
+  std::vector<int> fold, pre_bn;
   std::vector<int> lin_bn;
   Kind kind = TRAINING;
   std::vector<char> f32;
@@ -112,6 +115,48 @@
 
 bool strided_conv_ok(const Op &o) {
   return sgnn_conv_epi_supported(o.cin, o.cout) && sgnn_conv_epi_supported(o.cout, o.cin) && dw_shape_ok(o.cin, o.cout);
+}
+
+int stats_producer(const View &v, const Plan &P, int i) {
+  const Op &b = v.op(i);
+  for (int p = i - 1; p >= 0 && p >= i - 2; --p) {
+    const Op &o = v.op(p);
+    const bool fused_add = P.add_dst[p] >= 0;
+    if (p + 1 + (fused_add ? 1 : 0) != i || !o.is_conv()) continue;
+    if ((fused_add ? P.add_dst[p] : o.out) != b.in0) continue;
+    if (!sgnn_conv_epi_supported(o.cin, o.cout) || ConvSetup(v, o).n_out <= 0) continue;
+    return p;
+  }
+  return -1;
+}
+
+bool fold_candidate(const View &v, int i) {
+  if (i + 1 >= v.nops) return false;
+  const Op &b = v.op(i), &o = v.op(i + 1);
+  if (b.type != OP_BN || !o.is_conv() || o.in0 != b.out || o.lev != b.lev || o.cin != b.cin) return false;
+  const ConvSetup cs(v, o);
+  return cs.ok && sgnn_conv_fold_small_ok(o.cin, o.cout, cs.K, cs.n_out);
+}
+
+void plan_bn_folds(const View &v, const std::vector<int> &readers, Plan &P) {
+  if (!g_bn_fold || !g_tune.bn_fuse || P.kind != TRAINING) return;
+  for (int i = 0; i < v.nops; ++i) {
+    const Op &b = v.op(i);
+    if (b.type != OP_BN || b.out < v.n_ext || b.out >= v.nbuf || readers[b.out] != 1 || P.root[b.out] != b.out) continue;
+    if (b.lev < 0 || b.lev >= v.nlev || v.lev_n[b.lev] <= 0) continue;
+    const int j = i + 1;
+    if (j >= v.nops || !fold_candidate(v, i)) continue;
+    const Op &o = v.op(j);
+    const ConvSetup cs(v, o);
+    if (!cs.ok || !sgnn_conv_fold_small_ok(o.cin, o.cout, cs.K, cs.n_out)) continue;
+    const int p = stats_producer(v, P, i);
+    if (p < 0) continue;
+    const Op &po = v.op(p);
+    const int64_t nblk = sgnn_conv_grid_blocks(ConvSetup(v, po).n_out, po.cin, po.cout, po.K());
+    if (!bn_fuse_ok(nblk, b.cin, (cs.n_out + 15) / 16)) continue;
+    P.fold[i] = j;
+    P.pre_bn[j] = i;
+  }
 }
 
 void make_plan(const View &v, const int32_t *keep, Plan &P, Kind kind) {
@@ -126,6 +171,8 @@
   P.skip.assign(v.nops, 0);
   P.join_view.assign(v.nops, 0);
   P.lin_bn.assign(v.nops, -1);
+  P.fold.assign(v.nops, -1);
+  P.pre_bn.assign(v.nops, -1);
   P.root.resize(v.nbuf);
   P.col.assign(v.nbuf, 0);
   P.ld.resize(v.nbuf);
@@ -210,6 +257,7 @@
     P.col[b] = c;
     P.ld[b] = row_ld(r);
   }
+  plan_bn_folds(v, readers, P);
 }
 
 struct Layout {
@@ -403,7 +451,13 @@
   return (need + 255) & ~int64_t(255);
 }
 
-int64_t ws_need(const View &v) { return ws_main(v) + ws_stats(v); }
+bool may_fold(const View &v) {
+  if (!g_fuse || !g_bn_fold || !g_tune.bn_fuse) return false;
+  for (int i = 0; i + 1 < v.nops; ++i)
+    if (fold_candidate(v, i)) return true;
+  return false;
+}
+int64_t ws_need(const View &v) { return ws_main(v) + (may_fold(v) ? 2 : 1) * ws_stats(v); }
 
 struct SideLane {
   hipStream_t stream = nullptr;
@@ -431,7 +485,7 @@
   Layout L;
   std::vector<const double *> pre;
   std::vector<int64_t> pre_nblk;
-  double *stats_ws;
+  double *stats_ws, *stats_ws2;
 
   bool prepare(Kind kind, const int32_t *keep) {
     make_plan(v, keep, P, kind);
@@ -439,6 +493,7 @@
     pre = std::vector<const double *>(v.nops, nullptr);
     pre_nblk = std::vector<int64_t>(v.nops, 0);
     stats_ws = (double *)((char *)ws + ws_main(v));
+    stats_ws2 = (double *)((char *)stats_ws + ws_stats(v));
     return true;
   }
   int ch(int b) const { return b < 0 ? 0 : v.bufs[2 * b + 1]; }
@@ -448,6 +503,26 @@
   float *param(int p) const { return (p >= 0 && p < nparams) ? (float *)params[p] : nullptr; }
   const int32_t *index(int i) const { return (i >= 0 && i < nidx && idx) ? (const int32_t *)idx[i] : nullptr; }
   const int64_t *count(int c) const { return (lev_cnt && c >= 0 && c < v.nlev) ? (const int64_t *)lev_cnt[c] : nullptr; }
+  ConvPre conv_pre(int i, float *save, bool forward) const {
+    const Op &b = v.op(i);
+    ConvPre p{};
+    if (forward && training) {
+      p.fuse.partial = pre[i];
+      p.fuse.nblk = (int)pre_nblk[i];
+    }
+    p.fuse.eps = v.opf[4 * i];
+    p.fuse.momentum = v.opf[4 * i + 1];
+    p.fuse.running_mean = param(b.par + 2);
+    p.fuse.running_var = param(b.par + 3);
+    p.fuse.save_mean = save;
+    p.fuse.save_invstd = save + b.cin;
+    p.gamma = param(b.par);
+    p.beta = param(b.par + 1);
+    p.leak = v.opf[4 * i + 2];
+    p.n_bn = v.lev_n[b.lev];
+    p.n_bn_dev = count(b.lev);
+    return p;
+  }
   int wait_once(void *&wait_event) const {
     if (!wait_event) return SGNN_OK;
     sgnn_stamp("down-wait<", stream);
@@ -676,13 +751,26 @@
         if (g_fuse && training && cs.n_out > 0 && j < nops && v.op(j).type == OP_BN && v.op(j).in0 == dst_buf &&
             sgnn_conv_epi_supported(cin, cout)) {
           epi.stats = 1;
-          epi.partial = c.stats_ws;
-          c.pre[j] = c.stats_ws;
+          epi.partial = (PL.pre_bn[i] >= 0 && c.pre[PL.pre_bn[i]] == c.stats_ws) ? c.stats_ws2 : c.stats_ws;
+          c.pre[j] = epi.partial;
           c.pre_nblk[j] = sgnn_conv_grid_blocks(cs.n_out, cin, cout, cs.K);
         }
-        epi.ldx = c.ld(in0);
         epi.ldy = c.ld(dst_buf);
         epi.n_dev = c.count(cs.cnt_class);
+        if (PL.pre_bn[i] >= 0) {
+          const int bi = PL.pre_bn[i];
+          const ConvPre cp = c.conv_pre(bi, arena + L.aux_off[bi], true);
+          if (training && !cp.fuse.partial) {
+            sgnn_set_error("sgnn_prog_forward: a folded BatchNorm has no statistics partials");
+            return SGNN_EINVAL;
+          }
+          const int bin = v.op(bi).in0;
+          epi.ldx = c.ld(bin);
+          PROG_TRY(sgnn_conv_fwd_impl(B(bin), n, cin, c.param(par), cs.K, cs.tab_f, cs.ld_f, cs.n_out, cout, B(dst_buf), 0, 0,
+                                      nullptr, nullptr, 1, 1, cs.K, &epi, stream, &cp));
+          break;
+        }
+        epi.ldx = c.ld(in0);
         PROG_TRY(sgnn_conv_fwd_impl(B(in0), n, cin, c.param(par), cs.K, cs.tab_f, cs.ld_f, cs.n_out, cout, B(dst_buf), 0, 0,
                                     nullptr, nullptr, 1, 1, cs.K, &epi, stream));
         break;
@@ -693,6 +781,7 @@
                                      c.count(lev)));
         break;
       case OP_BN: {
+        if (PL.fold[i] >= 0) break;
         float *save = arena + L.aux_off[i];
         PROG_TRY(sgnn_bn_fwd_impl(B(in0), c.ld(in0), n, cin, c.param(par), c.param(par + 1), c.param(par + 2), c.param(par + 3),
                                   opf[4 * i], opf[4 * i + 1], training, opf[4 * i + 2], save, save + cin, B(out), c.ld(out),
@@ -919,9 +1008,17 @@
     }
   }
   const int64_t slice = dw_slice(c.v, i);
-  PROG_TRY(sgnn_conv_bwd_weight_impl(g.X(in0), cs.n, cin, c.ld(in0), dy, cout, ld_dy, cs.tab_f, cs.ld_f, cs.K, cs.n_out,
-                                     g.PG(o.par), 0, nullptr, nullptr, 1, 1, cs.K, lane.ws + lane.off, slice, (sgnn_stream_t)ls,
-                                     c.count(cs.cnt_class)));
+  if (c.P.pre_bn[i] >= 0) {
+    const int bi = c.P.pre_bn[i], bin = c.v.op(bi).in0;
+    const ConvPre cp = c.conv_pre(bi, const_cast<float *>(g.arena) + c.L.aux_off[bi], false);
+    PROG_TRY(sgnn_conv_bwd_weight_impl(g.X(bin), cs.n, cin, c.ld(bin), dy, cout, ld_dy, cs.tab_f, cs.ld_f, cs.K, cs.n_out,
+                                       g.PG(o.par), 0, nullptr, nullptr, 1, 1, cs.K, lane.ws + lane.off, slice, (sgnn_stream_t)ls,
+                                       c.count(cs.cnt_class), &cp));
+  } else {
+    PROG_TRY(sgnn_conv_bwd_weight_impl(g.X(in0), cs.n, cin, c.ld(in0), dy, cout, ld_dy, cs.tab_f, cs.ld_f, cs.K, cs.n_out,
+                                       g.PG(o.par), 0, nullptr, nullptr, 1, 1, cs.K, lane.ws + lane.off, slice, (sgnn_stream_t)ls,
+                                       c.count(cs.cnt_class)));
+  }
   if (ls != lane.hs) sgnn_stamp("dw>", (sgnn_stream_t)ls);
   lane.off += slice;
   return SGNN_OK;
diff --git a/sgnn_amd/csrc/tune.hip b/sgnn_amd/csrc/tune.hip
--- a/sgnn_amd/csrc/tune.hip
+++ b/sgnn_amd/csrc/tune.hip
@@ -8,6 +8,7 @@
      1,
      1,
      256,
+     1,
      1,
      1,
      1,
@@ -40,6 +41,7 @@
     {"prog_lin_bn", &sgnn_tune::prog_lin_bn, 0, 1, true},
     {"prog_lin_add", &sgnn_tune::prog_lin_add, 0, 1, true},
     {"bn_fuse", &sgnn_tune::bn_fuse, 0, 1, true},
+    {"prog_bn_fold_small", &sgnn_tune::prog_bn_fold_small, 0, 1, true},
 };
 const Field *find(const char *name) {
   if (!name) return nullptr;
```
